# tungphambasement/DCNN

Measured on AMD Instinct MI355X. Metric: images/sec (whole node) ResNet-18 Tiny-ImageNet training at 1/2/4/8 MI355X, higher is better.
Workload: dtype bf16; 1 GPU; model=resnet18_tiny_imagenet, global_batch=256, per_gpu_batch=256, parallelism=dp1, optimizer=adam, hipgraph=True, engine=native (C++ host API)

## Files before the change

### dcnn_amd/csrc/host/dcnn/nn.hpp

```cpp
#pragma once
#include <functional>
#include <map>
#include <memory>
#include <string>
#include <vector>

#include "json.hpp"
#include "ops.hpp"
#include "tensor.hpp"

namespace dcnn {

struct ParamArena;
struct Param {
  std::string name;
  std::vector<int64_t> shape;
  Layout layout = Layout::NCHW;
  Tensor value, grad, shadow;
  Tensor m, v;
  std::shared_ptr<ParamArena> arena;
};

struct ParamArena {
  Tensor value, grad, m, v, shadow;
// ... 39 lines not shown
  };
  MbCache& mbc() { return caches_[mb_]; }
  std::map<int, MbCache> caches_;
  int mb_ = 0;
  bool input_grad_ = true;
  Param& add_param(const std::string& n, const std::vector<int64_t>& shape, Layout phys, const std::vector<float>& init);
  std::string name_;
  Device dev_ = Device::cpu();
  std::vector<Param> params_;
};

class ConvBase : public Layer {
 public:
  std::vector<int64_t> output_shape(const std::vector<int64_t>& in) const override;
  void build(const std::vector<int64_t>& in, Device dev, uint64_t seed) override;
  Tensor forward(const Tensor& x, bool training) override;
  Tensor backward(const Tensor& dy) override { return backward_impl(dy, nullptr); }
  double flops(const std::vector<int64_t>& in) const override;
  virtual bool backward_residual(const Tensor& dy, const Tensor& residual, Tensor& dx) {
    (void)dy; (void)residual; (void)dx;
    return false;
  }

 protected:
  ConvBase(int in_ch, int out_ch, int kh, int kw, int groups, int sh, int sw, int ph, int pw, bool bias,
           std::string name)
      : Layer(std::move(name)), ci_(in_ch), co_(out_ch), kh_(kh), kw_(kw), g_(groups), sh_(sh), sw_(sw), ph_(ph),
        pw_(pw), bias_(bias) {}
  ConvShape shape_for(const std::vector<int64_t>& in) const;
  void geometry_config(json::Value& p) const;
  const float* bias_value() const { return bias_ ? params_[1].value.ptr<float>() : nullptr; }
  float* bias_grad() { return bias_ ? params_[1].grad.ptr<float>() : nullptr; }
  virtual bool depthwise() const { return false; }
  int group_in() const { return depthwise() ? 1 : ci_ / g_; }
  Tensor backward_impl(const Tensor& dy, const Tensor* residual);
  int ci_, co_, kh_, kw_, g_, sh_, sw_, ph_, pw_;
  bool bias_;
};

class Conv2D : public ConvBase {
 public:
  Conv2D(int in_ch, int out_ch, int kh, int kw, int sh = 1, int sw = 1, int ph = 0, int pw = 0, bool bias = true,
         std::string name = "conv2d");
  std::string type() const override { return "conv2d"; }
  json::Value parameters_config() const override;
  Tensor forward(const Tensor& x, bool training) override;
  Tensor backward(const Tensor& dy) override;
  bool takes_raw_input(const std::vector<int64_t>& in) const override;
  void set_stats_consumer(class BatchNorm* bn) { stats_to_ = bn; }
  void set_bnb_producer(class BatchNorm* bn) { bnb_from_ = bn; }
  void set_block_bnb_producer(class BatchNorm* bn) { bnb_block_from_ = bn; }
  bool backward_residual(const Tensor& dy, const Tensor& residual, Tensor& dx) override;
  bool ran_stem() const;
  void backward_stem_bn(const Tensor& dy, const gpu_ops::StemBn& bn);
  void sync_shadow() override;
  bool make_transposed_operand(std::vector<int64_t>& row, long& tiles);

 private:
  class BatchNorm* stats_to_ = nullptr;
  class BatchNorm* bnb_from_ = nullptr;
  class BatchNorm* bnb_block_from_ = nullptr;
  Tensor wt_;
  const void* dgrad_operand(bool& transposed) const;
};

class DepthwiseConv2D : public ConvBase {
 public:
  DepthwiseConv2D(int channels, int kh, int kw, int sh = 1, int sw = 1, int ph = 0, int pw = 0, bool bias = true,
                  std::string name = "depthwise_conv2d");
  std::string type() const override { return "depthwise_conv2d"; }
  json::Value parameters_config() const override;

 protected:
  bool depthwise() const override { return true; }
};

class GroupedConv2D : public ConvBase {
 public:
  GroupedConv2D(int in_ch, int out_ch, int kh, int kw, int groups, int sh = 1, int sw = 1, int ph = 0, int pw = 0,
                bool bias = true, std::string name = "grouped_conv2d");
  std::string type() const override { return "grouped_conv2d"; }
  json::Value parameters_config() const override;
  bool backward_residual(const Tensor& dy, const Tensor& residual, Tensor& dx) override;
};

class Dense : public Layer {
 public:
  Dense(int in_features, int out_features, bool bias = true, std::string name = "dense");
  std::string type() const override { return "dense"; }
  json::Value parameters_config() const override;
  std::vector<int64_t> output_shape(const std::vector<int64_t>& in) const override;
  void build(const std::vector<int64_t>& in, Device dev, uint64_t seed) override;
  Tensor forward(const Tensor& x, bool training) override;
  Tensor backward(const Tensor& dy) override;
  double flops(const std::vector<int64_t>& in) const override { return 6.0 * in[0] * in_ * out_; }

 private:
  int in_, out_;
  bool bias_;
};

class BatchNorm : public Layer {
 public:
  explicit BatchNorm(int num_features, float eps = 1e-5f, float momentum = 0.1f, bool affine = true,
                     std::string name = "batchnorm");
  std::string type() const override { return "batchnorm"; }
  json::Value parameters_config() const override;
  std::vector<int64_t> output_shape(const std::vector<int64_t>& in) const override { return in; }
  double flops(const std::vector<int64_t>& in) const override {
    return 15.0 * (double)in[0] * (double)in[1] * (double)in[2] * (double)in[3];
  }
  void build(const std::vector<int64_t>& in, Device dev, uint64_t seed) override;
  Tensor forward(const Tensor& x, bool training) override;
  Tensor backward(const Tensor& dy) override;
  void set_fused_relu(bool b) { fused_relu_ = b; }
  bool fused_relu() const { return fused_relu_; }
  Tensor forward_residual(const Tensor& x, const Tensor& residual, bool relu, bool training);
  Tensor backward_residual(const Tensor& dy, Tensor* branch);
  void forward_deferred(const Tensor& x, bool training);
  Tensor forward_dual(const Tensor& x, BatchNorm& deferred, bool relu, bool training);
  bool backward_dual(const Tensor& dy, BatchNorm& deferred, Tensor& dx, Tensor& dx_deferred);
  void set_fused_pool(class Pool2D* p) { fused_pool_ = p; }
  bool fused_pool() const { return fused_pool_ != nullptr; }
  gpu_ops::BnbOperands bnb_operands(int mb);
  void offer_bwd_stats(const void* dy, const float* slab, int rows) {
    bwd_dy_ = dy;
    bwd_slab_ = slab;
    bwd_rows_ = rows;
  }
  void offer_stats(const void* x, const float* slab, int rows) {
    pending_x_ = x;
    pending_slab_ = slab;
    pending_rows_ = rows;
  }
  bool backward_into_stem(const Tensor& dy, Conv2D& stem);
  Tensor running_mean, running_var;

 private:
  int c_;
  float eps_, momentum_;
  bool affine_;
  bool train_ = true;
  bool fused_relu_ = false;
  Tensor forward_impl(const Tensor& x, bool training, const Tensor* residual, bool relu);
  Tensor apply_deferred(bool training);
  class Pool2D* fused_pool_ = nullptr;
  gpu_ops::BnRaw deferred_raw_{nullptr, 0};
  const void* bwd_dy_ = nullptr;
  const float* bwd_slab_ = nullptr;
  int bwd_rows_ = 0;
  const void* pending_x_ = nullptr;
  const float* pending_slab_ = nullptr;
  int pending_rows_ = 0;
};

class Activation : public Layer {
 public:
  explicit Activation(std::string kind = "relu", std::string name = "activation");
  std::string type() const override { return "activation"; }
  json::Value parameters_config() const override;
  std::vector<int64_t> output_shape(const std::vector<int64_t>& in) const override { return in; }
  Tensor forward(const Tensor& x, bool training) override;
  Tensor backward(const Tensor& dy) override;
  bool is_relu() const;
  void set_passthrough(bool b) { passthrough_ = b; }

 private:
  std::string kind_;
  int code_;
  bool passthrough_ = false;
};

class GroupNorm : public Layer {
 public:
  GroupNorm(int num_groups, int num_channels, float eps = 1e-5f, bool affine = true, std::string name = "groupnorm");
  std::string type() const override { return "groupnorm"; }
  json::Value parameters_config() const override;
  std::vector<int64_t> output_shape(const std::vector<int64_t>& in) const override { return in; }
  void build(const std::vector<int64_t>& in, Device dev, uint64_t seed) override;
  Tensor forward(const Tensor& x, bool training) override;
  Tensor backward(const Tensor& dy) override;

 private:
  int g_, c_;
  float eps_;
  bool affine_;
  bool gb_identity_ = false;
  Tensor ident_, scratch_;
};

class Dropout : public Layer {
 public:
  explicit Dropout(float rate = 0.5f, std::string name = "dropout");
  std::string type() const override { return "dropout"; }
  json::Value parameters_config() const override;
  std::vector<int64_t> output_shape(const std::vector<int64_t>& in) const override { return in; }
  void build(const std::vector<int64_t>& in, Device dev, uint64_t seed) override;
  Tensor forward(const Tensor& x, bool training) override;
  Tensor backward(const Tensor& dy) override;

 private:
  float p_;
  uint64_t seed_ = 0, draw_ = 0;
};

class Pool2D : public Layer {
 public:
  Pool2D(bool max, int kh, int kw, int sh, int sw, int ph, int pw, std::string name);
  std::string type() const override { return max_ ? "maxpool2d" : "avgpool2d"; }
  json::Value parameters_config() const override;
  std::vector<int64_t> output_shape(const std::vector<int64_t>& in) const override;
  Tensor forward(const Tensor& x, bool training) override;
  Tensor backward(const Tensor& dy) override;
  bool is_max() const { return max_; }
  PoolShape shape_for(const std::vector<int64_t>& in) const;
  void set_fused_producer(class BatchNorm* bn) { bn_ = bn; }
  uint8_t* accept_prepooled(const Tensor& ypool, const std::vector<int64_t>& in);
  void clear_prepooled() { mbc().flag = false; }

 private:
  class BatchNorm* bn_ = nullptr;
  bool max_;
  int kh_, kw_, sh_, sw_, ph_, pw_;
};

class Flatten : public Layer {
 public:
  explicit Flatten(std::string name = "flatten") : Layer(std::move(name)) {}
  std::string type() const override { return "flatten"; }
  json::Value parameters_config() const override { return json::Value::object(); }
  std::vector<int64_t> output_shape(const std::vector<int64_t>& in) const override;
  Tensor forward(const Tensor& x, bool training) override;
  Tensor backward(const Tensor& dy) override;
};

class ResidualBlock : public Layer {
 public:
  ResidualBlock(std::vector<std::unique_ptr<Layer>> main, std::vector<std::unique_ptr<Layer>> shortcut,
                std::string activation = "relu", std::string name = "residual_block");
  std::string type() const override { return "residual_block"; }
  json::Value parameters_config() const override;
  std::vector<int64_t> output_shape(const std::vector<int64_t>& in) const override;
  double flops(const std::vector<int64_t>& in) const override;
  void build(const std::vector<int64_t>& in, Device dev, uint64_t seed) override;
  Tensor forward(const Tensor& x, bool training) override;
  Tensor backward(const Tensor& dy) override;
  void sync_shadow() override;
  void collect_params(std::vector<Param*>& out) override;
  void collect_layers(std::vector<Layer*>& out) override;
  void set_micro_batch(int mb) override;
  const std::vector<std::unique_ptr<Layer>>& main_path() const { return main_; }
  const std::vector<std::unique_ptr<Layer>>& shortcut_path() const { return short_; }
  class BatchNorm* fused_tail() const;
  class Conv2D* head_conv() const;
  class BatchNorm* dual_shortcut() const;

 private:
  std::vector<std::unique_ptr<Layer>> main_, short_;
  std::string act_;
};

std::unique_ptr<Layer> create_layer(const json::Value& rec);

void fuse_bn_relu(std::vector<std::unique_ptr<Layer>>& seq, bool on);
void fuse_blocks(std::vector<std::unique_ptr<Layer>>& seq, bool on);

class Sequential {
 public:
  explicit Sequential(std::string name = "sequential") : name_(std::move(name)) {}
  Sequential(Sequential&&) = default;
  Sequential& operator=(Sequential&&) = default;
// ... 175 lines not shown
```

### dcnn_amd/csrc/host/dcnn/ops.hpp

```cpp
#pragma once
#include <cstdint>

namespace dcnn {

struct ConvShape {
  int N, C, H, W, Co, KH, KW, SH, SW, PH, PW, OH, OW;
};
struct PoolShape {
  int N, C, H, W, OH, OW, KH, KW, SH, SW, PH, PW;
};
enum ActKind { ACT_RELU = 0, ACT_LEAKY_RELU = 1, ACT_ELU = 2, ACT_SIGMOID = 3, ACT_TANH = 4, ACT_LINEAR = 5 };

namespace cpu_ops {
void conv_fwd(const float* x, const float* w, const float* b, float* y, const ConvShape& s);
void conv_bwd(const float* x, const float* w, const float* dy, float* dx, float* dw, float* db, const ConvShape& s);
void dwconv_fwd(const float* x, const float* w, const float* b, float* y, const ConvShape& s);
void dwconv_bwd(const float* x, const float* w, const float* dy, float* dx, float* dw, float* db, const ConvShape& s);
void gconv_fwd(const float* x, const float* w, const float* b, float* y, const ConvShape& s, int groups);
void gconv_bwd(const float* x, const float* w, const float* dy, float* dx, float* dw, float* db, const ConvShape& s,
               int groups);
void dense_fwd(const float* x, const float* w, const float* b, float* y, long N, long In, long Out);
void dense_bwd(const float* x, const float* w, const float* dy, float* dx, float* dw, float* db, long N, long In,
               long Out);
void bn_fwd(const float* x, float* y, long N, long C, long HW, const float* g, const float* b, float eps, bool train,
// ... 22 lines not shown
          float bc2, float wd, bool decoupled);
void sgd(float* p, const float* g, float* vel, long n, float lr, float momentum);
}

namespace gpu_ops {
void begin_deferred_reduce();
void end_deferred_reduce();
void flush_deferred_reduce();
void set_fault(int f);
void input_to_nhwc(const float* x, void* y, int N, int C, int HW);
void nhwc_to_nchw(const void* x, void* y, int N, int HW, int C);
void nchw_to_nhwc_bf16(const void* x, void* y, int N, int HW, int C);
void cast_bf16(const float* x, void* y, long n);
void zero(void* p, long nbytes);
const float* conv_fwd(const void* x, const void* w, const float* bias, void* y, const ConvShape& s,
                      int* stat_rows = nullptr);
struct BnbOperands {
  const void* y;
  const void* x;
  const float* mean;
  const float* istd;
  const float* gamma = nullptr;
  const float* beta = nullptr;
  bool mask_from_x = false;
};
const float* conv_dgrad(const void* dy, const void* w, void* dx, const ConvShape& s, const void* residual = nullptr,
                        bool w_transposed = false, const BnbOperands* bnb = nullptr, int* bnb_rows = nullptr);
void weight_transpose(const void* w, void* wt, int Co, int T, int C);
void multi_weight_transpose(const int64_t* table, int n, long max_tiles);
void conv_wgrad(const void* dy, const void* x, float* gw, float* gb, const ConvShape& s);
void dwconv_fwd(const void* x, const void* w, const float* bias, void* y, const ConvShape& s);
void dwconv_dgrad(const void* dy, const void* w, void* dx, const ConvShape& s, const void* residual = nullptr);
void dwconv_wgrad(const void* dy, const void* x, float* gw, float* gb, const ConvShape& s);
void gconv_fwd(const void* x, const void* w, const float* bias, void* y, const ConvShape& s, int groups);
void gconv_dgrad(const void* dy, const void* w, void* dx, const ConvShape& s, int groups,
                 const void* residual = nullptr);
void gconv_wgrad(const void* dy, const void* x, float* gw, float* gb, const ConvShape& s, int groups);
bool stem_ok(const ConvShape& s);
const float* stem_fwd(const float* x, const void* w, const float* bias, void* y, const ConvShape& s,
                      int* stat_rows = nullptr);
void stem_wgrad(const void* dy, const float* x, float* gw, float* gb, const ConvShape& s);
struct StemBn {
  const void* x;
  const float* mean;
  const float* istd;
  const float* gamma;
  float* dgamma;
  float* dbeta;
  const float* slab;
  int rows;
  bool train;
};
void stem_wgrad_bn(const void* dy, const float* x, float* gw, float* gb, const ConvShape& s, const StemBn& bn);
void dense_fwd(const void* x, const void* w, const float* bias, void* y, int N, int In, int Out);
void dense_dgrad(const void* dy, const void* w, void* dx, int N, int In, int Out);
void dense_wgrad(const void* dy, const void* x, float* gw, float* gb, int N, int In, int Out);
void bn_fwd(const void* x, void* y, long R, int C, const float* g, const float* b, float eps, bool train,
            float* rmean, float* rvar, float momentum, float* smean, float* sistd, bool relu = false,
            const void* residual = nullptr);
void bn_fwd_slab(const void* x, void* y, long R, int C, const float* slab, int rows, const float* g, const float* b,
                 float eps, float* rmean, float* rvar, float momentum, float* smean, float* sistd, bool relu,
                 const void* residual = nullptr);
void bn_bwd_slab(const void* dy, const void* x, void* dx, long R, int C, const float* mean, const float* istd,
                 const float* g, float* dg, float* db, bool train, const float* slab, int rows);
void bn_bwd(const void* dy, const void* x, void* dx, long R, int C, const float* mean, const float* istd,
            const float* g, float* dg, float* db, bool train, const void* yout = nullptr, void* dy_out = nullptr);
struct SecondaryStats {
  SecondaryStats();
  ~SecondaryStats();
};
struct BnRaw {
  const float* slab;
  int rows;
};
BnRaw bn_stats_raw(const void* x, long R, int C, const float* slab, int rows);
struct BnFwdSide {
  const void* x;
  BnRaw raw;
  const float* g;
  const float* b;
  float eps;
  float* rmean;
  float* rvar;
  float momentum;
  float* smean;
  float* sistd;
};
bool bn_dual_ok(long R, int C);
void bn_fwd_dual(const BnFwdSide& a, const BnFwdSide& b, void* y, long R, int C, bool relu, bool train);
struct BnBwdSides {
  const void* x;
  void* dx;
  const float* mean;
  const float* istd;
  const float* g;
  float* dg;
  float* db;
};
void bn_bwd_dual(const void* dy, const BnBwdSides& a, const float* slab_a, int rows_a, const BnBwdSides& b, long R,
                 int C);
bool bn_relu_maxpool_ok(const PoolShape& p);
void bn_relu_maxpool(const void* x, void* y, uint8_t* idx, const PoolShape& p, const float* slab, int rows,
                     const float* g, const float* b, float eps, float* rmean, float* rvar, float momentum,
                     float* smean, float* sistd);
const float* maxpool_bwd_bnb(const void* dy, const uint8_t* idx, const void* ypool, const void* x, const float* mean,
                             const float* istd, void* dx, const PoolShape& p, int* rows);
void maxpool_fwd(const void* x, void* y, uint8_t* idx, const PoolShape& p);
void maxpool_bwd(const void* dy, const uint8_t* idx, void* dx, const PoolShape& p);
void avgpool_fwd(const void* x, void* y, const PoolShape& p);
void avgpool_bwd(const void* dy, void* dx, const PoolShape& p);
void act_fwd(int kind, const void* x, void* y, long n, float alpha);
void act_bwd(int kind, const void* x, const void* dy, void* dx, long n, float alpha);
double softmax_ce(const void* pred, const int64_t* labels, void* grad, int N, int C, long* correct);
double loss(int kind, const void* pred, const float* target, const int64_t* labels, void* grad, int N, int C,
            float param, long* correct, float grad_scale = 1.f);
void loss_launch(int kind, const void* pred, const float* target, const int64_t* labels, void* grad, int N, int C,
                 float param, float grad_scale = 1.f);
double read_last_loss(long* correct);
void groupnorm_fwd(const void* x, void* y, int N, int HW, int C, int G, const float* g, const float* b, float eps,
                   float* smean, float* sistd);
void groupnorm_bwd(const void* dy, const void* x, void* dx, int N, int HW, int C, int G, const float* g,
                   const float* mean, const float* istd, float* dg, float* db);
void softmax_fwd(const void* x, void* y, long rows, int C);
void softmax_bwd(const void* y, const void* dy, void* dx, long rows, int C);
void dropout(const void* x, void* y, long n, float p, uint64_t seed);
void add(const void* a, const void* b, void* y, long n, bool relu);
void relu_mask(const void* dy, const void* y, void* dx, long n);
void adam(float* p, const float* g, float* m, float* v, void* shadow, long n, float lr, float b1, float b2, float eps,
          float bc1, float bc2, float wd, bool decoupled);
void sgd(float* p, const float* g, float* vel, void* shadow, long n, float lr, float momentum);
void adam_hyper_step(float* hyper, float b1, float b2);
void adam_dev(float* p, const float* g, float* m, float* v, void* shadow, long n, float b1, float b2, float eps,
              float wd, bool decoupled, const float* hyper);
const void* loss_device();
}

}
```

### dcnn_amd/csrc/host/nn.cpp

```cpp
#include "dcnn/nn.hpp"

#include "../kernels/fusion_plan.h"

#include <algorithm>
#include <chrono>
#include <cmath>
#include <cstdio>
#include <cstdlib>
#include <filesystem>
#include <fstream>
#include <iostream>
#include <sstream>
#include <stdexcept>

namespace dcnn {

namespace {
struct Rng {
  uint64_t s;
  explicit Rng(uint64_t seed) : s(seed * 0x9e3779b97f4a7c15ull + 0x632be59bd9b4e019ull) {}
  uint64_t next() {
    uint64_t z = (s += 0x9e3779b97f4a7c15ull);
    z = (z ^ (z >> 30)) * 0xbf58476d1ce4e5b9ull;
    z = (z ^ (z >> 27)) * 0x94d049bb133111ebull;
// ... 125 lines not shown
    if (depthwise())
      cpu_ops::dwconv_fwd(x.ptr<float>(), w, b, y.ptr<float>(), s);
    else
      cpu_ops::gconv_fwd(x.ptr<float>(), w, b, y.ptr<float>(), s, g_);
  }
  mbc().a = x;
  return y;
}

Tensor ConvBase::backward_impl(const Tensor& dy, const Tensor* residual) {
  const Tensor& x_ = mbc().a;
  const ConvShape s = shape_for(x_.shape());
  float* gw = params_[0].grad.ptr<float>();
  float* gb = bias_grad();
  if (dev_.is_gpu()) {
    if (depthwise())
      gpu_ops::dwconv_wgrad(dy.data(), x_.data(), gw, gb, s);
    else
      gpu_ops::gconv_wgrad(dy.data(), x_.data(), gw, gb, s, g_);
    if (!input_grad_ && residual == nullptr) return Tensor();
    Tensor dx = act_empty(x_.shape(), dev_);
    const void* w = params_[0].shadow.data();
    const void* r = residual ? residual->data() : nullptr;
    if (depthwise())
      gpu_ops::dwconv_dgrad(dy.data(), w, dx.data(), s, r);
    else
      gpu_ops::gconv_dgrad(dy.data(), w, dx.data(), s, g_, r);
    return dx;
  }
  Tensor dx = input_grad_ ? act_empty(x_.shape(), dev_) : Tensor();
  float* dxp = input_grad_ ? dx.ptr<float>() : nullptr;
  const float* w = params_[0].value.ptr<float>();
  if (depthwise())
    cpu_ops::dwconv_bwd(x_.ptr<float>(), w, dy.ptr<float>(), dxp, gw, gb, s);
  else
    cpu_ops::gconv_bwd(x_.ptr<float>(), w, dy.ptr<float>(), dxp, gw, gb, s, g_);
  return dx;
}

Conv2D::Conv2D(int in_ch, int out_ch, int kh, int kw, int sh, int sw, int ph, int pw, bool bias, std::string name)
    : ConvBase(in_ch, out_ch, kh, kw, 1, sh, sw, ph, pw, bias, std::move(name)) {}

json::Value Conv2D::parameters_config() const {
  json::Value p = json::Value::object();
  p["in_channels"] = ci_;
  p["out_channels"] = co_;
  p["kernel_h"] = kh_;
  p["kernel_w"] = kw_;
  geometry_config(p);
  p["optimized"] = "mfma";
  return p;
}

bool Conv2D::takes_raw_input(const std::vector<int64_t>& in) const {
  return dev_.is_gpu() && in.size() == 4 && in[1] == ci_ && gpu_ops::stem_ok(shape_for(in));
}

Tensor Conv2D::forward(const Tensor& x, bool training) {
  Tensor& x_ = mbc().a;
  check_act(x, dev_, "conv2d");
  const ConvShape s = shape_for(x.shape());
  Tensor y = act_empty({s.N, s.Co, s.OH, s.OW}, dev_);
  const float* b = bias_value();
  if (dev_.is_gpu() && x.dtype() == DType::F32) {
    if (x.layout() != Layout::NCHW || !gpu_ops::stem_ok(s)) throw std::runtime_error(name_ + ": fp32 input");
    int rows = 0;
    const float* st = gpu_ops::stem_fwd(x.ptr<float>(), params_[0].shadow.data(), b, y.data(), s,
                                        stats_to_ && training ? &rows : nullptr);
    if (stats_to_ && training) stats_to_->offer_stats(y.data(), st, rows);
    x_ = x;
    return y;
  }
  if (dev_.is_gpu()) {
    int rows = 0;
    const float* st = gpu_ops::conv_fwd(x.data(), params_[0].shadow.data(), b, y.data(), s,
                                        stats_to_ && training ? &rows : nullptr);
    if (stats_to_ && training) stats_to_->offer_stats(y.data(), st, rows);
  } else
    cpu_ops::conv_fwd(x.ptr<float>(), params_[0].value.ptr<float>(), b, y.ptr<float>(), s);
  x_ = x;
  return y;
}

bool Conv2D::ran_stem() const {
  const Tensor& x_ = const_cast<Conv2D*>(this)->mbc().a;
  return dev_.is_gpu() && x_.defined() && x_.dtype() == DType::F32;
}

void Conv2D::backward_stem_bn(const Tensor& dy, const gpu_ops::StemBn& bn) {
  const Tensor& x_ = mbc().a;
  const ConvShape s = shape_for(x_.shape());
  gpu_ops::stem_wgrad_bn(dy.data(), x_.ptr<float>(), params_[0].grad.ptr<float>(), bias_grad(), s, bn);
}

Tensor Conv2D::backward(const Tensor& dy) {
  const Tensor& x_ = mbc().a;
  const ConvShape s = shape_for(x_.shape());
  float* gb = bias_grad();
  if (dev_.is_gpu() && x_.dtype() == DType::F32) {
    gpu_ops::stem_wgrad(dy.data(), x_.ptr<float>(), params_[0].grad.ptr<float>(), gb, s);
    return Tensor();
  }
  if (dev_.is_gpu()) {
    gpu_ops::conv_wgrad(dy.data(), x_.data(), params_[0].grad.ptr<float>(), gb, s);
    if (!input_grad_) return Tensor();
    Tensor dx = act_empty(x_.shape(), dev_);
    bool tr = false;
    const void* w = dgrad_operand(tr);
    if (bnb_from_ != nullptr) {
      const gpu_ops::BnbOperands ops = bnb_from_->bnb_operands(mb_);
      int rows = 0;
      const float* st = gpu_ops::conv_dgrad(dy.data(), w, dx.data(), s, nullptr, tr, &ops, &rows);
      if (rows > 0) bnb_from_->offer_bwd_stats(dx.data(), st, rows);
      return dx;
    }
    gpu_ops::conv_dgrad(dy.data(), w, dx.data(), s, nullptr, tr);
    return dx;
  }
  Tensor dx = act_empty(x_.shape(), dev_);
  {
    cpu_ops::conv_bwd(x_.ptr<float>(), params_[0].value.ptr<float>(), dy.ptr<float>(), dx.ptr<float>(),
                      params_[0].grad.ptr<float>(), gb, s);
  }
  return dx;
}

bool Conv2D::backward_residual(const Tensor& dy, const Tensor& residual, Tensor& dx) {
  const Tensor& x_ = mbc().a;
  if (!dev_.is_gpu() || x_.dtype() == DType::F32 || residual.shape() != x_.shape())
    throw std::runtime_error(name_ + ": backward_residual is a GPU fusion");
  const ConvShape s = shape_for(x_.shape());
  float* gb = bias_grad();
  gpu_ops::conv_wgrad(dy.data(), x_.data(), params_[0].grad.ptr<float>(), gb, s);
  dx = act_empty(x_.shape(), dev_);
  bool tr = false;
  const void* w = dgrad_operand(tr);
  if (bnb_block_from_ != nullptr) {
    const gpu_ops::BnbOperands ops = bnb_block_from_->bnb_operands(mb_);
    int rows = 0;
    const float* st = gpu_ops::conv_dgrad(dy.data(), w, dx.data(), s, residual.data(), tr, &ops, &rows);
    if (rows > 0) bnb_block_from_->offer_bwd_stats(dx.data(), st, rows);
    return true;
  }
  gpu_ops::conv_dgrad(dy.data(), w, dx.data(), s, residual.data(), tr);
  return true;
// ... 147 lines not shown
json::Value BatchNorm::parameters_config() const {
  json::Value p = json::Value::object();
  p["num_features"] = c_;
  p["epsilon"] = (double)eps_;
  p["momentum"] = (double)momentum_;
  p["affine"] = affine_;
  return p;
}

void BatchNorm::build(const std::vector<int64_t>& in, Device dev, uint64_t seed) {
  (void)in;
  (void)seed;
  dev_ = dev;
  params_.clear();
  if (affine_) {
    add_param("gamma", {c_, 1, 1, 1}, Layout::NCHW, std::vector<float>((size_t)c_, 1.f));
    add_param("beta", {c_, 1, 1, 1}, Layout::NCHW, std::vector<float>((size_t)c_, 0.f));
  }
  running_mean = Tensor::zeros({c_}, DType::F32, dev);
  running_var = Tensor::from_host(std::vector<float>((size_t)c_, 1.f), {c_}, dev);
  caches_.clear();
}

Tensor BatchNorm::forward(const Tensor& x, bool training) { return forward_impl(x, training, nullptr, fused_relu_); }

Tensor BatchNorm::forward_residual(const Tensor& x, const Tensor& residual, bool relu, bool training) {
  if (!dev_.is_gpu()) throw std::runtime_error(name_ + ": forward_residual is a GPU fusion");
  if (residual.shape() != x.shape()) throw std::runtime_error(name_ + ": residual shape mismatch");
  return forward_impl(x, training, &residual, relu);
}

Tensor BatchNorm::forward_impl(const Tensor& x, bool training, const Tensor* residual, bool relu) {
  check_act(x, dev_, "batchnorm");
  MbCache& mc = mbc();
  Tensor& x_ = mc.a;
  Tensor& mean_ = mc.b;
  Tensor& istd_ = mc.c;
  mean_.ensure({c_}, DType::F32, dev_);
  istd_.ensure({c_}, DType::F32, dev_);
  if (x.dim(1) != c_) throw std::runtime_error(name_ + ": channel count mismatch");
  train_ = training;
  const long N = x.dim(0), HW = x.dim(2) * x.dim(3);
  Tensor y = act_empty(x.shape(), dev_);
  const float* g = affine_ ? params_[0].value.ptr<float>() : nullptr;
  const float* b = affine_ ? params_[1].value.ptr<float>() : nullptr;
  const void* res = residual ? residual->data() : nullptr;
  const bool slab = dev_.is_gpu() && training && pending_x_ == x.data() && pending_slab_ && pending_rows_ > 0;
  if (fused_pool_ != nullptr) {
    fused_pool_->set_micro_batch(mb_);
    const PoolShape p = fused_pool_->shape_for(x.shape());
    if (dev_.is_gpu() && training && relu && residual == nullptr && gpu_ops::bn_relu_maxpool_ok(p)) {
      Tensor yp = act_empty({p.N, p.C, p.OH, p.OW}, dev_);
      uint8_t* idx = fused_pool_->accept_prepooled(yp, x.shape());
      gpu_ops::bn_relu_maxpool(x.data(), yp.data(), idx, p, slab ? pending_slab_ : nullptr, slab ? pending_rows_ : 0,
                               g, b, eps_, running_mean.ptr<float>(), running_var.ptr<float>(), momentum_,
                               mean_.ptr<float>(), istd_.ptr<float>());
      mc.d = Tensor();
      mc.flag = false;
      pending_x_ = nullptr;
      pending_slab_ = nullptr;
      pending_rows_ = 0;
      x_ = x;
      return yp;
    }
    fused_pool_->clear_prepooled();
  }
  if (slab) {
    gpu_ops::bn_fwd_slab(x.data(), y.data(), N * HW, c_, pending_slab_, pending_rows_, g, b, eps_,
                         running_mean.ptr<float>(), running_var.ptr<float>(), momentum_, mean_.ptr<float>(),
                         istd_.ptr<float>(), relu, res);
    mc.d = relu ? y : Tensor();
    mc.flag = relu && res == nullptr && training;
  } else if (dev_.is_gpu()) {
    gpu_ops::bn_fwd(x.data(), y.data(), N * HW, c_, g, b, eps_, training, running_mean.ptr<float>(),
                    running_var.ptr<float>(), momentum_, mean_.ptr<float>(), istd_.ptr<float>(), relu, res);
    mc.d = relu ? y : Tensor();
    mc.flag = relu && res == nullptr && training;
  } else {
    cpu_ops::bn_fwd(x.ptr<float>(), y.ptr<float>(), N, c_, HW, g, b, eps_, training, running_mean.ptr<float>(),
                    running_var.ptr<float>(), momentum_, mean_.ptr<float>(), istd_.ptr<float>());
  }
  pending_x_ = nullptr;
  pending_slab_ = nullptr;
  pending_rows_ = 0;
  x_ = x;
  return y;
}

void BatchNorm::forward_deferred(const Tensor& x, bool training) {
  check_act(x, dev_, "batchnorm");
  if (!dev_.is_gpu()) throw std::runtime_error(name_ + ": forward_deferred is a GPU fusion");
  if (x.dim(1) != c_) throw std::runtime_error(name_ + ": channel count mismatch");
  MbCache& mc = mbc();
  mc.a = x;
  mc.b.ensure({c_}, DType::F32, dev_);
  mc.c.ensure({c_}, DType::F32, dev_);
  mc.d = Tensor();
  mc.flag = false;
  train_ = training;
  deferred_raw_ = gpu_ops::BnRaw{nullptr, 0};
  if (training) {
    const bool slab = pending_x_ == x.data() && pending_slab_ && pending_rows_ > 0;
    deferred_raw_ = gpu_ops::bn_stats_raw(x.data(), x.dim(0) * x.dim(2) * x.dim(3), c_, slab ? pending_slab_ : nullptr,
                                          slab ? pending_rows_ : 0);
  }
  pending_x_ = nullptr;
  pending_slab_ = nullptr;
  pending_rows_ = 0;
}
// ... 61 lines not shown
  MbCache& mc = mbc();
  MbCache& oc = o.mbc();
  const Tensor& x_ = mc.a;
  if (!dev_.is_gpu() || bwd_dy_ != dy.data() || bwd_slab_ == nullptr || bwd_rows_ <= 0 || !train_ || !o.train_ ||
      oc.a.shape() != x_.shape() || o.c_ != c_)
    return false;
  const long R = x_.dim(0) * x_.dim(2) * x_.dim(3);
  if (!gpu_ops::bn_dual_ok(R, c_)) return false;
  dx = act_empty(x_.shape(), dev_);
  dx_o = act_empty(oc.a.shape(), dev_);
  auto side = [](BatchNorm& l, MbCache& c, Tensor& d) {
    return gpu_ops::BnBwdSides{c.a.data(),
                               d.data(),
                               c.b.ptr<float>(),
                               c.c.ptr<float>(),
                               l.affine_ ? l.params_[0].value.ptr<float>() : nullptr,
                               l.affine_ ? l.params_[0].grad.ptr<float>() : nullptr,
                               l.affine_ ? l.params_[1].grad.ptr<float>() : nullptr};
  };
  gpu_ops::bn_bwd_dual(dy.data(), side(*this, mc, dx), bwd_slab_, bwd_rows_, side(o, oc, dx_o), R, c_);
  bwd_dy_ = nullptr;
  bwd_slab_ = nullptr;
  bwd_rows_ = 0;
  return true;
}

Tensor BatchNorm::backward_residual(const Tensor& dy, Tensor* branch) {
  MbCache& mc = mbc();
  const Tensor& x_ = mc.a;
  const long N = x_.dim(0), HW = x_.dim(2) * x_.dim(3);
  Tensor dx = act_empty(x_.shape(), dev_);
  const float* g = affine_ ? params_[0].value.ptr<float>() : nullptr;
  float* dg = affine_ ? params_[0].grad.ptr<float>() : nullptr;
  float* db = affine_ ? params_[1].grad.ptr<float>() : nullptr;
  if (bwd_dy_ == dy.data() && bwd_slab_ != nullptr && bwd_rows_ > 0) {
    *branch = dy;
    gpu_ops::bn_bwd_slab(dy.data(), x_.data(), dx.data(), N * HW, c_, mc.b.ptr<float>(), mc.c.ptr<float>(), g, dg, db,
                         train_, bwd_slab_, bwd_rows_);
    bwd_dy_ = nullptr;
    bwd_slab_ = nullptr;
    bwd_rows_ = 0;
  } else if (mc.d.defined()) {
    *branch = act_empty(dy.shape(), dev_);
    gpu_ops::bn_bwd(dy.data(), x_.data(), dx.data(), N * HW, c_, mc.b.ptr<float>(), mc.c.ptr<float>(), g, dg, db,
                    train_, mc.d.data(), branch->data());
  } else {
    *branch = dy;
    gpu_ops::bn_bwd(dy.data(), x_.data(), dx.data(), N * HW, c_, mc.b.ptr<float>(), mc.c.ptr<float>(), g, dg, db,
                    train_);
  }
  return dx;
}

bool BatchNorm::backward_into_stem(const Tensor& dy, Conv2D& stem) {
  MbCache& mc = mbc();
  if (!dev_.is_gpu() || !train_ || bwd_dy_ != dy.data() || bwd_slab_ == nullptr || bwd_rows_ <= 0 ||
      !stem.ran_stem() || mc.a.dtype() != DType::BF16)
    return false;
  gpu_ops::StemBn bn{mc.a.data(),
                     mc.b.ptr<float>(),
                     mc.c.ptr<float>(),
                     affine_ ? params_[0].value.ptr<float>() : nullptr,
                     affine_ ? params_[0].grad.ptr<float>() : nullptr,
                     affine_ ? params_[1].grad.ptr<float>() : nullptr,
                     bwd_slab_,
                     bwd_rows_,
                     train_};
  stem.backward_stem_bn(dy, bn);
  bwd_dy_ = nullptr;
  bwd_slab_ = nullptr;
  bwd_rows_ = 0;
  return true;
}

Tensor BatchNorm::backward(const Tensor& dy) {
  MbCache& mc = mbc();
  const Tensor& x_ = mc.a;
  Tensor& mean_ = mc.b;
  Tensor& istd_ = mc.c;
  const long N = x_.dim(0), HW = x_.dim(2) * x_.dim(3);
  Tensor dx = act_empty(x_.shape(), dev_);
  const float* g = affine_ ? params_[0].value.ptr<float>() : nullptr;
  float* dg = affine_ ? params_[0].grad.ptr<float>() : nullptr;
  float* db = affine_ ? params_[1].grad.ptr<float>() : nullptr;
  if (dev_.is_gpu() && bwd_dy_ == dy.data() && bwd_slab_ != nullptr && bwd_rows_ > 0) {
    gpu_ops::bn_bwd_slab(dy.data(), x_.data(), dx.data(), N * HW, c_, mean_.ptr<float>(), istd_.ptr<float>(), g, dg,
                         db, train_, bwd_slab_, bwd_rows_);
    bwd_dy_ = nullptr;
    bwd_slab_ = nullptr;
    bwd_rows_ = 0;
  } else if (dev_.is_gpu())
    gpu_ops::bn_bwd(dy.data(), x_.data(), dx.data(), N * HW, c_, mean_.ptr<float>(), istd_.ptr<float>(), g, dg, db,
                    train_, mc.d.defined() ? mc.d.data() : nullptr);
  else
    cpu_ops::bn_bwd(x_.ptr<float>(), dy.ptr<float>(), mean_.ptr<float>(), istd_.ptr<float>(), g, dx.ptr<float>(), dg,
                    db, N, c_, HW, train_);
  return dx;
}

Activation::Activation(std::string kind, std::string name)
    : Layer(std::move(name)), kind_(std::move(kind)), code_(act_code(kind_)) {}

json::Value Activation::parameters_config() const {
  json::Value p = json::Value::object();
  p["activation"] = kind_;
  return p;
}

static float act_alpha(int code) { return code == ACT_ELU ? 1.0f : 0.01f; }

bool Activation::is_relu() const { return code_ == ACT_RELU; }

static int fuse_kind(const Layer* l) {
  if (dynamic_cast<const Conv2D*>(l)) return FK_CONV;
  if (dynamic_cast<const BatchNorm*>(l)) return FK_BN;
  if (auto* a = dynamic_cast<const Activation*>(l)) return a->is_relu() ? FK_RELU : FK_ACT;
  if (auto* p = dynamic_cast<const Pool2D*>(l)) return p->is_max() ? FK_MAXPOOL : FK_OTHER;
  return FK_OTHER;
}

static std::vector<int> fuse_kinds(const std::vector<std::unique_ptr<Layer>>& seq) {
  std::vector<int> k;
  for (const auto& l : seq) k.push_back(fuse_kind(l.get()));
  return k;
}

void fuse_bn_relu(std::vector<std::unique_ptr<Layer>>& seq, bool on) {
  const std::vector<int> f = plan_sequence_fusions(fuse_kinds(seq));
  for (size_t i = 0; i < seq.size(); ++i) {
// ... 400 lines not shown
  p.W = (int)in[3];
  p.KH = kh_;
  p.KW = kw_;
  p.SH = sh_;
  p.SW = sw_;
  p.PH = ph_;
  p.PW = pw_;
  p.OH = (p.H + 2 * ph_ - kh_) / sh_ + 1;
  p.OW = (p.W + 2 * pw_ - kw_) / sw_ + 1;
  return p;
}

std::vector<int64_t> Pool2D::output_shape(const std::vector<int64_t>& in) const {
  const PoolShape p = shape_for(in);
  return {in[0], in[1], p.OH, p.OW};
}

uint8_t* Pool2D::accept_prepooled(const Tensor& ypool, const std::vector<int64_t>& in) {
  MbCache& mc = mbc();
  const PoolShape p = shape_for(in);
  mc.a.ensure({(int64_t)p.N * p.C * p.OH * p.OW}, DType::U8, dev_);
  mc.b = ypool;
  mc.shape = in;
  mc.flag = true;
  return mc.a.ptr<uint8_t>();
}

Tensor Pool2D::forward(const Tensor& x, bool training) {
  (void)training;
  if (bn_ != nullptr && mbc().flag && mbc().b.defined() && mbc().b.data() == x.data())
    return x;
  mbc().flag = false;
  Tensor& idx_ = mbc().a;
  std::vector<int64_t>& in_shape_ = mbc().shape;
  check_act(x, dev_, "pool2d");
  const PoolShape p = shape_for(x.shape());
  Tensor y = act_empty({p.N, p.C, p.OH, p.OW}, dev_);
  in_shape_ = x.shape();
  if (max_) {
    const int64_t n = (int64_t)p.N * p.C * p.OH * p.OW;
    if (dev_.is_gpu()) {
      idx_.ensure({n}, DType::U8, dev_);
      gpu_ops::maxpool_fwd(x.data(), y.data(), idx_.ptr<uint8_t>(), p);
    } else {
      idx_.ensure({n}, DType::I32, dev_);
      cpu_ops::maxpool_fwd(x.ptr<float>(), y.ptr<float>(), idx_.ptr<int32_t>(), p);
    }
  } else if (dev_.is_gpu()) {
    gpu_ops::avgpool_fwd(x.data(), y.data(), p);
  } else {
    cpu_ops::avgpool_fwd(x.ptr<float>(), y.ptr<float>(), p);
  }
  return y;
}

Tensor Pool2D::backward(const Tensor& dy) {
  const Tensor& idx_ = mbc().a;
  const std::vector<int64_t>& in_shape_ = mbc().shape;
  const PoolShape p = shape_for(in_shape_);
  Tensor dx = act_empty(in_shape_, dev_);
  if (mbc().flag && bn_ != nullptr) {
    const gpu_ops::BnbOperands ops = bn_->bnb_operands(mb_);
    int rows = 0;
    const float* slab = gpu_ops::maxpool_bwd_bnb(dy.data(), idx_.ptr<uint8_t>(), mbc().b.data(), ops.x, ops.mean,
                                                 ops.istd, dx.data(), p, &rows);
    bn_->offer_bwd_stats(dx.data(), slab, rows);
    return dx;
  }
  if (max_) {
    if (dev_.is_gpu())
      gpu_ops::maxpool_bwd(dy.data(), idx_.ptr<uint8_t>(), dx.data(), p);
    else
      cpu_ops::maxpool_bwd(dy.ptr<float>(), idx_.ptr<int32_t>(), dx.ptr<float>(), p);
  } else if (dev_.is_gpu()) {
    gpu_ops::avgpool_bwd(dy.data(), dx.data(), p);
  } else {
    cpu_ops::avgpool_bwd(dy.ptr<float>(), dx.ptr<float>(), p);
  }
  return dx;
}

std::vector<int64_t> Flatten::output_shape(const std::vector<int64_t>& in) const {
  return {in[0], in[1] * in[2] * in[3], 1, 1};
}

Tensor Flatten::forward(const Tensor& x, bool training) {
  (void)training;
  std::vector<int64_t>& in_shape_ = mbc().shape;
  check_act(x, dev_, "flatten");
  in_shape_ = x.shape();
  const auto os = output_shape(x.shape());
  const int64_t HW = x.dim(2) * x.dim(3);
  if (!dev_.is_gpu()) return x.view(os);
  if (HW == 1) return x.view(os, Layout::NHWC);
  Tensor y = act_empty(os, dev_);
  gpu_ops::nhwc_to_nchw(x.data(), y.data(), (int)x.dim(0), (int)HW, (int)x.dim(1));
  return y;
}

Tensor Flatten::backward(const Tensor& dy) {
  const std::vector<int64_t>& in_shape_ = mbc().shape;
  const int64_t HW = in_shape_[2] * in_shape_[3];
  if (!dev_.is_gpu()) return dy.view(in_shape_);
  if (HW == 1) return dy.view(in_shape_, Layout::NHWC);
  Tensor dx = act_empty(in_shape_, dev_);
  gpu_ops::nchw_to_nhwc_bf16(dy.data(), dx.data(), (int)in_shape_[0], (int)HW, (int)in_shape_[1]);
// ... 153 lines not shown
std::vector<BatchNorm*> Sequential::batchnorms() {
  std::vector<Layer*> all;
  for (auto& l : layers_) l->collect_layers(all);
  std::vector<BatchNorm*> out;
  for (auto* l : all)
    if (auto* bn = dynamic_cast<BatchNorm*>(l)) out.push_back(bn);
  return out;
}

size_t Sequential::num_parameters() {
  size_t n = 0;
  for (auto* p : parameters()) n += (size_t)p->value.numel();
  return n;
}

void Sequential::zero_grad() {
  if (arena_) {
    gpu_ops::zero(arena_->grad.data(), (long)arena_->grad.nbytes());
    return;
  }
  for (auto* p : parameters()) {
    if (dev_.is_gpu())
      gpu_ops::zero(p->grad.data(), (long)p->grad.nbytes());
    else
      p->grad.zero_();
  }
}

std::vector<double> Sequential::layer_flops(const std::vector<int64_t>& in) const {
  std::vector<double> out;
  std::vector<int64_t> s = in;
  for (auto& l : layers_) {
    out.push_back(l->flops(s));
    s = l->output_shape(s);
  }
  return out;
}

Tensor Sequential::input_activation(const Tensor& x_in) const {
  if (x_in.rank() != 4 || x_in.dtype() != DType::F32) throw std::runtime_error("forward: expected fp32 (N, C, H, W)");
  Tensor x = x_in.device() == dev_ ? x_in : x_in.to(dev_);
  if (dev_.is_gpu() && !layers_.empty() && layers_[0]->takes_raw_input(x.shape())) return x;
  if (dev_.is_gpu()) {
    Tensor a = Tensor::empty(x.shape(), DType::BF16, dev_, Layout::NHWC);
    gpu_ops::input_to_nhwc(x.ptr<float>(), a.data(), (int)x.dim(0), (int)x.dim(1), (int)(x.dim(2) * x.dim(3)));
    x = a;
  }
  return x;
}

Tensor Sequential::forward_activation(const Tensor& x_in, int mb) {
  if (!initialized_) throw std::runtime_error("Sequential::forward before initialize()");
  Tensor x = x_in;
  for (auto& l : layers_) {
    l->set_micro_batch(mb);
    x = l->forward(x, training_);
  }
  return x;
}

Tensor Sequential::backward_activation(const Tensor& g_in, int mb) {
  Tensor g = g_in;
  static const bool defer_env = [] {
    const char* v = std::getenv("DCNN_DEFER_REDUCE");
    return !(v && std::string(v) == "0");
  }();
  const bool defer = dev_.is_gpu() && defer_env;
  static const bool stem_bn_env = [] {
    const char* v = std::getenv("DCNN_STEM_BN_FOLD");
    return !(v && std::string(v) == "0");
  }();
  const bool stem_bn_fold = dev_.is_gpu() && stem_bn_env && layers_.size() > 1;
  if (defer) gpu_ops::begin_deferred_reduce();
  try {
    for (size_t i = layers_.size(); i-- > 0;) {
      layers_[i]->set_micro_batch(mb);
      if (i == 1 && stem_bn_fold) {
        auto* bn = dynamic_cast<BatchNorm*>(layers_[1].get());
        auto* conv = dynamic_cast<Conv2D*>(layers_[0].get());
        if (bn && conv) {
          conv->set_micro_batch(mb);
          if (bn->backward_into_stem(g, *conv)) {
            if (bwd_hook_) bwd_hook_(1);
            if (bwd_hook_) bwd_hook_(0);
            g = Tensor();
            break;
          }
        }
      }
      g = layers_[i]->backward(g);
      if (bwd_hook_) bwd_hook_(i);
    }
  } catch (...) {
    if (defer) gpu_ops::end_deferred_reduce();
    throw;
  }
  if (defer) gpu_ops::end_deferred_reduce();
  return g;
}

Tensor Sequential::forward(const Tensor& x_in, int mb) {
  Tensor x = forward_activation(input_activation(x_in), mb);
  return x.view({x.dim(0), x.dim(1) * x.dim(2) * x.dim(3)}, x.layout());
}

void Sequential::backward(const Tensor& dlogits, int mb) {
  if (!layers_.empty()) layers_[0]->set_input_grad(false);
  Tensor g = dlogits.view({dlogits.dim(0), dlogits.dim(1), 1, 1}, dev_.is_gpu() ? Layout::NHWC : Layout::NCHW);
  backward_activation(g, mb);
}

json::Value Sequential::get_config() const {
  json::Value c = json::Value::object();
  c["name"] = name_;
  c["is_training"] = training_;
  json::Value ls = json::Value::array();
  for (auto& l : layers_) {
    json::Value r = json::Value::object();
    r["type"] = l->type();
    r["name"] = l->name();
    r["parameters"] = l->parameters_config();
    ls.push(std::move(r));
  }
  c["layers"] = std::move(ls);
  if (!input_chw_.empty() && input_chw_[0] > 0) {
    json::Value in = json::Value::array();
    for (auto v : input_chw_) in.push(v);
    c["input_shape"] = std::move(in);
  }
  return c;
}

void Sequential::print_config() const { std::cout << get_config().dump(2) << std::endl; }

Sequential Sequential::load_from_config(const json::Value& cfg) {
  Sequential m(cfg.get_string("name", "sequential"));
  for (auto& r : cfg.at("layers").items()) m.add(create_layer(r));
  m.set_training(cfg.get_bool("is_training", true));
  if (const json::Value* in = cfg.find("input_shape")) {
// ... 428 lines not shown
```

### dcnn_amd/csrc/host/ops_gpu.hip

```cpp
#include <hip/hip_runtime.h>

#include <algorithm>
#include <cmath>
#include <cstdio>
#include <cstdlib>
#include <cstring>
#include <map>
#include <mutex>
#include <stdexcept>
#include <string>
#include <unordered_map>
#include <vector>

#include "../kernels/api.h"
#include "dcnn/ops.hpp"
#include "dcnn/tensor.hpp"

#define HOST_HIP_CHECK(x)                                                                    \
  do {                                                                                       \
    hipError_t e_ = (x);                                                                     \
    if (e_ != hipSuccess) throw std::runtime_error(std::string(#x) + ": " + hipGetErrorString(e_)); \
  } while (0)

namespace dcnn {
// ... 663 lines not shown
  wgrad_split(splits, (long)s.C * s.KH * s.KW, s.C, gw, gb,
              [&](float* slab, float* bslab) { dcnn::dwconv_wgrad(kBF16, dy, x, slab, bslab, g, cur()); });
}

namespace {
GcArgs gc_args(const ConvShape& s, int groups) {
  return GcArgs{s.N, s.H, s.W, s.C, s.Co, groups, s.OH, s.OW, s.KH, s.KW, s.SH, s.SW, s.PH, s.PW};
}
}

void gconv_fwd(const void* x, const void* w, const float* bias, void* y, const ConvShape& s, int groups) {
  rec("gc_fwd", s, -1, {{"bias", bias != nullptr}});
  dcnn::gconv_fwd(kBF16, x, w, bias, y, gc_args(s, groups), cur());
}

void gconv_dgrad(const void* dy, const void* w, void* dx, const ConvShape& s, int groups, const void* residual) {
  rec("gc_dgrad", s, -1, {{"residual", residual != nullptr}});
  const GcArgs g = gc_args(s, groups);
  if (!dcnn::gconv_supported(kBF16, g)) throw std::invalid_argument("gconv_dgrad: unsupported grouped conv shape");
  void* wt = scratch(W_T, (size_t)s.C * s.KH * s.KW * (s.Co / groups) * 2);
  dcnn::gconv_weight_t(kBF16, w, wt, g, cur());
  dcnn::gconv_dgrad(kBF16, dy, wt, residual, dx, g, cur());
}

void gconv_wgrad(const void* dy, const void* x, float* gw, float* gb, const ConvShape& s, int groups) {
  rec("gc_wgrad", s, -1, {{"bias", gb != nullptr}, {"deferred", g_defer}});
  const GcArgs g = gc_args(s, groups);
  const int splits = dcnn::gconv_wgrad_splits(kBF16, g);
  wgrad_split(splits, (long)s.Co * s.KH * s.KW * (s.C / groups), s.Co, gw, gb,
              [&](float* slab, float* bslab) { dcnn::gconv_wgrad(kBF16, dy, x, slab, bslab, g, cur()); });
}

bool stem_ok(const ConvShape& s) {
  return s.KH == 3 && s.KW == 3 && s.SH == 1 && s.SW == 1 && s.PH == 1 && s.PW == 1 &&
         stem_supported(s.N, s.C, s.H, s.W, s.Co);
}

const float* stem_fwd(const float* x, const void* w, const float* bias, void* y, const ConvShape& s, int* stat_rows) {
  rec("stem_fwd", s, -1, {{"bias", bias != nullptr}, {"stats", stat_rows != nullptr}});
  StemArgs a{};
  a.x = x; a.w = w; a.w_bf16 = 1;
  a.ws[0] = 9l * s.C; a.ws[1] = 1; a.ws[2] = 3l * s.C; a.ws[3] = s.C;
  a.bias = bias; a.y = static_cast<bf16*>(y);
  a.N = s.N; a.Ci = s.C; a.H = s.H; a.W = s.W; a.Co = s.Co;
  if (stat_rows) {
    *stat_rows = stem_tiles_host(s.N, s.H, s.W);
    a.slab = static_cast<float*>(scratch(fwd_stats_slot(), (size_t)*stat_rows * 3 * s.Co * 4));
  }
  dcnn::stem_fwd(a, cur());
  return a.slab;
}

static void stem_wgrad_impl(const void* dy, const float* x, float* gw, float* gb, const ConvShape& s,
                            const StemBn* bn);

void stem_wgrad(const void* dy, const float* x, float* gw, float* gb, const ConvShape& s) {
  stem_wgrad_impl(dy, x, gw, gb, s, nullptr);
}

static std::pair<const float*, int> reduce_stats(int mode, const float* slab, int rows, int C);

void stem_wgrad_bn(const void* dy, const float* x, float* gw, float* gb, const ConvShape& s, const StemBn& bn) {
  stem_wgrad_impl(dy, x, gw, gb, s, &bn);
}

static void stem_wgrad_impl(const void* dy, const float* x, float* gw, float* gb, const ConvShape& s,
                            const StemBn* bn) {
  rec("stem_wgrad", s, -1, {{"bias", gb != nullptr}, {"deferred", g_defer}, {"bn", bn != nullptr}});
  std::pair<const float*, int> st{nullptr, 0};
  if (bn) st = reduce_stats(1, bn->slab, bn->rows, s.Co);
  const int blocks = bn ? stem_wgrad_blocks_bnt(s.N, s.H, s.W) : stem_wgrad_blocks(s.N, s.H, s.W);
  const long n = 9l * s.C * s.Co;
  wgrad_split(blocks, n, s.Co, gw, gb, [&](float* slab, float* bslab) {
    StemArgs a{};
    a.x = x; a.dy = static_cast<const bf16*>(dy); a.slab = slab; a.bias_slab = bslab;
    a.gs[0] = 9l * s.C; a.gs[1] = 1; a.gs[2] = 3l * s.C; a.gs[3] = s.C;
    a.n_slab = n;
    a.N = s.N; a.Ci = s.C; a.H = s.H; a.W = s.W; a.Co = s.Co;
    if (bn) {
      a.bn_x = static_cast<const bf16*>(bn->x); a.bn_mean = bn->mean; a.bn_istd = bn->istd; a.bn_gamma = bn->gamma;
      a.bn_sums = st.first; a.bn_parts = st.second; a.bn_count = (float)((long)s.N * s.H * s.W);
      a.bn_dgamma = bn->dgamma; a.bn_dbeta = bn->dbeta; a.bn_eval = bn->train ? 0 : 1;
    }
    dcnn::stem_wgrad(a, blocks, cur());
  });
}

void dense_fwd(const void* x, const void* w, const float* bias, void* y, int N, int In, int Out) {
  NtArgs a{static_cast<const bf16*>(x), static_cast<const bf16*>(w), y, N, Out, In, In, In, Out, kPlain, 0, 0, 0, 0,
           1, 1, 1, 1, 1, 1, 0, 0, bias, nullptr, nullptr, 0, 0};
  gemm_nt(a, cur());
}

void dense_dgrad(const void* dy, const void* w, void* dx, int N, int In, int Out) {
  bf16* wt = static_cast<bf16*>(scratch(W_T, (size_t)In * Out * 2));
  conv_weight_transpose(kBF16, w, wt, Out, 1, In, cur());
  NtArgs a{static_cast<const bf16*>(dy), wt, dx, N, In, Out, Out, Out, In, kPlain, 0, 0, 0, 0, 1, 1, 1, 1, 1, 1, 0, 0,
           nullptr, nullptr, nullptr, 0, 0};
  gemm_nt(a, cur());
}

void dense_wgrad(const void* dy, const void* x, float* gw, float* gb, int N, int In, int Out) {
  const int splits = gemm_tn_splits(Out, In, N);
  wgrad_split(splits, (long)Out * In, Out, gw, gb, [&](float* slab, float* bslab) {
    TnArgs a{static_cast<const bf16*>(dy), static_cast<const bf16*>(x), slab, bslab, Out, In, N, kPlain, 0, 0, 0, 0,
             1, 1, 1, 1, 1, 1, 0, 0, In, 0};
    gemm_tn(a, splits, cur());
  });
}

static std::pair<const float*, int> reduce_stats(int mode, const float* slab, int rows, int C) {
  const int parts = bn_stat_parts(rows);
  float* sums = static_cast<float*>(scratch(STAT_SUMS, (size_t)2 * C * 4));
  float* part = parts > 1 ? static_cast<float*>(scratch(STAT_PART, (size_t)parts * 3 * C * 4)) : nullptr;
  bn_stat_reduce(mode, slab, rows, C, sums, part, nullptr, cur());
  return {parts > 1 ? part : sums, parts};
}

void bn_fwd(const void* x, void* y, long R, int C, const float* g, const float* b, float eps, bool train,
            float* rmean, float* rvar, float momentum, float* smean, float* sistd, bool relu, const void* residual) {
  if (!train) {
    bn_apply(kBF16, x, y, R, C, nullptr, 1, (float)R, g, b, eps, residual, relu ? 1 : 0, smean, sistd, rmean, rvar,
             momentum, 1, cur());
    return;
  }
  const int rows = bn_partial_rows(R, C);
  float* slab = static_cast<float*>(scratch(STAT_SLAB, (size_t)rows * 3 * C * 4));
  bn_partial(kBF16, x, nullptr, nullptr, nullptr, nullptr, nullptr, R, C, slab, 0, nullptr, cur());
  const auto st = reduce_stats(0, slab, rows, C);
  bn_apply(kBF16, x, y, R, C, st.first, st.second, (float)R, g, b, eps, residual, relu ? 1 : 0, smean, sistd, rmean,
           rvar, momentum, 0, cur());
}

void bn_fwd_slab(const void* x, void* y, long R, int C, const float* slab, int rows, const float* g, const float* b,
                 float eps, float* rmean, float* rvar, float momentum, float* smean, float* sistd, bool relu,
                 const void* residual) {
// ... 24 lines not shown
  if (slab != nullptr && rows > 0) return BnRaw{slab, rows};
  const int n = bn_partial_rows(R, C);
  float* s = static_cast<float*>(scratch(STAT_SLAB2, (size_t)n * 3 * C * 4));
  bn_partial(kBF16, x, nullptr, nullptr, nullptr, nullptr, nullptr, R, C, s, 0, nullptr, cur());
  return BnRaw{s, n};
}

bool bn_dual_ok(long R, int C) { return bn_apply_dual_supported(R, C); }

static void reduce_pair(int mode, const float* slab_a, int rows_a, const float* slab_b, int rows_b, int C,
                        std::pair<const float*, int>& a, std::pair<const float*, int>& b) {
  const int pa = bn_stat_parts(rows_a), pb = bn_stat_parts(rows_b);
  float* sa = static_cast<float*>(scratch(STAT_SUMS, (size_t)2 * C * 4));
  float* sb = static_cast<float*>(scratch(STAT_SUMS2, (size_t)2 * C * 4));
  float* qa = pa > 1 ? static_cast<float*>(scratch(STAT_PART, (size_t)pa * 3 * C * 4)) : nullptr;
  float* qb = pb > 1 ? static_cast<float*>(scratch(STAT_PART2, (size_t)pb * 3 * C * 4)) : nullptr;
  bn_stat_reduce2(mode, slab_a, rows_a, sa, qa, slab_b, rows_b, sb, qb, C, cur());
  a = {pa > 1 ? qa : sa, pa};
  b = {pb > 1 ? qb : sb, pb};
}

void bn_fwd_dual(const BnFwdSide& a, const BnFwdSide& b, void* y, long R, int C, bool relu, bool train) {
  std::pair<const float*, int> sa{nullptr, 1}, sb{nullptr, 1};
  if (train) reduce_pair(0, a.raw.slab, a.raw.rows, b.raw.slab, b.raw.rows, C, sa, sb);
  auto side = [&](const BnFwdSide& s, const std::pair<const float*, int>& st) {
    return BnSide{s.x,     st.first, st.second, (float)R, s.g,        s.b,    s.eps,
                  s.smean, s.sistd,  s.rmean,   s.rvar,   s.momentum, train ? 0 : 1};
  };
  if (!bn_apply_dual(side(a, sa), side(b, sb), y, R, C, relu ? 1 : 0, cur()))
    throw std::runtime_error("bn_fwd_dual: unsupported shape");
}

void bn_bwd_dual(const void* dy, const BnBwdSides& a, const float* slab_a, int rows_a, const BnBwdSides& b, long R,
                 int C) {
  const int rows_b = bn_partial_rows(R, C);
  float* slab_b = static_cast<float*>(scratch(STAT_SLAB, (size_t)rows_b * 2 * C * 4));
  bn_partial(kBF16, b.x, dy, nullptr, nullptr, b.mean, b.istd, R, C, slab_b, 1, nullptr, cur());
  std::pair<const float*, int> sa, sb;
  reduce_pair(1, slab_a, rows_a, slab_b, rows_b, C, sa, sb);
  auto side = [&](const BnBwdSides& s, const std::pair<const float*, int>& st) {
    return BnBwdSide{s.x, s.dx, s.mean, s.istd, s.g, st.first, st.second, (float)R, s.dg, s.db};
  };
  if (!bn_bwd_apply_dual(dy, side(a, sa), side(b, sb), R, C, cur()))
    throw std::runtime_error("bn_bwd_dual: unsupported shape");
}

bool bn_relu_maxpool_ok(const PoolShape& p) {
  const PoolGeom g = geom(p);
  return dcnn::bn_relu_maxpool_supported(g) && dcnn::maxpool_bwd_bnb_supported(g);
}

void bn_relu_maxpool(const void* x, void* y, uint8_t* idx, const PoolShape& p, const float* slab, int rows,
                     const float* g, const float* b, float eps, float* rmean, float* rvar, float momentum,
                     float* smean, float* sistd) {
  const long R = (long)p.N * p.H * p.W;
  if (slab == nullptr || rows <= 0) {
    rows = bn_partial_rows(R, p.C);
    float* s = static_cast<float*>(scratch(STAT_SLAB, (size_t)rows * 3 * p.C * 4));
    bn_partial(kBF16, x, nullptr, nullptr, nullptr, nullptr, nullptr, R, p.C, s, 0, nullptr, cur());
    slab = s;
  }
  const auto st = reduce_stats(0, slab, rows, p.C);
  dcnn::bn_relu_maxpool(static_cast<const bf16*>(x), static_cast<bf16*>(y), idx, geom(p), st.first, st.second,
                        (float)R, g, b, eps, smean, sistd, rmean, rvar, momentum, cur());
}

const float* maxpool_bwd_bnb(const void* dy, const uint8_t* idx, const void* ypool, const void* x, const float* mean,
                             const float* istd, void* dx, const PoolShape& p, int* rows) {
  const PoolGeom g = geom(p);
  *rows = maxpool_bwd_bnb_rows(g);
  float* slab = static_cast<float*>(scratch(BWD_STATS, (size_t)*rows * 2 * p.C * 4));
  dcnn::maxpool_bwd_bnb(static_cast<const bf16*>(dy), idx, static_cast<const bf16*>(ypool),
                        static_cast<const bf16*>(x), mean, istd, static_cast<bf16*>(dx), g, slab, nullptr, cur());
  return slab;
}

void maxpool_fwd(const void* x, void* y, uint8_t* idx, const PoolShape& p) {
  if (p.KH * p.KW > 256) throw std::invalid_argument("maxpool: window larger than 256 taps");
  dcnn::maxpool_fwd(kBF16, x, y, idx, geom(p), cur());
}
void maxpool_bwd(const void* dy, const uint8_t* idx, void* dx, const PoolShape& p) {
  dcnn::maxpool_bwd(kBF16, dy, idx, dx, geom(p), cur());
}
void avgpool_fwd(const void* x, void* y, const PoolShape& p) { dcnn::avgpool_fwd(kBF16, x, y, geom(p), cur()); }
void avgpool_bwd(const void* dy, void* dx, const PoolShape& p) { dcnn::avgpool_bwd(kBF16, dy, dx, geom(p), cur()); }

void act_fwd(int kind, const void* x, void* y, long n, float alpha) { dcnn::act_fwd(kBF16, x, y, n, kind, alpha, cur()); }
void act_bwd(int kind, const void* x, const void* dy, void* dx, long n, float alpha) {
  dcnn::act_bwd(kBF16, x, dy, dx, n, kind, alpha, cur());
}

double read_loss(const char* out, long* correct) {
  if (gpu::Graph::capturing()) {
    if (correct) *correct = -1;
    return std::nan("");
  }
  char host[16];
  hipStream_t s = cur();
  HOST_HIP_CHECK(hipMemcpyAsync(host, out, 16, hipMemcpyDeviceToHost, s));
  HOST_HIP_CHECK(hipStreamSynchronize(s));
  float l;
  int c;
  std::memcpy(&l, host, 4);
  std::memcpy(&c, host + 8, 4);
  if (correct) *correct = c;
  return l;
}

double softmax_ce(const void* pred, const int64_t* labels, void* grad, int N, int C, long* correct) {
  float* ws = N > 4 ? static_cast<float*>(scratch(LOSS_WS, (size_t)loss_workspace_floats(N) * 4)) : nullptr;
  static unsigned* tickets = nullptr;
  if (N > 4 && !tickets) {
    tickets = static_cast<unsigned*>(scratch(TICKETS, 64 * 4));
    HOST_HIP_CHECK(hipMemsetAsync(tickets, 0, 64 * 4, cur()));
  }
  char* out = static_cast<char*>(scratch(LOSS_OUT, 16));
  float* loss = reinterpret_cast<float*>(out);
  int* corr = reinterpret_cast<int*>(out + 8);
  loss_fused(kBF16, pred, nullptr, labels, grad, loss, corr, N, C, 1, 1e-15f, 1.0f, ws, N > 4 ? tickets : nullptr,
             cur());
  return read_loss(out, correct);
}

double loss(int kind, const void* pred, const float* target, const int64_t* labels, void* grad, int N, int C,
            float param, long* correct, float grad_scale) {
  loss_launch(kind, pred, target, labels, grad, N, C, param, grad_scale);
// ... 67 lines not shown
```

### dcnn_amd/csrc/host/train.cpp

```cpp
#include "dcnn/train.hpp"

#include <algorithm>
#include <atomic>
#include <chrono>
#include <cmath>
#include <cstdio>
#include <cstring>
#include <filesystem>
#include <fstream>
#include <sstream>
#include <stdexcept>
#include <thread>

namespace dcnn_native {
bool decode_jpeg(const unsigned char* data, size_t n, std::vector<unsigned char>& rgb, int& w, int& h,
                 std::string* err);
}

namespace dcnn {

LossResult Loss::compute(const Tensor& pred, const Tensor* labels_in, const Tensor* target_in, float grad_scale) const {
  if (pred.rank() != 2) throw std::runtime_error("loss: expected [N, C] predictions");
  const int N = (int)pred.dim(0), C = (int)pred.dim(1);
  const Device dev = pred.device();
// ... 496 lines not shown
  }
  std::vector<std::pair<std::string, int>> files;
  if (split == "train") {
    for (size_t c = 0; c < wnids.size(); ++c) {
      const std::string dir = root + "/train/" + wnids[c] + "/images";
      std::vector<std::string> names;
      for (auto& e : std::filesystem::directory_iterator(dir)) names.push_back(e.path().filename().string());
      std::sort(names.begin(), names.end());
      int k = 0;
      for (auto& n : names) {
        if (max_per_class > 0 && k++ >= max_per_class) break;
        files.emplace_back(dir + "/" + n, (int)c);
      }
    }
  } else {
    std::istringstream ss(read_file(root + "/val/val_annotations.txt"));
    std::string l;
    while (std::getline(ss, l)) {
      std::istringstream ls(l);
      std::string f, w;
      if (!std::getline(ls, f, '\t') || !std::getline(ls, w, '\t')) continue;
      auto it = std::find(wnids.begin(), wnids.end(), w);
      if (it != wnids.end()) files.emplace_back(root + "/val/images/" + f, (int)(it - wnids.begin()));
    }
  }
  const size_t N = files.size();
  std::vector<float> img(N * 3 * 64 * 64, 0.f);
  std::vector<int64_t> lab(N);
  std::atomic<int> failures{0};
  parallel_for(N, [&](size_t i) {
    lab[i] = files[i].second;
    std::vector<unsigned char> rgb;
    int w = 0, h = 0;
    bool ok = false;
    try {
      const std::string blob = read_file(files[i].first);
      ok = dcnn_native::decode_jpeg(reinterpret_cast<const unsigned char*>(blob.data()), blob.size(), rgb, w, h,
                                    nullptr);
    } catch (...) {
    }
    if (!ok || w != 64 || h != 64) {
      ++failures;
      return;
    }
    float* o = img.data() + i * 3 * 4096;
    for (int c = 0; c < 3; ++c)
      for (int p = 0; p < 4096; ++p) o[c * 4096 + p] = rgb[(size_t)p * 3 + c] / 255.f;
  });
  if (failures) std::fprintf(stderr, "load_tiny_imagenet: %d undecodable images zero-filled\n", failures.load());
  return ImageDataset(std::move(img), std::move(lab), 3, 64, 64, (int)wnids.size(), seed);
}

Sequential create_model(const std::string& name) {
  if (name == "mnist_cnn")
    return SequentialBuilder("mnist_cnn_model").input({1, 28, 28})
        .conv2d(8, 5, 5, 1, 1, 0, 0, true, "conv1").batchnorm(1e-5f, 0.1f, true, "bn1")
        .activation("relu", "relu1").maxpool2d(3, 3, 3, 3, 0, 0, "pool1")
        .conv2d(16, 1, 1, 1, 1, 0, 0, true, "conv2_1x1").batchnorm(1e-5f, 0.1f, true, "bn2")
        .activation("relu", "relu2")
        .conv2d(48, 5, 5, 1, 1, 0, 0, true, "conv3").batchnorm(1e-5f, 0.1f, true, "bn3")
        .activation("relu", "relu3").maxpool2d(2, 2, 2, 2, 0, 0, "pool2")
        .flatten("flatten").dense(10, true, "output").build();
  if (name == "resnet9_cifar10")
    return SequentialBuilder("ResNet-9-CIFAR10").input({3, 32, 32})
        .conv2d(64, 3, 3, 1, 1, 1, 1, true, "conv1").batchnorm(1e-5f, 0.1f, true, "bn1").activation("relu", "relu1")
        .conv2d(128, 3, 3, 1, 1, 1, 1, true, "conv2").batchnorm(1e-5f, 0.1f, true, "bn2").activation("relu", "relu2")
        .maxpool2d(2, 2, 2, 2, 0, 0, "pool1")
        .basic_residual_block(128, 128, 1, "res_block1").basic_residual_block(128, 128, 1, "res_block2")
        .conv2d(256, 3, 3, 1, 1, 1, 1, true, "conv3").batchnorm(1e-5f, 0.1f, true, "bn3").activation("relu", "relu3")
        .maxpool2d(2, 2, 2, 2, 0, 0, "pool2")
        .basic_residual_block(256, 256, 1, "res_block3").basic_residual_block(256, 256, 1, "res_block4")
        .conv2d(512, 3, 3, 1, 1, 1, 1, true, "conv4").batchnorm(1e-5f, 0.1f, true, "bn4").activation("relu", "relu4")
        .maxpool2d(2, 2, 2, 2, 0, 0, "pool3")
        .basic_residual_block(512, 512, 1, "res_block5")
        .avgpool2d(4, 4, 1, 1, 0, 0, "avgpool").flatten("flatten").dense(10, true, "output").build();
  if (name == "resnet18_tiny_imagenet" || name == "resnet34_tiny_imagenet") {
    const bool r34 = name == "resnet34_tiny_imagenet";
    SequentialBuilder b(r34 ? "ResNet-34-Tiny-ImageNet" : "ResNet-18-Tiny-ImageNet");
    b.input({3, 64, 64}).conv2d(32, 3, 3, 1, 1, 1, 1, false, "conv1").batchnorm(1e-3f, 0.1f, true, "bn1")
        .activation("relu", "relu1").maxpool2d(2, 2, 2, 2, 0, 0, "maxpool");
    const int per[4] = {r34 ? 3 : 2, r34 ? 4 : 2, r34 ? 6 : 2, r34 ? 3 : 2};
    const int width[4] = {64, 128, 256, 512};
    int in = 32;
    for (int L = 0; L < 4; ++L)
      for (int i = 1; i <= per[L]; ++i) {
        b.basic_residual_block(in, width[L], (i == 1 && L > 0) ? 2 : 1,
                               "layer" + std::to_string(L + 1) + "_block" + std::to_string(i));
        in = width[L];
      }
    return b.avgpool2d(4, 4, 1, 1, 0, 0, "avgpool").flatten("flatten").dense(200, true, "fc").build();
  }
  if (name == "resnet50_tiny_imagenet") {
    SequentialBuilder b("ResNet-50-Tiny-ImageNet");
    b.input({3, 64, 64}).conv2d(64, 3, 3, 1, 1, 1, 1, true, "conv1").batchnorm(1e-5f, 0.1f, true, "bn1")
        .activation("relu", "relu1").maxpool2d(3, 3, 2, 2, 1, 1, "maxpool");
    const int per[4] = {3, 4, 6, 3}, mid[4] = {64, 128, 256, 512};
    int in = 64;
    for (int L = 0; L < 4; ++L)
      for (int i = 1; i <= per[L]; ++i) {
        b.bottleneck_residual_block(in, mid[L], 4 * mid[L], (i == 1 && L > 0) ? 2 : 1,
                                    "layer" + std::to_string(L + 1) + "_block" + std::to_string(i));
        in = 4 * mid[L];
      }
    return b.avgpool2d(4, 4, 1, 1, 0, 0, "avgpool").flatten("flatten").dense(200, true, "fc").build();
  }
  if (name == "mobilenet_v1_cifar10" || name == "mobilenet_v1_tiny_imagenet") {
// ... 97 lines not shown
```

### dcnn_amd/csrc/kernels/api.h

```cpp
#pragma once
#include <hip/hip_runtime.h>
#include <stdint.h>

#include "fusion_plan.h"
typedef __bf16 bf16;

namespace dcnn {
struct BnbArgs {
  const bf16* y; const bf16* x; const float* mean; const float* istd;
  const float* gamma; const float* beta; int mask_x;
};
struct NtArgs {
  const bf16* A; const bf16* B; void* C;
  int M, N, K; int lda, ldb, ldc; int mode;
  int nb, sh, sw, cs, gh, gw; int kh, kw, strh, strw, padh, padw;
  const float* bias; const bf16* residual; float* stats; int out_f32; int relu;
};
struct TnArgs {
  const bf16* dY; const bf16* X; float* slab; float* bias_slab;
  int M, N, P; int mode; int nb, sh, sw, cs, gh, gw; int kh, kw, strh, strw, padh, padw; int ldx; int k_per_split;
};
struct G2Args {
  const bf16* A; const bf16* B; bf16* C;
  unsigned a_bytes, b_bytes;
// ... 113 lines not shown
void gemm_g2f(const G2Args& a, hipStream_t s);
int gemm_g2f_stat_rows(int M, int N);
void gemm_t2f(T2Args a, int splits, hipStream_t s);
int gemm_t2f_splits(int M, int N, int P);
void set_f32_mode(int mode);
int get_f32_mode();
void conv_weight_transpose_f32(const float* w, float* wt, int Co, int T_, int Ci, hipStream_t s);
void gemm_tn(TnArgs a, int splits, hipStream_t s);
int gemm_tn_splits(int M, int N, int P);
struct ConvRouteGeom {
  int N, C, H, W, Co, KH, KW, SH, SW, PH, PW, OH, OW, g1s_mode;
};
enum ConvRoute : int { ROUTE_GENERIC = 0, ROUTE_GEMM_G2 = 1, ROUTE_HALO = 2, ROUTE_G1S = 3, ROUTE_HALO_S2 = 4 };
int conv_fwd_route(ConvRouteGeom g);
int conv_dgrad_route(ConvRouteGeom g);
int conv_wgrad_route(ConvRouteGeom g);
void splitk_reduce(const float* slab, float* out, long n, int splits, int accumulate, hipStream_t s);
void splitk_reduce2(const float* slab, float* out, long n, const float* bslab, float* bout, long nb, int splits,
                    int accumulate, hipStream_t s);

constexpr int kMaxRed = 48;
struct RedEnt { const float* slab; float* out; long n; int splits, unit0, chunks, groups, vec, wpc; };
struct MultiRed { int count; RedEnt e[kMaxRed]; };
void multi_splitk_reduce(MultiRed t, hipStream_t s);

int bn_partial_rows(long R, int C);
void bn_partial(int dtype, const void* x, const void* dy, const void* yout, void* dy_out, const float* mean,
                const float* istd, long R, int C, float* slab, int mode, float* zero_sums, hipStream_t s);
int bn_stat_parts(int rows);
void bn_stat_reduce2(int mode, const float* slab, int rows, float* out, float* part, const float* slab2, int rows2,
                     float* out2, float* part2, int C, hipStream_t s);
void bn_stat_reduce(int mode, const float* slab, int rows, int C, float* out, float* part, unsigned* ticket,
                    hipStream_t s);
void bn_apply(int dtype, const void* x, void* y, long R, int C, const float* sums, int parts, float count, const float* gamma,
              const float* beta, float eps, const void* residual, int relu, float* save_mean, float* save_istd,
              float* run_mean, float* run_var, float momentum, int use_running, hipStream_t s);
struct BnSide {
  const void* x; const float* sums; int parts; float count; const float* gamma; const float* beta; float eps;
  float* save_mean; float* save_istd; float* run_mean; float* run_var; float momentum; int use_running;
};
bool bn_apply_dual(const BnSide& a, const BnSide& b, void* y, long R, int C, int relu, hipStream_t s);
bool bn_apply_dual_supported(long R, int C);
struct BnBwdSide {
  const void* x; void* dx; const float* mean; const float* istd; const float* gamma; const float* sums; int parts;
  float count; float* dgamma; float* dbeta;
};
bool bn_bwd_apply_dual(const void* dy, const BnBwdSide& a, const BnBwdSide& b, long R, int C, hipStream_t s);
void bn_bwd_apply(int dtype, const void* dy, const void* yout, const void* x, void* dx, long R, int C, const float* mean,
                  const float* istd, const float* gamma, const float* sums, int parts, float count, float* dgamma,
                  float* dbeta, int eval_mode, hipStream_t s);
bool bn_relu_maxpool_supported(PoolGeom g);
void bn_relu_maxpool(const bf16* x, bf16* y, uint8_t* idx, PoolGeom g, const float* sums, int parts, float count,
                     const float* gamma, const float* beta, float eps, float* save_mean, float* save_istd,
                     float* run_mean, float* run_var, float momentum, hipStream_t s);
void gn_fwd(int dtype, const void* x, void* y, int N, int HW, int C, int G, const float* gamma, const float* beta,
            float eps, float* save_mean, float* save_istd, hipStream_t s);
void gn_bwd(int dtype, const void* dy, const void* x, void* dx, int N, int HW, int C, int G, const float* gamma,
            const float* mean, const float* istd, float* dgamma, float* dbeta, float* aff, hipStream_t s);

void maxpool_fwd(int dt, const void* x, void* y, uint8_t* idx, PoolGeom g, hipStream_t s);
void maxpool_bwd(int dt, const void* dy, const uint8_t* idx, void* dx, PoolGeom g, hipStream_t s);
bool maxpool_bwd_bnb_supported(PoolGeom g);
int maxpool_bwd_bnb_rows(PoolGeom g);
void maxpool_bwd_bnb(const bf16* dy, const uint8_t* idx, const bf16* ypool, const bf16* x, const float* mean,
                     const float* istd, bf16* dx, PoolGeom g, float* slab, float* zero_sums, hipStream_t s);
void avgpool_fwd(int dt, const void* x, void* y, PoolGeom g, hipStream_t s);
void avgpool_bwd(int dt, const void* dy, void* dx, PoolGeom g, hipStream_t s);
void act_fwd(int dt, const void* x, void* y, long n, int type, float a, hipStream_t s);
void act_bwd(int dt, const void* x, const void* dy, void* dx, long n, int type, float a, hipStream_t s);
void softmax_rows(int dt, const void* x, void* y, long rows, int C, hipStream_t s);
void softmax_rows_bwd(int dt, const void* y, const void* dy, void* dx, long rows, int C, hipStream_t s);
void dropout(int dt, const void* x, void* y, long n, float p, uint64_t seed, const uint64_t* ctr, hipStream_t s);
void counter_bump(uint64_t* ctr, uint64_t* slot, hipStream_t s);
void nchw_to_nhwc(int dt, const float* x, void* y, int N, int C, int HW, hipStream_t s);
void nchw_to_nhwc_pad(int dt, const float* x, void* y, int N, int C, int Cp, int HW, hipStream_t s);
void conv_weight_transpose(int src_dt, const void* w, bf16* wt, int Co, int T_, int Ci, hipStream_t s);
void cast_f32_bf16(const float* x, bf16* y, long n, hipStream_t s);
struct StemArgs {
  const float* x; const void* w; int w_bf16; long ws[4];
  const float* bias; bf16* y; float* slab; float* zero_ptr; int zero_n;
  const bf16* dy; float* bias_slab; long gs[4]; long n_slab;
  int halo_bytes; int N, Ci, H, W, Co, TH;
  const bf16* bn_x; const float* bn_mean; const float* bn_istd; const float* bn_gamma; const float* bn_sums;
  int bn_parts; float bn_count; float* bn_dgamma; float* bn_dbeta; int bn_eval;
};
bool stem_supported(int N, int Ci, int H, int W, int Co);
int stem_tiles_host(int N, int H, int W);
int stem_wgrad_blocks(int N, int H, int W);
int stem_wgrad_blocks_bnt(int N, int H, int W);
void stem_fwd(StemArgs a, hipStream_t s);
void stem_wgrad(StemArgs a, int blocks, hipStream_t s);
void multi_weight_transpose(const int64_t* table, int n, long max_tiles, hipStream_t s, int f32 = 0);
void im2col(const float* x, float* col, int N, int C, int H, int W, int KH, int KW, int SH, int SW, int PH, int PW,
            int OH, int OW, hipStream_t s);
void col2im(const float* col, float* x, int N, int C, int H, int W, int KH, int KW, int SH, int SW, int PH, int PW,
            int OH, int OW, hipStream_t s);
int loss_workspace_floats(int N);
void loss_fused(int dt, const void* pred, const float* target, const int64_t* labels, void* grad, float* loss_out,
                int* correct, int N, int C, int type, float param, float gscale, float* ws, unsigned* ticket,
                hipStream_t s);
void adam_step(float* p, const float* g, float* m, float* v, bf16* shadow, long n, float lr, float b1, float b2,
               float eps, float bc1, float bc2, float wd, int decoupled, const float* hyper, hipStream_t s);
void sgd_step(float* p, const float* g, float* vel, bf16* shadow, long n, float lr, float mom, const float* hyper,
              hipStream_t s);
void adam_scalars(float* hyper, float b1, float b2, hipStream_t s);
void grad_pack_bf16(const float* g, bf16* out, long n, float scale, hipStream_t s);
void grad_sum_chunks_bf16(const bf16* src, int w, long ld, long n, bf16* dst, hipStream_t s);
void grad_unpack_bf16(const bf16* in, float* g, long n, hipStream_t s);
void zero_bytes(void* p, long nbytes, hipStream_t s);
void copy_pair(void* d0, const void* s0, long n0, void* d1, const void* s1, long n1, hipStream_t s);
void split3_bf16(const float* in, bf16* out, long rows, int C, int pattern, hipStream_t s);
void im2col_nhwc(int dt, const void* x, void* col, const ConvGeom& g, hipStream_t s);
void col2im_nhwc(int dt, const void* col, void* x, const void* residual, const ConvGeom& g, int chan_major,
                 hipStream_t s);
enum { AUG_HFLIP = 0, AUG_VFLIP, AUG_ROTATION, AUG_BRIGHTNESS, AUG_CONTRAST, AUG_NOISE, AUG_CROP, AUG_CUTOUT,
       AUG_NORMALIZE };
constexpr int kAugMaxOps = 12;
constexpr int kAugMaxFloats = 16384;
struct AugOpDev {
  int kind;
  float p;
  float a[6];
};
struct AugBatchArgs {
  const void* src;
  int src_u8;
  const int64_t* idx;
  const int64_t* labels;
  int64_t* labels_out;
  float* out;
  int B, C, H, W;
  unsigned long long seed;
  int nops;
  AugOpDev ops[kAugMaxOps];
};
bool augment_batch_supported(int C, int H, int W);
void augment_batch(const AugBatchArgs& a, hipStream_t s);
// ... 4 lines not shown
```

### dcnn_amd/csrc/kernels/bindings.cpp

```cpp
#include <tuple>
#include <pybind11/pybind11.h>
#include <pybind11/stl.h>
#include <algorithm>
#include <array>
#include <vector>
#include <hip/hip_runtime.h>
#include <stdint.h>

namespace py = pybind11;
#include "api.h"


using namespace dcnn;
void bind_runtime(py::module_& m);
void bind_rccl(py::module_& m);
template <typename T>
static inline T P(uintptr_t x) { return reinterpret_cast<T>(x); }
static inline hipStream_t S(uintptr_t x) { return reinterpret_cast<hipStream_t>(x); }

using Ptr4 = std::array<uintptr_t, 4>;
static BnbArgs bnb_of(const Ptr4& b) {
  return BnbArgs{P<const bf16*>(b[0]), P<const bf16*>(b[1]), P<const float*>(b[2]), P<const float*>(b[3])};
}

// ... 342 lines not shown

  auto gc = [](const std::array<int, 14>& g) {
    return GcArgs{g[0], g[1], g[2], g[3], g[4], g[5], g[6], g[7], g[8], g[9], g[10], g[11], g[12], g[13]};
  };
  m.def("gconv_supported", [gc](int dt, std::array<int, 14> g) { return gconv_supported(dt, gc(g)); });
  m.def("gconv_wgrad_splits", [gc](int dt, std::array<int, 14> g) { return gconv_wgrad_splits(dt, gc(g)); });
  m.def("gconv_fwd", [gc](int dt, uintptr_t x, uintptr_t w, uintptr_t bias, uintptr_t y, std::array<int, 14> g,
                          uintptr_t st) {
    gconv_fwd(dt, P<const void*>(x), P<const void*>(w), P<const float*>(bias), P<void*>(y), gc(g), S(st));
  });
  m.def("gconv_weight_t", [gc](int dt, uintptr_t w, uintptr_t wt, std::array<int, 14> g, uintptr_t st) {
    gconv_weight_t(dt, P<const void*>(w), P<void*>(wt), gc(g), S(st));
  });
  m.def("gconv_dgrad", [gc](int dt, uintptr_t dy, uintptr_t wt, uintptr_t residual, uintptr_t dx,
                            std::array<int, 14> g, uintptr_t st) {
    gconv_dgrad(dt, P<const void*>(dy), P<const void*>(wt), P<const void*>(residual), P<void*>(dx), gc(g), S(st));
  });
  m.def("gconv_wgrad", [gc](int dt, uintptr_t dy, uintptr_t x, uintptr_t slab, uintptr_t bslab,
                            std::array<int, 14> g, uintptr_t st) {
    gconv_wgrad(dt, P<const void*>(dy), P<const void*>(x), P<float*>(slab), P<float*>(bslab), gc(g), S(st));
  });

  auto geom = [](int N, int H, int W, int C, int OH, int OW, int ph, int pw, int sh, int sw, int padh, int padw) {
    return PoolGeom{N, H, W, C, OH, OW, ph, pw, sh, sw, padh, padw};
  };
  m.def("maxpool_fwd", [geom](int dt, uintptr_t x, uintptr_t y, uintptr_t idx, int N, int H, int W, int C, int OH,
                              int OW, int ph, int pw, int sh, int sw, int padh, int padw, uintptr_t st) {
    maxpool_fwd(dt, P<const void*>(x), P<void*>(y), P<uint8_t*>(idx), geom(N, H, W, C, OH, OW, ph, pw, sh, sw, padh, padw),
                S(st));
  });
  m.def("maxpool_bwd", [geom](int dt, uintptr_t dy, uintptr_t idx, uintptr_t dx, int N, int H, int W, int C, int OH,
                              int OW, int ph, int pw, int sh, int sw, int padh, int padw, uintptr_t st) {
    maxpool_bwd(dt, P<const void*>(dy), P<const uint8_t*>(idx), P<void*>(dx),
                geom(N, H, W, C, OH, OW, ph, pw, sh, sw, padh, padw), S(st));
  });
  m.def("maxpool_bwd_bnb_supported", [geom](int N, int H, int W, int C, int OH, int OW, int ph, int pw, int sh, int sw,
                                            int padh, int padw) {
    return maxpool_bwd_bnb_supported(geom(N, H, W, C, OH, OW, ph, pw, sh, sw, padh, padw));
  });
  m.def("bn_relu_maxpool_supported", [geom](int N, int H, int W, int C, int OH, int OW, int ph, int pw, int sh, int sw,
                                            int padh, int padw) {
    return bn_relu_maxpool_supported(geom(N, H, W, C, OH, OW, ph, pw, sh, sw, padh, padw));
  });
  m.def("bn_relu_maxpool", [geom](uintptr_t x, uintptr_t y, uintptr_t idx, int N, int H, int W, int C, int OH, int OW,
                                  int ph, int pw, int sh, int sw, int padh, int padw, uintptr_t sums, int parts,
                                  float count,
                                  uintptr_t gamma, uintptr_t beta, float eps, uintptr_t save_mean, uintptr_t save_istd,
                                  uintptr_t run_mean, uintptr_t run_var, float momentum, uintptr_t st) {
    bn_relu_maxpool(P<const bf16*>(x), P<bf16*>(y), P<uint8_t*>(idx), geom(N, H, W, C, OH, OW, ph, pw, sh, sw, padh, padw),
                    P<const float*>(sums), parts, count, P<const float*>(gamma), P<const float*>(beta), eps,
                    P<float*>(save_mean), P<float*>(save_istd), P<float*>(run_mean), P<float*>(run_var), momentum,
                    S(st));
  });
  m.def("maxpool_bwd_bnb_rows", [geom](int N, int H, int W, int C, int OH, int OW, int ph, int pw, int sh, int sw,
                                       int padh, int padw) {
    return maxpool_bwd_bnb_rows(geom(N, H, W, C, OH, OW, ph, pw, sh, sw, padh, padw));
  });
  m.def("maxpool_bwd_bnb", [geom](uintptr_t dy, uintptr_t idx, uintptr_t ypool, uintptr_t x, uintptr_t mean,
                                  uintptr_t istd, uintptr_t dx, int N, int H, int W, int C, int OH, int OW, int ph,
                                  int pw, int sh, int sw, int padh, int padw, uintptr_t slab, uintptr_t zero_sums,
                                  uintptr_t st) {
    maxpool_bwd_bnb(P<const bf16*>(dy), P<const uint8_t*>(idx), P<const bf16*>(ypool), P<const bf16*>(x),
                    P<const float*>(mean), P<const float*>(istd), P<bf16*>(dx),
                    geom(N, H, W, C, OH, OW, ph, pw, sh, sw, padh, padw), P<float*>(slab), P<float*>(zero_sums), S(st));
  });
  m.def("avgpool_fwd", [geom](int dt, uintptr_t x, uintptr_t y, int N, int H, int W, int C, int OH, int OW, int ph,
                              int pw, int sh, int sw, int padh, int padw, uintptr_t st) {
    avgpool_fwd(dt, P<const void*>(x), P<void*>(y), geom(N, H, W, C, OH, OW, ph, pw, sh, sw, padh, padw), S(st));
  });
  m.def("avgpool_bwd", [geom](int dt, uintptr_t dy, uintptr_t dx, int N, int H, int W, int C, int OH, int OW, int ph,
                              int pw, int sh, int sw, int padh, int padw, uintptr_t st) {
    avgpool_bwd(dt, P<const void*>(dy), P<void*>(dx), geom(N, H, W, C, OH, OW, ph, pw, sh, sw, padh, padw), S(st));
  });
  m.def("act_fwd", [](int dt, uintptr_t x, uintptr_t y, long n, int type, float a, uintptr_t st) {
    act_fwd(dt, P<const void*>(x), P<void*>(y), n, type, a, S(st));
  });
  m.def("act_bwd", [](int dt, uintptr_t x, uintptr_t dy, uintptr_t dx, long n, int type, float a, uintptr_t st) {
    act_bwd(dt, P<const void*>(x), P<const void*>(dy), P<void*>(dx), n, type, a, S(st));
  });
  m.def("softmax_rows", [](int dt, uintptr_t x, uintptr_t y, long rows, int C, uintptr_t st) {
    softmax_rows(dt, P<const void*>(x), P<void*>(y), rows, C, S(st));
  });
  m.def("softmax_rows_bwd", [](int dt, uintptr_t y, uintptr_t dy, uintptr_t dx, long rows, int C, uintptr_t st) {
    softmax_rows_bwd(dt, P<const void*>(y), P<const void*>(dy), P<void*>(dx), rows, C, S(st));
  });
  m.def("dropout", [](int dt, uintptr_t x, uintptr_t y, long n, float p, uint64_t seed, uintptr_t ctr, uintptr_t st) {
    dropout(dt, P<const void*>(x), P<void*>(y), n, p, seed, P<const uint64_t*>(ctr), S(st));
  });
  m.def("counter_bump", [](uintptr_t ctr, uintptr_t slot, uintptr_t st) {
    counter_bump(P<uint64_t*>(ctr), P<uint64_t*>(slot), S(st));
  });
  m.def("nchw_to_nhwc", [](int dt, uintptr_t x, uintptr_t y, int N, int C, int HW, uintptr_t st) {
    nchw_to_nhwc(dt, P<const float*>(x), P<void*>(y), N, C, HW, S(st));
  });
  m.def("nchw_to_nhwc_pad", [](int dt, uintptr_t x, uintptr_t y, int N, int C, int Cp, int HW, uintptr_t st) {
    nchw_to_nhwc_pad(dt, P<const float*>(x), P<void*>(y), N, C, Cp, HW, S(st));
  });
  m.def("conv_weight_transpose", [](int dt, uintptr_t w, uintptr_t wt, int Co, int T_, int Ci, uintptr_t st) {
    conv_weight_transpose(dt, P<const void*>(w), P<bf16*>(wt), Co, T_, Ci, S(st));
  });
  m.def("multi_splitk_reduce", [](std::vector<std::array<int64_t, 4>> ents, uintptr_t st) {
    for (size_t b = 0; b < ents.size(); b += kMaxRed) {
      MultiRed t{};
      t.count = (int)std::min(ents.size() - b, (size_t)kMaxRed);
      for (int k = 0; k < t.count; ++k) {
        const auto& e = ents[b + k];
        t.e[k].slab = P<const float*>((uintptr_t)e[0]); t.e[k].out = P<float*>((uintptr_t)e[1]);
        t.e[k].n = e[2]; t.e[k].splits = (int)e[3];
      }
      multi_splitk_reduce(t, S(st));
    }
  });
  m.def("multi_red_max", []() { return kMaxRed; });
  m.def("stem_supported", &stem_supported);
  m.def("stem_tiles", &stem_tiles_host);
  m.def("stem_wgrad_blocks", &stem_wgrad_blocks);
  m.def("stem_fwd", [](uintptr_t x, uintptr_t w, int w_bf16, std::array<long, 4> ws, uintptr_t bias, uintptr_t y,
                       uintptr_t slab, uintptr_t zero_ptr, int zero_n, int N, int Ci, int H, int W, int Co,
                       uintptr_t st) {
    StemArgs a{};
    a.x = P<const float*>(x); a.w = P<const void*>(w); a.w_bf16 = w_bf16;
    for (int i = 0; i < 4; ++i) a.ws[i] = ws[i];
    a.bias = P<const float*>(bias); a.y = P<bf16*>(y); a.slab = P<float*>(slab);
    a.zero_ptr = P<float*>(zero_ptr); a.zero_n = zero_n;
    a.N = N; a.Ci = Ci; a.H = H; a.W = W; a.Co = Co;
    stem_fwd(a, S(st));
  });
  m.def("stem_wgrad", [](uintptr_t x, uintptr_t dy, uintptr_t slab, uintptr_t bias_slab, std::array<long, 4> gs,
                         int N, int Ci, int H, int W, int Co, int blocks, uintptr_t st) {
    StemArgs a{};
    a.x = P<const float*>(x); a.dy = P<const bf16*>(dy); a.slab = P<float*>(slab);
    a.bias_slab = P<float*>(bias_slab);
    for (int i = 0; i < 4; ++i) a.gs[i] = gs[i];
    a.n_slab = (long)Co * Ci * 9;
    a.N = N; a.Ci = Ci; a.H = H; a.W = W; a.Co = Co;
    stem_wgrad(a, blocks, S(st));
  });
  m.def("multi_weight_transpose", [](uintptr_t table, int n, long max_tiles, uintptr_t st, int f32) {
    multi_weight_transpose(P<const int64_t*>(table), n, max_tiles, S(st), f32);
  });
  m.def("cast_f32_bf16",[](uintptr_t x, uintptr_t y, long n, uintptr_t st) {
    cast_f32_bf16(P<const float*>(x), P<bf16*>(y), n, S(st));
  });
  m.def("im2col_nhwc", [](int dt, uintptr_t x, uintptr_t col, int N, int H, int W, int C, int OH, int OW, int KH, int KW,
                          int SH, int SW, int PH, int PW, uintptr_t st) {
    im2col_nhwc(dt, P<const void*>(x), P<void*>(col), ConvGeom{N, H, W, C, OH, OW, KH, KW, SH, SW, PH, PW}, S(st));
  });
  m.def("col2im_nhwc", [](int dt, uintptr_t col, uintptr_t x, uintptr_t residual, int N, int H, int W, int C, int OH,
                          int OW, int KH, int KW, int SH, int SW, int PH, int PW, int chan_major, uintptr_t st) {
    col2im_nhwc(dt, P<const void*>(col), P<void*>(x), P<const void*>(residual),
                ConvGeom{N, H, W, C, OH, OW, KH, KW, SH, SW, PH, PW}, chan_major, S(st));
  });
  m.def("im2col", [](uintptr_t x, uintptr_t col, int N, int C, int H, int W, int KH, int KW, int SH, int SW, int PH,
                     int PW, int OH, int OW, uintptr_t st) {
    im2col(P<const float*>(x), P<float*>(col), N, C, H, W, KH, KW, SH, SW, PH, PW, OH, OW, S(st));
  });
  m.def("col2im", [](uintptr_t col, uintptr_t x, int N, int C, int H, int W, int KH, int KW, int SH, int SW, int PH,
                     int PW, int OH, int OW, uintptr_t st) {
    col2im(P<const float*>(col), P<float*>(x), N, C, H, W, KH, KW, SH, SW, PH, PW, OH, OW, S(st));
  });
  m.def("loss_workspace_floats", &loss_workspace_floats);
  m.def("loss_fused", [](int dt, uintptr_t pred, uintptr_t target, uintptr_t labels, uintptr_t grad, uintptr_t loss,
                         uintptr_t correct, int N, int C, int type, float param, float gscale, uintptr_t ws,
                         uintptr_t ticket, uintptr_t st) {
    loss_fused(dt, P<const void*>(pred), P<const float*>(target), P<const int64_t*>(labels), P<void*>(grad),
               P<float*>(loss), P<int*>(correct), N, C, type, param, gscale, P<float*>(ws), P<unsigned*>(ticket),
               S(st));
  });
  m.def("adam_step", [](uintptr_t p, uintptr_t g, uintptr_t mm, uintptr_t v, uintptr_t shadow, long n, float lr,
                        float b1, float b2, float eps, float bc1, float bc2, float wd, int dec, uintptr_t hyper,
                        uintptr_t st) {
    adam_step(P<float*>(p), P<const float*>(g), P<float*>(mm), P<float*>(v), P<bf16*>(shadow), n, lr, b1, b2, eps, bc1,
              bc2, wd, dec, P<const float*>(hyper), S(st));
  });
  m.def("adam_scalars", [](uintptr_t hyper, float b1, float b2, uintptr_t st) {
    adam_scalars(P<float*>(hyper), b1, b2, S(st));
  });
  m.def("sgd_step", [](uintptr_t p, uintptr_t g, uintptr_t vel, uintptr_t shadow, long n, float lr, float mom,
                       uintptr_t hyper, uintptr_t st) {
    sgd_step(P<float*>(p), P<const float*>(g), P<float*>(vel), P<bf16*>(shadow), n, lr, mom, P<const float*>(hyper),
             S(st));
  });
  m.def("zero_bytes", [](uintptr_t p, long nbytes, uintptr_t st) { zero_bytes(P<void*>(p), nbytes, S(st)); });
  m.def("grad_pack_bf16", [](uintptr_t g, uintptr_t out, long n, float scale, uintptr_t st) {
    grad_pack_bf16(P<const float*>(g), P<bf16*>(out), n, scale, S(st));
  });
  m.def("grad_sum_chunks_bf16", [](uintptr_t src, int w, long ld, long n, uintptr_t dst, uintptr_t st) {
    grad_sum_chunks_bf16(P<const bf16*>(src), w, ld, n, P<bf16*>(dst), S(st));
  });
// ... 26 lines not shown
```

### dcnn_amd/csrc/kernels/norm.hip

```cpp
#include <cstdlib>
#include <type_traits>

#include "common.h"
#include "api.h"

namespace dcnn {

template <typename T, int V>
struct VecIO;
template <>
struct VecIO<bf16, 8> {
  __device__ static __forceinline__ void load(const bf16* p, float* f) {
    unpack8(*reinterpret_cast<const uint4*>(p), f);
  }
  __device__ static __forceinline__ void store(bf16* p, const float* f) {
    *reinterpret_cast<uint4*>(p) = pack8(f);
  }
};
template <>
struct VecIO<float, 8> {
  __device__ static __forceinline__ void load(const float* p, float* f) {
    const float4 a = reinterpret_cast<const float4*>(p)[0], b = reinterpret_cast<const float4*>(p)[1];
    f[0] = a.x; f[1] = a.y; f[2] = a.z; f[3] = a.w; f[4] = b.x; f[5] = b.y; f[6] = b.z; f[7] = b.w;
  }
// ... 230 lines not shown
__global__ void __launch_bounds__(256) bn_apply_kernel(const T* __restrict__ x, T* __restrict__ y, long R, int C,
                                                       const float* __restrict__ sums, int parts, float count,
                                                       const float* __restrict__ gamma,
                                                       const float* __restrict__ beta, float eps,
                                                       const T* __restrict__ residual, int relu,
                                                       float* __restrict__ save_mean, float* __restrict__ save_istd,
                                                       float* __restrict__ run_mean, float* __restrict__ run_var,
                                                       float momentum, int use_running) {
  extern __shared__ __attribute__((aligned(16))) float sh[];
  float* scale = sh;
  float* shift = sh + C;
  for (int c = threadIdx.x; c < C; c += blockDim.x) {
    float mean, istd;
    if (use_running) {
      mean = run_mean[c];
      istd = rsqrtf(run_var[c] + eps);
    } else {
      float var;
      read_stats<0>(sums, parts, C, c, mean, var);
      istd = rsqrtf(var + eps);
      if (blockIdx.x == 0) {
        if (save_mean) { save_mean[c] = mean; save_istd[c] = istd; }
        if (run_mean) {
          const float unbiased = count > 1.f ? var * count / (count - 1.f) : var;
          run_mean[c] = (1.f - momentum) * run_mean[c] + momentum * mean;
          run_var[c] = (1.f - momentum) * run_var[c] + momentum * unbiased;
        }
      }
    }
    const float g = gamma ? gamma[c] : 1.f, b = beta ? beta[c] : 0.f;
    scale[c] = g * istd;
    shift[c] = b - mean * g * istd;
  }
  __syncthreads();
  const long nv = R * C / V;
  for (long i = blockIdx.x * (long)blockDim.x + threadIdx.x; i < nv; i += (long)gridDim.x * blockDim.x) {
    const long o = i * V;
    const int c0 = (int)(o % C);
    float xv[V];
    vload<T, V>(x + o, xv);
    float r[V];
    if (residual) vload<T, V>(residual + o, r);
#pragma unroll
    for (int v = 0; v < V; ++v) {
      float t = xv[v] * scale[c0 + v] + shift[c0 + v];
      if (residual) t += r[v];
      if (relu) t = fmaxf(t, 0.f);
      xv[v] = t;
    }
    vstore<T, V>(y + o, xv);
  }
}

template <int P>
__global__ void __launch_bounds__(256) bn_relu_maxpool_kernel(const bf16* __restrict__ x, bf16* __restrict__ y,
                                                              uint8_t* __restrict__ idx, PoolGeom g,
                                                              const float* __restrict__ sums, int parts,
                                                              float count, const float* __restrict__ gamma,
                                                              const float* __restrict__ beta, float eps,
                                                              float* __restrict__ save_mean,
                                                              float* __restrict__ save_istd,
                                                              float* __restrict__ run_mean,
                                                              float* __restrict__ run_var, float momentum) {
  extern __shared__ __attribute__((aligned(16))) float sh[];
  float* scale = sh;
  float* shift = sh + g.C;
  for (int c = threadIdx.x; c < g.C; c += blockDim.x) {
    float mean, var;
    read_stats<0>(sums, parts, g.C, c, mean, var);
    const float istd = rsqrtf(var + eps);
    if (blockIdx.x == 0) {
      if (save_mean) { save_mean[c] = mean; save_istd[c] = istd; }
      if (run_mean) {
        const float unbiased = count > 1.f ? var * count / (count - 1.f) : var;
        run_mean[c] = (1.f - momentum) * run_mean[c] + momentum * mean;
        run_var[c] = (1.f - momentum) * run_var[c] + momentum * unbiased;
      }
    }
    const float gm = gamma ? gamma[c] : 1.f, b = beta ? beta[c] : 0.f;
    scale[c] = gm * istd;
    shift[c] = b - mean * gm * istd;
  }
  __syncthreads();
  const int CV = g.C / 8;
  const long total = (long)g.N * g.OH * g.OW * CV;
  const bool small = total < (1l << 32);
  for (long i = blockIdx.x * (long)blockDim.x + threadIdx.x; i < total; i += (long)gridDim.x * blockDim.x) {
    int cv, ox, oy, n;
    if (small) {
      const unsigned iu = (unsigned)i;
      unsigned t = iu / (unsigned)CV;
      cv = (int)(iu - t * (unsigned)CV);
      ox = (int)(t % (unsigned)g.OW);
      t /= (unsigned)g.OW;
      oy = (int)(t % (unsigned)g.OH);
      n = (int)(t / (unsigned)g.OH);
    } else {
      cv = (int)(i % CV);
      long t = i / CV;
      ox = (int)(t % g.OW);
      t /= g.OW;
      oy = (int)(t % g.OH);
      n = (int)(t / g.OH);
    }
    float sc[8], sf[8], best[8], v[8];
    uint8_t bi[8];
#pragma unroll
    for (int e = 0; e < 8; ++e) { sc[e] = scale[cv * 8 + e]; sf[e] = shift[cv * 8 + e]; best[e] = -INFINITY; bi[e] = 0; }
    auto take = [&](const uint4& raw, int local) {
      unpack8(raw, v);
#pragma unroll
      for (int e = 0; e < 8; ++e) {
        const float r = (float)(bf16)fmaxf(v[e] * sc[e] + sf[e], 0.f);
        if (r > best[e]) { best[e] = r; bi[e] = (uint8_t)local; }
      }
    };
    if constexpr (P > 0) {
      uint4 w[P * P];
#pragma unroll
      for (int ky = 0; ky < P; ++ky)
#pragma unroll
        for (int kx = 0; kx < P; ++kx)
          w[ky * P + kx] = *reinterpret_cast<const uint4*>(
              x + (((long)n * g.H + oy * P + ky) * g.W + ox * P + kx) * g.C + cv * 8);
#pragma unroll
      for (int k = 0; k < P * P; ++k) take(w[k], k);
    } else {
      for (int ky = 0; ky < g.ph; ++ky)
        for (int kx = 0; kx < g.pw; ++kx) {
          const int iy = oy * g.ph + ky, ix = ox * g.pw + kx;
          take(*reinterpret_cast<const uint4*>(x + (((long)n * g.H + iy) * g.W + ix) * g.C + cv * 8), ky * g.pw + kx);
        }
    }
    *reinterpret_cast<uint4*>(y + i * 8) = pack8(best);
    *reinterpret_cast<uint2*>(idx + i * 8) = *reinterpret_cast<uint2*>(bi);
  }
}

template <typename T, int V>
__global__ void __launch_bounds__(256) bn_bwd_apply_kernel(const T* __restrict__ dy, const T* __restrict__ yout,
                                                           const T* __restrict__ x, T* __restrict__ dx, long R,
                                                           int C, const float* __restrict__ mean,
                                                           const float* __restrict__ istd,
                                                           const float* __restrict__ gamma,
                                                           const float* __restrict__ sums, int parts,
                                                           float count, float* __restrict__ dgamma,
                                                           float* __restrict__ dbeta, int eval_mode) {
  extern __shared__ __attribute__((aligned(16))) float sh[];
  float* ca = sh;
  float* cb = sh + C;
  float* cc = sh + 2 * C;
  float* cm = sh + 3 * C;
  float* ci = sh + 4 * C;
  for (int c = threadIdx.x; c < C; c += blockDim.x) {
    const float g = gamma ? gamma[c] : 1.f;
    float sdy = 0.f, sdyx = 0.f;
    if (sums) read_stats<1>(sums, parts, C, c, sdy, sdyx);
    ca[c] = g * istd[c];
    cb[c] = eval_mode ? 0.f : sdy / count;
    cc[c] = eval_mode ? 0.f : sdyx / count;
    cm[c] = mean[c];
    ci[c] = istd[c];
    if (blockIdx.x == 0 && sums) {
      if (dgamma) dgamma[c] += sdyx;
      if (dbeta) dbeta[c] += sdy;
    }
  }
  __syncthreads();
  const long nv = R * C / V;
  for (long i = blockIdx.x * (long)blockDim.x + threadIdx.x; i < nv; i += (long)gridDim.x * blockDim.x) {
    const long o = i * V;
    const int c0 = (int)(o % C);
    float d[V], xv[V];
    vload<T, V>(dy + o, d);
    vload<T, V>(x + o, xv);
    if (yout) {
      float yo[V];
      vload<T, V>(yout + o, yo);
#pragma unroll
      for (int v = 0; v < V; ++v) d[v] = yo[v] > 0.f ? d[v] : 0.f;
    }
#pragma unroll
    for (int v = 0; v < V; ++v) {
      const int c = c0 + v;
      const float xh = (xv[v] - cm[c]) * ci[c];
      d[v] = ca[c] * (d[v] - cb[c] - xh * cc[c]);
    }
    vstore<T, V>(dx + o, d);
// ... 613 lines not shown
    hipLaunchKernelGGL((bn_partial_kernel<T, 1>), dim3(blocks), dim3(256), shm, s, x, dy, yout, dy_out, mean,
                       istd, R, C, rpb, slab, mode, zs);
  }
  DCNN_LAUNCH_CHECK();
}

void bn_partial(int dtype, const void* x, const void* dy, const void* yout, void* dy_out, const float* mean,
                const float* istd, long R, int C, float* slab, int mode, float* zero_sums, hipStream_t s) {
  if (dtype == 0)
    bn_partial_t<float>((const float*)x, (const float*)dy, (const float*)yout, (float*)dy_out, mean, istd, R, C,
                        slab, mode, zero_sums, s);
  else
    bn_partial_t<bf16>((const bf16*)x, (const bf16*)dy, (const bf16*)yout, (bf16*)dy_out, mean, istd, R, C, slab,
                       mode, zero_sums, s);
}

int bn_stat_parts(int rows) {
  const int per = g_stat_waves * kStatRW;
  return (rows + per - 1) / per;
}

void bn_stat_reduce2(int mode, const float* slab, int rows, float* out, float* part, const float* slab2, int rows2,
                     float* out2, float* part2, int C, hipStream_t s) {
  const int ny = bn_stat_parts(rows), ny2 = slab2 ? bn_stat_parts(rows2) : 0;
  if ((ny > 1 && !part) || (ny2 > 1 && !part2)) throw std::runtime_error("bn_stat_reduce: partials buffer required");
  const dim3 grid((unsigned)((C + 63) / 64), (unsigned)(ny > ny2 ? ny : ny2), slab2 ? 2u : 1u);
#define DCNN_SR(W)                                                                                           \
  if (g_stat_waves == W) {                                                                                   \
    if (mode == 0)                                                                                           \
      hipLaunchKernelGGL((bn_stat_reduce_kernel<0, W>), grid, dim3(64 * W), 0, s, slab, rows, C, part, nullptr, out, \
                         ny, slab2, rows2, part2, out2, ny2);                                                \
    else                                                                                                     \
      hipLaunchKernelGGL((bn_stat_reduce_kernel<1, W>), grid, dim3(64 * W), 0, s, slab, rows, C, part, nullptr, out, \
                         ny, slab2, rows2, part2, out2, ny2);                                                \
  }
  DCNN_SR(4) DCNN_SR(8) DCNN_SR(16)
#undef DCNN_SR
  DCNN_LAUNCH_CHECK();
}

void bn_stat_reduce(int mode, const float* slab, int rows, int C, float* out, float* part, unsigned* ticket,
                    hipStream_t s) {
  (void)ticket;
  bn_stat_reduce2(mode, slab, rows, out, part, nullptr, 0, nullptr, nullptr, C, s);
}

bool bn_relu_maxpool_supported(PoolGeom g) {
  return g.C % 8 == 0 && g.ph == g.sh && g.pw == g.sw && g.padh == 0 && g.padw == 0 && g.ph * g.pw <= 255 &&
         g.OH == g.H / g.ph && g.OW == g.W / g.pw;
}

void bn_relu_maxpool(const bf16* x, bf16* y, uint8_t* idx, PoolGeom g, const float* sums, int parts, float count,
                     const float* gamma, const float* beta, float eps, float* save_mean, float* save_istd,
                     float* run_mean, float* run_var, float momentum, hipStream_t s) {
  if (!bn_relu_maxpool_supported(g)) throw std::runtime_error("bn_relu_maxpool: unsupported geometry");
  const long total = (long)g.N * g.OH * g.OW * g.C / 8;
  auto k = (g.ph == 2 && g.pw == 2) ? bn_relu_maxpool_kernel<2> : bn_relu_maxpool_kernel<0>;
  hipLaunchKernelGGL(k, dim3(grid_for(total, 256, 2048)), dim3(256), 2 * g.C * sizeof(float), s,
                     x, y, idx, g, sums, parts, count, gamma, beta, eps, save_mean, save_istd, run_mean, run_var,
                     momentum);
  DCNN_LAUNCH_CHECK();
}

template <typename T>
static void bn_apply_t(const T* x, T* y, long R, int C, const float* sums, int parts, float count, const float* gamma,
                       const float* beta, float eps, const T* residual, int relu, float* save_mean,
                       float* save_istd, float* run_mean, float* run_var, float momentum, int use_running,
                       hipStream_t s) {
  const size_t shm = 2 * C * sizeof(float);
  if (bn_v_ok(R, C)) {
    int U, g;
    const unsigned nv = (unsigned)(R * C / 8);
    bn_v_launch_shape(nv, C, &U, &g);
#define DCNN_BNV(U_, RES_)                                                                                       \
  if (U == U_ && (residual != nullptr) == RES_)                                                                  \
    hipLaunchKernelGGL((bn_apply_v_kernel<T, U_, RES_>), dim3(g), dim3(256), shm, s, x, y, nv, C, sums, parts, count, \
                       gamma, beta, eps, residual, relu, save_mean, save_istd, run_mean, run_var, momentum, use_running);
    DCNN_BNV(1, false) DCNN_BNV(2, false) DCNN_BNV(4, false) DCNN_BNV(1, true) DCNN_BNV(2, true) DCNN_BNV(4, true)
#undef DCNN_BNV
    DCNN_LAUNCH_CHECK();
    return;
  }
  if (C % 8 == 0) {
    const int g = grid_for(R * C / 8, 256, 2048);
    hipLaunchKernelGGL((bn_apply_kernel<T, 8>), dim3(g), dim3(256), shm, s, x, y, R, C, sums, parts, count, gamma, beta,
                       eps, residual, relu, save_mean, save_istd, run_mean, run_var, momentum, use_running);
  } else {
    const int g = grid_for(R * C, 256, 2048);
    hipLaunchKernelGGL((bn_apply_kernel<T, 1>), dim3(g), dim3(256), shm, s, x, y, R, C, sums, parts, count, gamma, beta,
                       eps, residual, relu, save_mean, save_istd, run_mean, run_var, momentum, use_running);
  }
  DCNN_LAUNCH_CHECK();
}

void bn_apply(int dtype, const void* x, void* y, long R, int C, const float* sums, int parts, float count,
              const float* gamma, const float* beta, float eps, const void* residual, int relu, float* save_mean,
              float* save_istd, float* run_mean, float* run_var, float momentum, int use_running, hipStream_t s) {
  if (dtype == 0)
    bn_apply_t<float>((const float*)x, (float*)y, R, C, sums, parts, count, gamma, beta, eps, (const float*)residual,
                      relu, save_mean, save_istd, run_mean, run_var, momentum, use_running, s);
  else
    bn_apply_t<bf16>((const bf16*)x, (bf16*)y, R, C, sums, parts, count, gamma, beta, eps, (const bf16*)residual,
                     relu, save_mean, save_istd, run_mean, run_var, momentum, use_running, s);
}

template <typename T>
static void bn_bwd_apply_t(const T* dy, const T* yout, const T* x, T* dx, long R, int C, const float* mean,
                           const float* istd, const float* gamma, const float* sums, int parts, float count,
                           float* dgamma, float* dbeta, int eval_mode, hipStream_t s) {
  if (bn_v_ok(R, C)) {
    int U, g;
    const unsigned nv = (unsigned)(R * C / 8);
// ... 63 lines not shown
```

### dcnn_amd/csrc/kernels/pool_act.hip

```cpp
#include "common.h"
#include "api.h"

namespace dcnn {

template <typename T>
__device__ __forceinline__ float ld(const T* p, long i) { return to_f(p[i]); }



template <typename T>
__global__ void maxpool_fwd_kernel(const T* __restrict__ x, T* __restrict__ y, uint8_t* __restrict__ idx, PoolGeom g) {
  const long total = (long)g.N * g.OH * g.OW * g.C;
  for (long i = blockIdx.x * (long)blockDim.x + threadIdx.x; i < total; i += (long)gridDim.x * blockDim.x) {
    const int c = (int)(i % g.C);
    long t = i / g.C;
    const int ox = (int)(t % g.OW);
    t /= g.OW;
    const int oy = (int)(t % g.OH);
    const int n = (int)(t / g.OH);
    float best = -INFINITY;
    int bi = 0;
    for (int ky = 0; ky < g.ph; ++ky) {
      const int iy = oy * g.sh - g.padh + ky;
      if (iy < 0 || iy >= g.H) continue;
// ... 166 lines not shown
      const int iy = oy * g.sh - g.padh + ky;
      if (iy < 0 || iy >= g.H) continue;
      for (int kx = 0; kx < g.pw; ++kx) {
        const int ix = ox * g.sw - g.padw + kx;
        if (ix < 0 || ix >= g.W) continue;
        unpack8(*reinterpret_cast<const uint4*>(x + ((size_t)(n * g.H + iy) * g.W + ix) * g.C + cv * 8), v);
#pragma unroll
        for (int e = 0; e < 8; ++e)
          if (v[e] > best[e]) { best[e] = v[e]; bi[e] = (uint8_t)(ky * g.pw + kx); }
      }
    }
    *reinterpret_cast<uint4*>(y + (size_t)i * 8) = pack8(best);
    *reinterpret_cast<uint2*>(idx + (size_t)i * 8) = *reinterpret_cast<uint2*>(bi);
  }
}

__global__ void __launch_bounds__(256) maxpool_bwd_ov8_kernel(const bf16* __restrict__ dy,
                                                              const uint8_t* __restrict__ idx, bf16* __restrict__ dx,
                                                              PoolGeom g) {
  const int CV = g.C >> 3;
  const int total = g.N * g.H * g.W * CV;
  for (int i = blockIdx.x * blockDim.x + threadIdx.x; i < total; i += gridDim.x * blockDim.x) {
    const int cv = i % CV;
    int t = i / CV;
    const int ix = t % g.W;
    t /= g.W;
    const int iy = t % g.H, n = t / g.H;
    const int oy0 = max(0, (iy + g.padh - g.ph + g.sh) / g.sh), oy1 = min(g.OH - 1, (iy + g.padh) / g.sh);
    const int ox0 = max(0, (ix + g.padw - g.pw + g.sw) / g.sw), ox1 = min(g.OW - 1, (ix + g.padw) / g.sw);
    float acc[8];
#pragma unroll
    for (int e = 0; e < 8; ++e) acc[e] = 0.f;
    for (int oy = oy0; oy <= oy1; ++oy) {
      const int ky = iy - (oy * g.sh - g.padh);
      if (ky < 0 || ky >= g.ph) continue;
      for (int ox = ox0; ox <= ox1; ++ox) {
        const int kx = ix - (ox * g.sw - g.padw);
        if (kx < 0 || kx >= g.pw) continue;
        const size_t o = ((size_t)(n * g.OH + oy) * g.OW + ox) * g.C + cv * 8;
        const uint2 ib = *reinterpret_cast<const uint2*>(idx + o);
        const uint8_t* b = reinterpret_cast<const uint8_t*>(&ib);
        const int local = ky * g.pw + kx;
        float d[8];
        unpack8(*reinterpret_cast<const uint4*>(dy + o), d);
#pragma unroll
        for (int e = 0; e < 8; ++e)
          if (b[e] == local) acc[e] += d[e];
      }
    }
    *reinterpret_cast<uint4*>(dx + (size_t)i * 8) = pack8(acc);
  }
}

__global__ void __launch_bounds__(256) maxpool_bwd_bnb_kernel(const bf16* __restrict__ dy,
                                                              const uint8_t* __restrict__ idx,
                                                              const bf16* __restrict__ ypool,
                                                              const bf16* __restrict__ x,
                                                              const float* __restrict__ mean,
                                                              const float* __restrict__ istd, bf16* __restrict__ dx,
                                                              PoolGeom g, float* __restrict__ slab,
                                                              float* __restrict__ zero_sums) {
  __shared__ float red[256 * 16];
  if (zero_sums && blockIdx.x == 0)
    for (int j = threadIdx.x; j < 2 * g.C; j += blockDim.x) zero_sums[j] = 0.f;
  const int CV = g.C / 8;
  const long total = (long)g.N * g.H * g.W * CV;
  const int cv = threadIdx.x % CV;
  float mu[8], is[8], s[8], q[8];
#pragma unroll
  for (int e = 0; e < 8; ++e) {
    mu[e] = mean[cv * 8 + e];
    is[e] = istd[cv * 8 + e];
    s[e] = q[e] = 0.f;
  }
  for (long i = blockIdx.x * (long)blockDim.x + threadIdx.x; i < total; i += (long)gridDim.x * blockDim.x) {
    long t = i / CV;
    const int ix = (int)(t % g.W);
    t /= g.W;
    const int iy = (int)(t % g.H);
    const int n = (int)(t / g.H);
    const int oy = iy / g.ph, ox = ix / g.pw;
    float out[8];
    if (oy < g.OH && ox < g.OW) {
      const long o = (((long)n * g.OH + oy) * g.OW + ox) * g.C + cv * 8;
      const int local = (iy - oy * g.ph) * g.pw + (ix - ox * g.pw);
      float d[8], yp[8], xv[8];
      unpack8(*reinterpret_cast<const uint4*>(dy + o), d);
      unpack8(*reinterpret_cast<const uint4*>(ypool + o), yp);
      unpack8(*reinterpret_cast<const uint4*>(x + i * 8), xv);
      const uint2 ib = *reinterpret_cast<const uint2*>(idx + o);
      const uint8_t* b = reinterpret_cast<const uint8_t*>(&ib);
#pragma unroll
      for (int e = 0; e < 8; ++e) {
        out[e] = (b[e] == local && yp[e] > 0.f) ? d[e] : 0.f;
        s[e] += out[e];
        q[e] += out[e] * (xv[e] - mu[e]) * is[e];
      }
    } else {
#pragma unroll
      for (int e = 0; e < 8; ++e) out[e] = 0.f;
    }
    *reinterpret_cast<uint4*>(dx + i * 8) = pack8(out);
  }
#pragma unroll
  for (int e = 0; e < 8; ++e) {
    red[threadIdx.x * 16 + e] = s[e];
// ... 359 lines not shown
    if (pool_nov4f(g)) {
      const long total = (long)g.N * g.H * g.W * g.C / 4;
      hipLaunchKernelGGL(maxpool_bwd_nov4f_kernel, dim3(grid_for(total, 256)), dim3(256), 0, s, (const float*)dy, idx,
                         (float*)dx, g);
      DCNN_LAUNCH_CHECK();
      return;
    }
  }
  if constexpr (std::is_same<T, bf16>::value) {
    if (pool_nov8(g)) {
      const long total = (long)g.N * g.H * g.W * g.C / 8;
      hipLaunchKernelGGL(maxpool_bwd_nov8_kernel, dim3(grid_for(total, 256)), dim3(256), 0, s, (const bf16*)dy, idx,
                         (bf16*)dx, g);
      DCNN_LAUNCH_CHECK();
      return;
    }
  }
  if constexpr (std::is_same<T, bf16>::value) {
    if (pool_ov8(g)) {
      const long total = (long)g.N * g.H * g.W * g.C / 8;
      hipLaunchKernelGGL(maxpool_bwd_ov8_kernel, dim3(grid_for(total, 256)), dim3(256), 0, s, (const bf16*)dy, idx,
                         (bf16*)dx, g);
      DCNN_LAUNCH_CHECK();
      return;
    }
  }
  const long total = (long)g.N * g.H * g.W * g.C;
  hipLaunchKernelGGL(maxpool_bwd_kernel<T>, dim3(grid_for(total, 256)), dim3(256), 0, s, (const T*)dy, idx, (T*)dx, g);
  DCNN_LAUNCH_CHECK();
}
template <typename T>
static void avgpool_fwd_t(const void* x, void* y, PoolGeom g, hipStream_t s) {
  if (g.OH == 1 && g.OW == 1 && g.ph == g.H && g.pw == g.W && g.padh == 0 && g.padw == 0) {
    const long total = (long)g.N * g.C;
    hipLaunchKernelGGL(global_avgpool_fwd_kernel<T>, dim3(grid_for(total, 256)), dim3(256), 0, s, (const T*)x, (T*)y,
                       g.N, g.H * g.W, g.C);
  } else {
    const long total = (long)g.N * g.OH * g.OW * g.C;
    hipLaunchKernelGGL(avgpool_fwd_kernel<T>, dim3(grid_for(total, 256)), dim3(256), 0, s, (const T*)x, (T*)y, g);
  }
  DCNN_LAUNCH_CHECK();
}
template <typename T>
static void avgpool_bwd_t(const void* dy, void* dx, PoolGeom g, hipStream_t s) {
  const long total = (long)g.N * g.H * g.W * g.C;
  if (g.OH == 1 && g.OW == 1 && g.ph == g.H && g.pw == g.W && g.padh == 0 && g.padw == 0)
    hipLaunchKernelGGL(global_avgpool_bwd_kernel<T>, dim3(grid_for(total, 256)), dim3(256), 0, s, (const T*)dy, (T*)dx,
                       g.N, g.H * g.W, g.C);
  else
    hipLaunchKernelGGL(avgpool_bwd_kernel<T>, dim3(grid_for(total, 256)), dim3(256), 0, s, (const T*)dy, (T*)dx, g);
  DCNN_LAUNCH_CHECK();
}

template <int P>
__global__ void __launch_bounds__(256) maxpool_bwd_bnb_w_kernel(const bf16* __restrict__ dy,
                                                                const uint8_t* __restrict__ idx,
                                                                const bf16* __restrict__ ypool,
                                                                const bf16* __restrict__ x,
                                                                const float* __restrict__ mean,
                                                                const float* __restrict__ istd,
                                                                bf16* __restrict__ dx, PoolGeom g,
                                                                float* __restrict__ slab,
                                                                float* __restrict__ zero_sums) {
  __shared__ float red[256 * 16];
  if (zero_sums && blockIdx.x == 0)
    for (int j = threadIdx.x; j < 2 * g.C; j += blockDim.x) zero_sums[j] = 0.f;
  const unsigned CV = g.C / 8;
  const unsigned total = (unsigned)g.N * g.OH * g.OW * CV;
  const int cv = threadIdx.x % CV;
  float mu[8], is[8], s[8], q[8];
#pragma unroll
  for (int e = 0; e < 8; ++e) {
    mu[e] = mean[cv * 8 + e];
    is[e] = istd[cv * 8 + e];
    s[e] = q[e] = 0.f;
  }
  for (unsigned i = blockIdx.x * 256u + threadIdx.x; i < total; i += gridDim.x * 256u) {
    unsigned t = i / CV;
    const int ox = (int)(t % g.OW);
    t /= g.OW;
    const int oy = (int)(t % g.OH);
    const int n = (int)(t / g.OH);
    float d[8], yp[8];
    unpack8(*reinterpret_cast<const uint4*>(dy + (size_t)i * 8), d);
    unpack8(*reinterpret_cast<const uint4*>(ypool + (size_t)i * 8), yp);
    const uint2 ib = *reinterpret_cast<const uint2*>(idx + (size_t)i * 8);
    const uint8_t* b = reinterpret_cast<const uint8_t*>(&ib);
    auto put = [&](const uint4& raw, int local, size_t xi) {
      float xv[8], out[8];
      unpack8(raw, xv);
#pragma unroll
      for (int e = 0; e < 8; ++e) {
        out[e] = (b[e] == local && yp[e] > 0.f) ? d[e] : 0.f;
        s[e] += out[e];
        q[e] += out[e] * (xv[e] - mu[e]) * is[e];
      }
      *reinterpret_cast<uint4*>(dx + xi) = pack8(out);
    };
    if constexpr (P > 0) {
      size_t xi[P * P];
      uint4 w[P * P];
#pragma unroll
      for (int ky = 0; ky < P; ++ky)
#pragma unroll
        for (int kx = 0; kx < P; ++kx) {
          xi[ky * P + kx] = (((size_t)n * g.H + oy * P + ky) * g.W + ox * P + kx) * g.C + cv * 8;
          w[ky * P + kx] = *reinterpret_cast<const uint4*>(x + xi[ky * P + kx]);
        }
#pragma unroll
      for (int k = 0; k < P * P; ++k) put(w[k], k, xi[k]);
    } else {
      for (int ky = 0; ky < g.ph; ++ky)
        for (int kx = 0; kx < g.pw; ++kx) {
          const size_t xi = (((size_t)n * g.H + oy * g.ph + ky) * g.W + ox * g.pw + kx) * g.C + cv * 8;
          put(*reinterpret_cast<const uint4*>(x + xi), ky * g.pw + kx, xi);
        }
    }
  }
#pragma unroll
  for (int e = 0; e < 8; ++e) {
    red[threadIdx.x * 16 + e] = s[e];
    red[threadIdx.x * 16 + 8 + e] = q[e];
  }
  __syncthreads();
  for (int j = threadIdx.x; j < 2 * g.C; j += blockDim.x) {
    const int which = j / g.C, c = j % g.C, grp = c / 8, e = c % 8;
    float a = 0.f;
    for (int tt = grp; tt < (int)blockDim.x; tt += CV) a += red[tt * 16 + which * 8 + e];
    slab[((long)blockIdx.x * 2 + which) * g.C + c] = a;
  }
}

static int bnb_pool_blocks(const PoolGeom& g) {
  const long total = (long)g.N * g.H * g.W * g.C / 8;
  return grid_for(total, 256, 1024);
}

bool maxpool_bwd_bnb_supported(PoolGeom g) { return pool_nov8(g) && 256 % (g.C / 8) == 0; }

int maxpool_bwd_bnb_rows(PoolGeom g) { return bnb_pool_blocks(g); }

void maxpool_bwd_bnb(const bf16* dy, const uint8_t* idx, const bf16* ypool, const bf16* x, const float* mean,
                     const float* istd, bf16* dx, PoolGeom g, float* slab, float* zero_sums, hipStream_t s) {
  if (!maxpool_bwd_bnb_supported(g)) throw std::runtime_error("maxpool_bwd_bnb: unsupported geometry");
  if (g.H % g.ph == 0 && g.W % g.pw == 0 && g.OH == g.H / g.ph && g.OW == g.W / g.pw &&
      (long)g.N * g.H * g.W * g.C < (1l << 31)) {
    hipLaunchKernelGGL((g.ph == 2 && g.pw == 2) ? maxpool_bwd_bnb_w_kernel<2> : maxpool_bwd_bnb_w_kernel<0>,
                       dim3(bnb_pool_blocks(g)), dim3(256), 0, s, dy, idx, ypool, x, mean,
                       istd, dx, g, slab, zero_sums);
    DCNN_LAUNCH_CHECK();
    return;
  }
  hipLaunchKernelGGL(maxpool_bwd_bnb_kernel, dim3(bnb_pool_blocks(g)), dim3(256), 0, s, dy, idx, ypool, x, mean, istd,
                     dx, g, slab, zero_sums);
  DCNN_LAUNCH_CHECK();
}

void maxpool_fwd(int dt, const void* x, void* y, uint8_t* idx, PoolGeom g, hipStream_t s) { DCNN_DT(dt, maxpool_fwd_t, x, y, idx, g, s); }
void maxpool_bwd(int dt, const void* dy, const uint8_t* idx, void* dx, PoolGeom g, hipStream_t s) { DCNN_DT(dt, maxpool_bwd_t, dy, idx, dx, g, s); }
void avgpool_fwd(int dt, const void* x, void* y, PoolGeom g, hipStream_t s) { DCNN_DT(dt, avgpool_fwd_t, x, y, g, s); }
void avgpool_bwd(int dt, const void* dy, void* dx, PoolGeom g, hipStream_t s) { DCNN_DT(dt, avgpool_bwd_t, dy, dx, g, s); }

template <typename T>
static void act_fwd_t(const void* x, void* y, long n, int type, float a, hipStream_t s) {
  hipLaunchKernelGGL(act_fwd_kernel<T>, dim3(grid_for(n / 8 + 1, 256)), dim3(256), 0, s, (const T*)x, (T*)y, n, type, a);
  DCNN_LAUNCH_CHECK();
}
template <typename T>
static void act_bwd_t(const void* x, const void* dy, void* dx, long n, int type, float a, hipStream_t s) {
  hipLaunchKernelGGL(act_bwd_kernel<T>, dim3(grid_for(n, 256)), dim3(256), 0, s, (const T*)x, (const T*)dy, (T*)dx, n,
                     type, a);
  DCNN_LAUNCH_CHECK();
}
template <typename T>
static void softmax_t(const void* x, void* y, long rows, int C, hipStream_t s) {
  hipLaunchKernelGGL(softmax_rows_kernel<T>, dim3((rows * 64 + 255) / 256), dim3(256), 0, s, (const T*)x, (T*)y, rows, C);
  DCNN_LAUNCH_CHECK();
}
template <typename T>
static void softmax_bwd_t(const void* y, const void* dy, void* dx, long rows, int C, hipStream_t s) {
  hipLaunchKernelGGL(softmax_rows_bwd_kernel<T>, dim3((rows * 64 + 255) / 256), dim3(256), 0, s, (const T*)y,
                     (const T*)dy, (T*)dx, rows, C);
  DCNN_LAUNCH_CHECK();
}
template <typename T>
static void dropout_t(const void* x, void* y, long n, float p, uint64_t seed, const uint64_t* ctr, hipStream_t s) {
  hipLaunchKernelGGL(dropout_kernel<T>, dim3(grid_for((n + 3) / 4, 256)), dim3(256), 0, s, (const T*)x, (T*)y, n, p, seed,
                     ctr);
  DCNN_LAUNCH_CHECK();
}
template <typename T>
static void nchw_to_nhwc_t(const float* x, void* y, int N, int C, int HW, hipStream_t s) {
  hipLaunchKernelGGL(nchw_to_nhwc_kernel<T>, dim3(grid_for((long)N * C * HW, 256)), dim3(256), 0, s, x, (T*)y, N, C, HW);
  DCNN_LAUNCH_CHECK();
}
template <typename T>
static void nchw_to_nhwc_pad_t(const float* x, void* y, int N, int C, int Cp, int HW, hipStream_t s) {
  hipLaunchKernelGGL(nchw_to_nhwc_pad_kernel<T>, dim3(grid_for((long)N * Cp * HW, 256)), dim3(256), 0, s, x, (T*)y, N, C,
                     Cp, HW);
  DCNN_LAUNCH_CHECK();
}
template <typename T>
static void wt_t(const void* w, bf16* wt, int Co, int T_, int Ci, hipStream_t s) {
  hipLaunchKernelGGL(conv_weight_transpose_kernel<T>, dim3(grid_for((long)Co * T_ * Ci, 256)), dim3(256), 0, s,
                     (const T*)w, wt, Co, T_, Ci);
  DCNN_LAUNCH_CHECK();
}

void act_fwd(int dt, const void* x, void* y, long n, int type, float a, hipStream_t s) { DCNN_DT(dt, act_fwd_t, x, y, n, type, a, s); }
void act_bwd(int dt, const void* x, const void* dy, void* dx, long n, int type, float a, hipStream_t s) { DCNN_DT(dt, act_bwd_t, x, dy, dx, n, type, a, s); }
// ... 33 lines not shown
```

### dcnn_amd/csrc/kernels/stem.hip

```cpp
#include "common.h"
#include "api.h"

namespace dcnn {

namespace {
constexpr int SPX = 512;
constexpr int HALO_MAX = 6 * 130 * 4;

__device__ __forceinline__ int stem_tiles(const StemArgs& p) { return p.N * (p.H / p.TH); }

__device__ __forceinline__ void stage_halo(const StemArgs& p, int tile, bf16* hs) {
  constexpr int J = 3;
  const int tpi = p.H / p.TH, n = tile / tpi, y0 = (tile - n * tpi) * p.TH;
  const int HW2 = p.W + 2, rows = p.TH + 2, w4 = p.W >> 2, per_c = rows * w4, total = p.Ci * per_c;
  float4 v[J];
#pragma unroll
  for (int j = 0; j < J; ++j) {
    const int i = threadIdx.x + j * 256;
    const int c = i / per_c, r = i - c * per_c, hy = r / w4, x4 = r - hy * w4;
    const int y = y0 + hy - 1;
    v[j] = make_float4(0.f, 0.f, 0.f, 0.f);
    if (i < total && (unsigned)y < (unsigned)p.H)
      v[j] = *reinterpret_cast<const float4*>(p.x + (((long)n * p.Ci + c) * p.H + y) * p.W + x4 * 4);
  }
  for (int i = threadIdx.x; i < (4 - p.Ci) * rows * HW2; i += 256) {
    const int c = p.Ci + i / (rows * HW2), r = i % (rows * HW2);
    hs[r * 4 + c] = (bf16)0.f;
  }
  for (int i = threadIdx.x; i < p.Ci * rows * 2; i += 256) {
    const int c = i / (rows * 2), r = i % (rows * 2), hy = r >> 1;
    hs[(hy * HW2 + (r & 1) * (HW2 - 1)) * 4 + c] = (bf16)0.f;
  }
#pragma unroll
  for (int j = 0; j < J; ++j) {
    const int i = threadIdx.x + j * 256;
    const int c = i / per_c, r = i - c * per_c, hy = r / w4, x4 = r - hy * w4;
    if (i < total) {
      bf16* d = hs + (hy * HW2 + 1 + x4 * 4) * 4 + c;
      d[0] = (bf16)v[j].x; d[4] = (bf16)v[j].y; d[8] = (bf16)v[j].z; d[12] = (bf16)v[j].w;
    }
  }
}

__device__ __forceinline__ float wval(const StemArgs& p, int co, int tap, int ch) {
  if (ch >= p.Ci || tap > 8) return 0.f;
  const long o = co * p.ws[0] + ch * p.ws[1] + (tap / 3) * p.ws[2] + (tap % 3) * p.ws[3];
  return p.w_bf16 ? (float)reinterpret_cast<const bf16*>(p.w)[o] : reinterpret_cast<const float*>(p.w)[o];
}

__device__ __forceinline__ bf16x8 cat44(bf16x4 lo, bf16x4 hi) {
  return bf16x8{lo[0], lo[1], lo[2], lo[3], hi[0], hi[1], hi[2], hi[3]};
}
}

template <int NCB>
__global__ void __launch_bounds__(256, NCB <= 2 ? 8 : 4) stem_fwd_kernel(StemArgs p) {
  constexpr int CO = NCB * 16;
  __shared__ __attribute__((aligned(16))) bf16 halo[HALO_MAX];
  __shared__ __attribute__((aligned(16))) bf16 stg[4][16 * CO];
  __shared__ float red[4][3][CO];
  const int lane = threadIdx.x & 63, wid = threadIdx.x >> 6, kg = lane >> 4, col = lane & 15;
  const int tile = blockIdx.x;
  if (p.zero_ptr && tile == 0)
    for (int i = threadIdx.x; i < p.zero_n; i += 256) p.zero_ptr[i] = 0.f;
  stage_halo(p, tile, halo);

  bf16x8 b0[NCB], b1[NCB];
  float bias[NCB];
#pragma unroll
  for (int cb = 0; cb < NCB; ++cb) {
    const int co = cb * 16 + col;
#pragma unroll
    for (int e = 0; e < 8; ++e) {
      b0[cb][e] = (bf16)wval(p, co, 2 * kg + (e >> 2), e & 3);
      b1[cb][e] = (bf16)(kg == 0 ? wval(p, co, 8, e & 3) * (e < 4) : 0.f);
    }
    bias[cb] = p.bias ? p.bias[co] : 0.f;
  }
  __syncthreads();

  const int HW2 = p.W + 2;
  const int tpi = p.H / p.TH, n = tile / tpi, y0 = (tile - n * tpi) * p.TH;
  const int t0 = 2 * kg, t1 = 2 * kg + 1;
  const int o0 = (t0 / 3) * HW2 + t0 % 3, o1 = (t1 / 3) * HW2 + t1 % 3, o8 = 2 * HW2 + 2;
  float s[NCB], q[NCB], piv[NCB];
#pragma unroll
  for (int cb = 0; cb < NCB; ++cb) s[cb] = q[cb] = piv[cb] = 0.f;
  bool first = true;
  const bf16x4 z4 = bf16x4{(bf16)0.f, (bf16)0.f, (bf16)0.f, (bf16)0.f};
  for (int g = wid; g < SPX / 16; g += 4) {
    const int px = g * 16 + col, py = px / p.W, pxx = px - py * p.W;
    const int hp = py * HW2 + pxx;
    const bf16x4* h4 = reinterpret_cast<const bf16x4*>(halo);
    const bf16x8 a0 = cat44(h4[hp + o0], h4[hp + o1]);
    const bf16x8 a1 = cat44(kg == 0 ? h4[hp + o8] : z4, z4);
#pragma unroll
    for (int cb = 0; cb < NCB; ++cb) {
      f32x4 acc = __builtin_amdgcn_mfma_f32_16x16x32_bf16(a0, b0[cb], f32x4{0.f, 0.f, 0.f, 0.f}, 0, 0, 0);
      acc = __builtin_amdgcn_mfma_f32_16x16x32_bf16(a1, b1[cb], acc, 0, 0, 0);
      if (first) piv[cb] = __shfl((float)(bf16)(acc[0] + bias[cb]), col, 64);
#pragma unroll
      for (int r = 0; r < 4; ++r) {
        const bf16 v = (bf16)(acc[r] + bias[cb]);
        const float f = (float)v - piv[cb];
        s[cb] += f;
        q[cb] += f * f;
        stg[wid][(kg * 4 + r) * CO + cb * 16 + col] = v;
      }
    }
    first = false;
    asm volatile("s_waitcnt lgkmcnt(0)" ::: "memory");
    __builtin_amdgcn_wave_barrier();
    const long obase = (((long)n * p.H + y0) * p.W + g * 16) * CO;
    for (int c = lane; c < 2 * CO; c += 64)
      reinterpret_cast<uint4*>(p.y + obase)[c] = reinterpret_cast<const uint4*>(stg[wid])[c];
    asm volatile("s_waitcnt lgkmcnt(0)" ::: "memory");
    __builtin_amdgcn_wave_barrier();
  }
  if (!p.slab) return;
#pragma unroll
  for (int cb = 0; cb < NCB; ++cb) {
    s[cb] += __shfl_xor(s[cb], 16);
    s[cb] += __shfl_xor(s[cb], 32);
    q[cb] += __shfl_xor(q[cb], 16);
    q[cb] += __shfl_xor(q[cb], 32);
    if (kg == 0) {
      red[wid][0][cb * 16 + col] = s[cb];
      red[wid][1][cb * 16 + col] = q[cb];
      red[wid][2][cb * 16 + col] = piv[cb];
    }
  }
  __syncthreads();
  for (int c = threadIdx.x; c < CO; c += 256) {
    Welford t{0.f, 0.f, 0.f};
#pragma unroll
    for (int w = 0; w < 4; ++w) {
      const int ng = w < SPX / 16 ? (SPX / 16 - 1 - w) / 4 + 1 : 0;
      t = welford_merge(t, welford_from_shifted((float)(ng * 16), red[w][2][c], red[w][0][c], red[w][1][c]));
    }
    store_welford(p.slab, tile, CO, c, t);
  }
}

template <int NCB, bool BNT>
__global__ void __launch_bounds__(256, NCB <= 2 ? (BNT ? 3 : 4) : 2) stem_wgrad_kernel(StemArgs p) {
  constexpr int CO = NCB * 16;
  extern __shared__ __attribute__((aligned(16))) char smem[];
  bf16* halo = reinterpret_cast<bf16*>(smem);
  bf16* dys = reinterpret_cast<bf16*>(smem + p.halo_bytes);
  const int lane = threadIdx.x & 63, wid = threadIdx.x >> 6, kg = lane >> 4, col = lane & 15;
  const int HW2 = p.W + 2;
  const int ntile = stem_tiles(p);
  const i32x4 rs_dy = raw_rsrc(p.dy, (unsigned)((long)p.N * p.H * p.W * CO * 2));
  float* coef = reinterpret_cast<float*>(smem + p.halo_bytes + SPX * CO * 2);
  if constexpr (BNT) {
    for (int c = threadIdx.x; c < CO; c += 256) {
      float sdy, sdyx;
      if (p.bn_parts <= 1) {
        sdy = p.bn_sums[c];
        sdyx = p.bn_sums[CO + c];
      } else {
        sdy = p.bn_sums[c];
        sdyx = p.bn_sums[CO + c];
        for (int q = 1; q < p.bn_parts; ++q) {
          sdy += p.bn_sums[(long)q * 3 * CO + c];
          sdyx += p.bn_sums[(long)q * 3 * CO + CO + c];
        }
      }
      const float is = p.bn_istd[c], a = (p.bn_gamma ? p.bn_gamma[c] : 1.f) * is;
      coef[c] = a;
      coef[CO + c] = p.bn_eval ? 0.f : -a * is * (sdyx / p.bn_count);
      coef[2 * CO + c] = p.bn_mean[c];
      coef[3 * CO + c] = p.bn_eval ? 0.f : -a * (sdy / p.bn_count);
      if (blockIdx.x == 0) {
        if (p.bn_dgamma) p.bn_dgamma[c] += sdyx;
        if (p.bn_dbeta) p.bn_dbeta[c] += sdy;
      }
    }
  }
  constexpr int NVT = SPX * CO / 8 / 256;
  f32x4 acc[NCB][3];
#pragma unroll
  for (int cb = 0; cb < NCB; ++cb)
#pragma unroll
    for (int nb = 0; nb < 3; ++nb) acc[cb][nb] = f32x4{0.f, 0.f, 0.f, 0.f};
  int koff[3];
  bool kval[3], kone[3];
#pragma unroll
  for (int nb = 0; nb < 3; ++nb) {
    const int k = nb * 16 + col, tap = k >> 2, ch = k & 3;
    kval[nb] = k < 36 && ch < p.Ci;
    kone[nb] = k == 36;
    koff[nb] = ((tap < 9 ? (tap / 3) * HW2 + tap % 3 : 0) * 4) + ch;
  }
  for (int tile = blockIdx.x; tile < ntile; tile += gridDim.x) {
    __syncthreads();
    const int tpi = p.H / p.TH, n = tile / tpi, y0 = (tile - n * tpi) * p.TH;
    const unsigned src = (unsigned)((((long)n * p.H + y0) * p.W) * CO * 2);
#pragma unroll
    for (int j = 0; j < SPX * CO * 2 / 1024 / 4; ++j) {
      const int blk = wid * (SPX * CO * 2 / 1024 / 4) + j;
      glds16_opaque(rs_dy, reinterpret_cast<char*>(dys) + blk * 1024, src + blk * 1024 + lane * 16);
    }
    stage_halo(p, tile, halo);
    uint4 xv[BNT ? NVT : 1];
    if constexpr (BNT) {
      const char* xb = reinterpret_cast<const char*>(p.bn_x) + src;
#pragma unroll
      for (int j = 0; j < NVT; ++j) xv[j] = *reinterpret_cast<const uint4*>(xb + (threadIdx.x + j * 256) * 16);
    }
    asm volatile("s_waitcnt vmcnt(0)" ::: "memory");
    __syncthreads();
    if constexpr (BNT) {
      {
        constexpr int j0 = 0, RV = NVT;
#pragma unroll
        for (int j = 0; j < RV; ++j) {
          const int v = threadIdx.x + (j0 + j) * 256;
          int c0 = (v % (CO / 8)) * 8;
          asm volatile("" : "+v"(c0));
          uint4* q = reinterpret_cast<uint4*>(dys) + v;
          float d[8], xf[8];
          unpack8(*q, d);
          unpack8(xv[j], xf);
#pragma unroll
          for (int e = 0; e < 8; ++e)
            d[e] = coef[c0 + e] * d[e] + coef[CO + c0 + e] * (xf[e] - coef[2 * CO + c0 + e]) + coef[3 * CO + c0 + e];
          *q = pack8(d);
        }
      }
      __syncthreads();
    }
    for (int ks = wid; ks < SPX / 32; ks += 4) {
      const int p0 = ks * 32 + kg * 8, py = p0 / p.W, px0 = p0 - py * p.W;
      bf16x8 a[NCB], b[3];
#pragma unroll
      for (int cb = 0; cb < NCB; ++cb)
#pragma unroll
        for (int e = 0; e < 8; ++e) a[cb][e] = dys[(p0 + e) * CO + cb * 16 + col];
      const int hb = (py * HW2 + px0) * 4;
#pragma unroll
      for (int nb = 0; nb < 3; ++nb)
#pragma unroll
        for (int e = 0; e < 8; ++e)
          b[nb][e] = kval[nb] ? halo[hb + e * 4 + koff[nb]] : (bf16)(kone[nb] ? 1.f : 0.f);
#pragma unroll
      for (int cb = 0; cb < NCB; ++cb)
#pragma unroll
        for (int nb = 0; nb < 3; ++nb) acc[cb][nb] = __builtin_amdgcn_mfma_f32_16x16x32_bf16(a[cb], b[nb], acc[cb][nb], 0, 0, 0);
    }
  }
  __syncthreads();
  float* red = reinterpret_cast<float*>(smem);
#pragma unroll
  for (int cb = 0; cb < NCB; ++cb)
#pragma unroll
    for (int nb = 0; nb < 3; ++nb)
#pragma unroll
      for (int r = 0; r < 4; ++r) red[(wid * CO + cb * 16 + kg * 4 + r) * 48 + nb * 16 + col] = acc[cb][nb][r];
  __syncthreads();
  float* out = p.slab + (long)blockIdx.x * p.n_slab;
  for (int i = threadIdx.x; i < CO * 37; i += 256) {
    const int co = i / 37, k = i - co * 37, tap = k >> 2, ch = k & 3;
    const float v = red[(0 * CO + co) * 48 + k] + red[(1 * CO + co) * 48 + k] + red[(2 * CO + co) * 48 + k] +
                    red[(3 * CO + co) * 48 + k];
    if (k == 36) {
      if (p.bias_slab) p.bias_slab[(long)blockIdx.x * CO + co] = v;
    } else if (ch < p.Ci) {
      out[co * p.gs[0] + ch * p.gs[1] + (tap / 3) * p.gs[2] + (tap % 3) * p.gs[3]] = v;
    }
  }
}

bool stem_supported(int N, int Ci, int H, int W, int Co) {
  if (Ci < 1 || Ci > 4 || Co % 16 || Co > 64 || W % 16 || SPX % W) return false;
  const int th = SPX / W;
  if (H % th || (th + 2) * (W + 2) * 4 > HALO_MAX || Ci * (th + 2) * (W / 4) > 3 * 256) return false;
  return N > 0 && (long)N * Ci * H * W < (1l << 31);
}

int stem_tiles_host(int N, int H, int W) { return N * (H / (SPX / W)); }

int stem_wgrad_blocks(int N, int H, int W) {
  const int t = stem_tiles_host(N, H, W);
  return t < 1024 ? t : 1024;
}

int stem_wgrad_blocks_bnt(int N, int H, int W) {
  static const int forced = [] {
    const char* e = std::getenv("DCNN_STEM_BNT_BLOCKS");
    return e ? std::atoi(e) : 0;
  }();
  int dev = 0, cus = 256;
  if (hipGetDevice(&dev) == hipSuccess) hipDeviceGetAttribute(&cus, hipDeviceAttributeMultiprocessorCount, dev);
  const int t = stem_tiles_host(N, H, W), want = forced > 0 ? forced : 3 * cus;
  return t < want ? t : want;
}

void stem_fwd(StemArgs a, hipStream_t s) {
  if (!stem_supported(a.N, a.Ci, a.H, a.W, a.Co)) throw std::runtime_error("stem_fwd: unsupported shape");
  a.TH = SPX / a.W;
  const int grid = stem_tiles_host(a.N, a.H, a.W);
  switch (a.Co / 16) {
    case 1: hipLaunchKernelGGL(stem_fwd_kernel<1>, dim3(grid), dim3(256), 0, s, a); break;
    case 2: hipLaunchKernelGGL(stem_fwd_kernel<2>, dim3(grid), dim3(256), 0, s, a); break;
    case 3: hipLaunchKernelGGL(stem_fwd_kernel<3>, dim3(grid), dim3(256), 0, s, a); break;
    default: hipLaunchKernelGGL(stem_fwd_kernel<4>, dim3(grid), dim3(256), 0, s, a); break;
  }
  DCNN_LAUNCH_CHECK();
}

void stem_wgrad(StemArgs a, int blocks, hipStream_t s) {
  if (!stem_supported(a.N, a.Ci, a.H, a.W, a.Co)) throw std::runtime_error("stem_wgrad: unsupported shape");
  if (blocks < 1 || blocks > stem_tiles_host(a.N, a.H, a.W)) throw std::runtime_error("stem_wgrad: bad block count");
  a.TH = SPX / a.W;
  a.halo_bytes = (((a.TH + 2) * (a.W + 2) * 8) + 15) / 16 * 16;
  const bool bnt = a.bn_x != nullptr;
  if (bnt && (!a.bn_mean || !a.bn_istd || !a.bn_sums || a.bn_parts < 1 || a.bn_count <= 0.f))
    throw std::runtime_error("stem_wgrad: incomplete BatchNorm-backward operands");
  const int main = a.halo_bytes + SPX * a.Co * 2 + (bnt ? 4 * a.Co * 4 : 0), epi = 4 * a.Co * 48 * 4;
  const int lds = main > epi ? main : epi;
#define DCNN_SW(C)                                                                                        \
  {                                                                                                       \
    auto k = bnt ? stem_wgrad_kernel<C, true> : stem_wgrad_kernel<C, false>;                              \
    DCNN_HIP_CHECK(hipFuncSetAttribute((const void*)k, hipFuncAttributeMaxDynamicSharedMemorySize, lds)); \
    hipLaunchKernelGGL(k, dim3(blocks), dim3(256), lds, s, a);                                            \
  }
  switch (a.Co / 16) {
    case 1: DCNN_SW(1) break;
    case 2: DCNN_SW(2) break;
    case 3: DCNN_SW(3) break;
    default: DCNN_SW(4) break;
  }
#undef DCNN_SW
  DCNN_LAUNCH_CHECK();
}

}
```

Before: 91290 images/sec.

## Fold stem max-pool backward into stem BN-fused weight-gradient kernel

Backward through the stem's max-pool no longer writes the full-resolution input gradient. A sums-only kernel computes the BatchNorm backward statistics from a forward-saved selected-x tensor. The stem wgrad kernel then recomputes the unpooled, BN-adjusted gradient on the fly from the pooled dy, argmax indices and pooled output. This removes a full-size bf16 gradient write and read, at the cost of an extra xsel buffer in forward, gathered loads in the wgrad kernel, and more complex host gating. It is on by default and can be disabled with environment variables.

```diff
diff --git a/dcnn_amd/csrc/host/dcnn/nn.hpp b/dcnn_amd/csrc/host/dcnn/nn.hpp
--- a/dcnn_amd/csrc/host/dcnn/nn.hpp
+++ b/dcnn_amd/csrc/host/dcnn/nn.hpp
@@ -115,7 +115,7 @@
   void set_block_bnb_producer(class BatchNorm* bn) { bnb_block_from_ = bn; }
   bool backward_residual(const Tensor& dy, const Tensor& residual, Tensor& dx) override;
   bool ran_stem() const;
-  void backward_stem_bn(const Tensor& dy, const gpu_ops::StemBn& bn);
+  void backward_stem_bn(const Tensor& dy, const gpu_ops::StemBn& bn, const gpu_ops::StemPool* pool = nullptr);
   void sync_shadow() override;
   bool make_transposed_operand(std::vector<int64_t>& row, long& tiles);
 
@@ -197,6 +197,12 @@
     pending_rows_ = rows;
   }
   bool backward_into_stem(const Tensor& dy, Conv2D& stem);
+  bool stem_fold_ready(const Conv2D& stem);
+  void set_stem_xsel(bool b) { stem_xsel_ = b; }
+  void offer_bwd_stats_pooled(const void* dy, const float* slab, int rows, const gpu_ops::StemPool& pool) {
+    offer_bwd_stats(dy, slab, rows);
+    bwd_pool_ = pool;
+  }
   Tensor running_mean, running_var;
 
  private:
@@ -205,6 +211,7 @@
   bool affine_;
   bool train_ = true;
   bool fused_relu_ = false;
+  bool stem_xsel_ = false;
   Tensor forward_impl(const Tensor& x, bool training, const Tensor* residual, bool relu);
   Tensor apply_deferred(bool training);
   class Pool2D* fused_pool_ = nullptr;
@@ -212,6 +219,7 @@
   const void* bwd_dy_ = nullptr;
   const float* bwd_slab_ = nullptr;
   int bwd_rows_ = 0;
+  gpu_ops::StemPool bwd_pool_{};
   const void* pending_x_ = nullptr;
   const float* pending_slab_ = nullptr;
   int pending_rows_ = 0;
@@ -227,6 +235,7 @@
   Tensor backward(const Tensor& dy) override;
   bool is_relu() const;
   void set_passthrough(bool b) { passthrough_ = b; }
+  bool passthrough() const { return passthrough_; }
 
  private:
   std::string kind_;
@@ -278,8 +287,12 @@
   bool is_max() const { return max_; }
   PoolShape shape_for(const std::vector<int64_t>& in) const;
   void set_fused_producer(class BatchNorm* bn) { bn_ = bn; }
+  class BatchNorm* fused_producer() const { return bn_; }
+  bool stem_pooled_ok();
+  Tensor backward_stem_pooled(const Tensor& dy);
   uint8_t* accept_prepooled(const Tensor& ypool, const std::vector<int64_t>& in);
   void clear_prepooled() { mbc().flag = false; }
+  void* prepooled_xsel(bool want);
 
  private:
   class BatchNorm* bn_ = nullptr;
diff --git a/dcnn_amd/csrc/host/dcnn/ops.hpp b/dcnn_amd/csrc/host/dcnn/ops.hpp
--- a/dcnn_amd/csrc/host/dcnn/ops.hpp
+++ b/dcnn_amd/csrc/host/dcnn/ops.hpp
@@ -98,6 +98,13 @@
   bool train;
 };
 void stem_wgrad_bn(const void* dy, const float* x, float* gw, float* gb, const ConvShape& s, const StemBn& bn);
+struct StemPool {
+  const void* dy;
+  const uint8_t* idx;
+  const void* ypool;
+};
+void stem_wgrad_bn_pool(const StemPool& pool, const float* x, float* gw, float* gb, const ConvShape& s,
+                        const StemBn& bn);
 void dense_fwd(const void* x, const void* w, const float* bias, void* y, int N, int In, int Out);
 void dense_dgrad(const void* dy, const void* w, void* dx, int N, int In, int Out);
 void dense_wgrad(const void* dy, const void* x, float* gw, float* gb, int N, int In, int Out);
@@ -148,9 +155,12 @@
 bool bn_relu_maxpool_ok(const PoolShape& p);
 void bn_relu_maxpool(const void* x, void* y, uint8_t* idx, const PoolShape& p, const float* slab, int rows,
                      const float* g, const float* b, float eps, float* rmean, float* rvar, float momentum,
-                     float* smean, float* sistd);
+                     float* smean, float* sistd, void* xsel = nullptr);
 const float* maxpool_bwd_bnb(const void* dy, const uint8_t* idx, const void* ypool, const void* x, const float* mean,
                              const float* istd, void* dx, const PoolShape& p, int* rows);
+bool maxpool_bwd_bnb_sums_ok(const PoolShape& p);
+const float* maxpool_bwd_bnb_sums(const void* dy, const uint8_t* idx, const void* ypool, const void* xsel,
+                                  const float* mean, const float* istd, const PoolShape& p, int* rows);
 void maxpool_fwd(const void* x, void* y, uint8_t* idx, const PoolShape& p);
 void maxpool_bwd(const void* dy, const uint8_t* idx, void* dx, const PoolShape& p);
 void avgpool_fwd(const void* x, void* y, const PoolShape& p);
diff --git a/dcnn_amd/csrc/host/nn.cpp b/dcnn_amd/csrc/host/nn.cpp
--- a/dcnn_amd/csrc/host/nn.cpp
+++ b/dcnn_amd/csrc/host/nn.cpp
@@ -201,6 +201,15 @@
   return p;
 }
 
+static bool stem_recompute_env() {
+  static const bool on = [] {
+    const char* v = std::getenv("DCNN_STEM_RECOMPUTE");
+    const char* f = std::getenv("DCNN_STEM_BN_FOLD");
+    return !(v && std::string(v) == "0") && !(f && std::string(f) == "0");
+  }();
+  return on;
+}
+
 bool Conv2D::takes_raw_input(const std::vector<int64_t>& in) const {
   return dev_.is_gpu() && in.size() == 4 && in[1] == ci_ && gpu_ops::stem_ok(shape_for(in));
 }
@@ -236,10 +245,13 @@
   return dev_.is_gpu() && x_.defined() && x_.dtype() == DType::F32;
 }
 
-void Conv2D::backward_stem_bn(const Tensor& dy, const gpu_ops::StemBn& bn) {
+void Conv2D::backward_stem_bn(const Tensor& dy, const gpu_ops::StemBn& bn, const gpu_ops::StemPool* pool) {
   const Tensor& x_ = mbc().a;
   const ConvShape s = shape_for(x_.shape());
-  gpu_ops::stem_wgrad_bn(dy.data(), x_.ptr<float>(), params_[0].grad.ptr<float>(), bias_grad(), s, bn);
+  if (pool)
+    gpu_ops::stem_wgrad_bn_pool(*pool, x_.ptr<float>(), params_[0].grad.ptr<float>(), bias_grad(), s, bn);
+  else
+    gpu_ops::stem_wgrad_bn(dy.data(), x_.ptr<float>(), params_[0].grad.ptr<float>(), bias_grad(), s, bn);
 }
 
 Tensor Conv2D::backward(const Tensor& dy) {
@@ -493,9 +505,10 @@
     if (dev_.is_gpu() && training && relu && residual == nullptr && gpu_ops::bn_relu_maxpool_ok(p)) {
       Tensor yp = act_empty({p.N, p.C, p.OH, p.OW}, dev_);
       uint8_t* idx = fused_pool_->accept_prepooled(yp, x.shape());
+      void* xsel = fused_pool_->prepooled_xsel(stem_xsel_ && gpu_ops::maxpool_bwd_bnb_sums_ok(p));
       gpu_ops::bn_relu_maxpool(x.data(), yp.data(), idx, p, slab ? pending_slab_ : nullptr, slab ? pending_rows_ : 0,
                                g, b, eps_, running_mean.ptr<float>(), running_var.ptr<float>(), momentum_,
-                               mean_.ptr<float>(), istd_.ptr<float>());
+                               mean_.ptr<float>(), istd_.ptr<float>(), xsel);
       mc.d = Tensor();
       mc.flag = false;
       pending_x_ = nullptr;
@@ -663,11 +676,20 @@
   return dx;
 }
 
+bool BatchNorm::stem_fold_ready(const Conv2D& stem) {
+  return dev_.is_gpu() && train_ && stem.ran_stem() && mbc().a.defined() && mbc().a.dtype() == DType::BF16;
+}
+
 bool BatchNorm::backward_into_stem(const Tensor& dy, Conv2D& stem) {
   MbCache& mc = mbc();
-  if (!dev_.is_gpu() || !train_ || bwd_dy_ != dy.data() || bwd_slab_ == nullptr || bwd_rows_ <= 0 ||
-      !stem.ran_stem() || mc.a.dtype() != DType::BF16)
+  const bool pooled = bwd_pool_.dy != nullptr;
+  if (bwd_dy_ != dy.data() || bwd_slab_ == nullptr || bwd_rows_ <= 0 || !stem_fold_ready(stem)) {
+    if (pooled) {
+      bwd_pool_ = gpu_ops::StemPool{};
+      throw std::runtime_error(name_ + ": the max-pool backward left its input gradient to the stem fold, which cannot run");
+    }
     return false;
+  }
   gpu_ops::StemBn bn{mc.a.data(),
                      mc.b.ptr<float>(),
                      mc.c.ptr<float>(),
@@ -677,7 +699,9 @@
                      bwd_slab_,
                      bwd_rows_,
                      train_};
-  stem.backward_stem_bn(dy, bn);
+  const gpu_ops::StemPool pool = bwd_pool_;
+  bwd_pool_ = gpu_ops::StemPool{};
+  stem.backward_stem_bn(dy, bn, pooled ? &pool : nullptr);
   bwd_dy_ = nullptr;
   bwd_slab_ = nullptr;
   bwd_rows_ = 0;
@@ -686,6 +710,10 @@
 
 Tensor BatchNorm::backward(const Tensor& dy) {
   MbCache& mc = mbc();
+  if (bwd_pool_.dy != nullptr) {
+    bwd_pool_ = gpu_ops::StemPool{};
+    throw std::runtime_error(name_ + ": backward after a max-pool backward that left its input gradient to the stem fold");
+  }
   const Tensor& x_ = mc.a;
   Tensor& mean_ = mc.b;
   Tensor& istd_ = mc.c;
@@ -1192,6 +1220,33 @@
     cpu_ops::avgpool_fwd(x.ptr<float>(), y.ptr<float>(), p);
   }
   return y;
+}
+
+void* Pool2D::prepooled_xsel(bool want) {
+  MbCache& mc = mbc();
+  if (!want) {
+    mc.c = Tensor();
+    return nullptr;
+  }
+  mc.c = act_empty(mc.b.shape(), dev_);
+  return mc.c.data();
+}
+
+bool Pool2D::stem_pooled_ok() {
+  return dev_.is_gpu() && max_ && bn_ != nullptr && mbc().flag && mbc().b.defined() && mbc().c.defined() &&
+         gpu_ops::maxpool_bwd_bnb_sums_ok(shape_for(mbc().shape));
+}
+
+Tensor Pool2D::backward_stem_pooled(const Tensor& dy) {
+  if (!stem_pooled_ok()) throw std::runtime_error(name_ + ": backward_stem_pooled without a pre-pooled forward");
+  const PoolShape p = shape_for(mbc().shape);
+  const gpu_ops::BnbOperands ops = bn_->bnb_operands(mb_);
+  const uint8_t* idx = mbc().a.ptr<uint8_t>();
+  int rows = 0;
+  const float* slab =
+      gpu_ops::maxpool_bwd_bnb_sums(dy.data(), idx, mbc().b.data(), mbc().c.data(), ops.mean, ops.istd, p, &rows);
+  bn_->offer_bwd_stats_pooled(dy.data(), slab, rows, gpu_ops::StemPool{dy.data(), idx, mbc().b.data()});
+  return dy;
 }
 
 Tensor Pool2D::backward(const Tensor& dy) {
@@ -1451,6 +1506,14 @@
 Tensor Sequential::forward_activation(const Tensor& x_in, int mb) {
   if (!initialized_) throw std::runtime_error("Sequential::forward before initialize()");
   Tensor x = x_in;
+  if (layers_.size() > 3)
+    if (auto* bn = dynamic_cast<BatchNorm*>(layers_[1].get())) {
+      auto* pool = dynamic_cast<Pool2D*>(layers_[3].get());
+      auto* act = dynamic_cast<Activation*>(layers_[2].get());
+      bn->set_stem_xsel(dev_.is_gpu() && training_ && stem_recompute_env() && x.dtype() == DType::F32 &&
+                        layers_[0]->takes_raw_input(x.shape()) && dynamic_cast<Conv2D*>(layers_[0].get()) &&
+                        act && act->passthrough() && pool && pool->fused_producer() == bn);
+    }
   for (auto& l : layers_) {
     l->set_micro_batch(mb);
     x = l->forward(x, training_);
@@ -1470,6 +1533,7 @@
     return !(v && std::string(v) == "0");
   }();
   const bool stem_bn_fold = dev_.is_gpu() && stem_bn_env && layers_.size() > 1;
+  const bool stem_pool_fold = stem_bn_fold && stem_recompute_env();
   if (defer) gpu_ops::begin_deferred_reduce();
   try {
     for (size_t i = layers_.size(); i-- > 0;) {
@@ -1484,6 +1548,21 @@
             if (bwd_hook_) bwd_hook_(0);
             g = Tensor();
             break;
+          }
+        }
+      }
+      if (i == 3 && stem_pool_fold) {
+        auto* pool = dynamic_cast<Pool2D*>(layers_[i].get());
+        auto* bn = dynamic_cast<BatchNorm*>(layers_[1].get());
+        auto* conv = dynamic_cast<Conv2D*>(layers_[0].get());
+        auto* act = dynamic_cast<Activation*>(layers_[2].get());
+        if (pool && bn && conv && act && act->passthrough() && pool->fused_producer() == bn) {
+          bn->set_micro_batch(mb);
+          conv->set_micro_batch(mb);
+          if (bn->stem_fold_ready(*conv) && pool->stem_pooled_ok()) {
+            g = pool->backward_stem_pooled(g);
+            if (bwd_hook_) bwd_hook_(i);
+            continue;
           }
         }
       }
diff --git a/dcnn_amd/csrc/host/ops_gpu.hip b/dcnn_amd/csrc/host/ops_gpu.hip
--- a/dcnn_amd/csrc/host/ops_gpu.hip
+++ b/dcnn_amd/csrc/host/ops_gpu.hip
@@ -739,7 +739,7 @@
 }
 
 static void stem_wgrad_impl(const void* dy, const float* x, float* gw, float* gb, const ConvShape& s,
-                            const StemBn* bn);
+                            const StemBn* bn, const StemPool* pool = nullptr);
 
 void stem_wgrad(const void* dy, const float* x, float* gw, float* gb, const ConvShape& s) {
   stem_wgrad_impl(dy, x, gw, gb, s, nullptr);
@@ -751,9 +751,16 @@
   stem_wgrad_impl(dy, x, gw, gb, s, &bn);
 }
 
+void stem_wgrad_bn_pool(const StemPool& pool, const float* x, float* gw, float* gb, const ConvShape& s,
+                        const StemBn& bn) {
+  if (!pool.dy || !pool.idx || !pool.ypool) throw std::runtime_error("stem_wgrad_bn_pool: incomplete pooled operands");
+  stem_wgrad_impl(nullptr, x, gw, gb, s, &bn, &pool);
+}
+
 static void stem_wgrad_impl(const void* dy, const float* x, float* gw, float* gb, const ConvShape& s,
-                            const StemBn* bn) {
-  rec("stem_wgrad", s, -1, {{"bias", gb != nullptr}, {"deferred", g_defer}, {"bn", bn != nullptr}});
+                            const StemBn* bn, const StemPool* pool) {
+  rec("stem_wgrad", s, -1,
+      {{"bias", gb != nullptr}, {"deferred", g_defer}, {"bn", bn != nullptr}, {"pool", pool != nullptr}});
   std::pair<const float*, int> st{nullptr, 0};
   if (bn) st = reduce_stats(1, bn->slab, bn->rows, s.Co);
   const int blocks = bn ? stem_wgrad_blocks_bnt(s.N, s.H, s.W) : stem_wgrad_blocks(s.N, s.H, s.W);
@@ -769,6 +776,10 @@
       a.bn_sums = st.first; a.bn_parts = st.second; a.bn_count = (float)((long)s.N * s.H * s.W);
       a.bn_dgamma = bn->dgamma; a.bn_dbeta = bn->dbeta; a.bn_eval = bn->train ? 0 : 1;
     }
+    if (pool) {
+      a.pool_dy = static_cast<const bf16*>(pool->dy); a.pool_idx = pool->idx;
+      a.pool_y = static_cast<const bf16*>(pool->ypool);
+    }
     dcnn::stem_wgrad(a, blocks, cur());
   });
 }
@@ -899,7 +910,7 @@
 
 void bn_relu_maxpool(const void* x, void* y, uint8_t* idx, const PoolShape& p, const float* slab, int rows,
                      const float* g, const float* b, float eps, float* rmean, float* rvar, float momentum,
-                     float* smean, float* sistd) {
+                     float* smean, float* sistd, void* xsel) {
   const long R = (long)p.N * p.H * p.W;
   if (slab == nullptr || rows <= 0) {
     rows = bn_partial_rows(R, p.C);
@@ -909,7 +920,7 @@
   }
   const auto st = reduce_stats(0, slab, rows, p.C);
   dcnn::bn_relu_maxpool(static_cast<const bf16*>(x), static_cast<bf16*>(y), idx, geom(p), st.first, st.second,
-                        (float)R, g, b, eps, smean, sistd, rmean, rvar, momentum, cur());
+                        (float)R, g, b, eps, smean, sistd, rmean, rvar, momentum, cur(), static_cast<bf16*>(xsel));
 }
 
 const float* maxpool_bwd_bnb(const void* dy, const uint8_t* idx, const void* ypool, const void* x, const float* mean,
@@ -919,6 +930,18 @@
   float* slab = static_cast<float*>(scratch(BWD_STATS, (size_t)*rows * 2 * p.C * 4));
   dcnn::maxpool_bwd_bnb(static_cast<const bf16*>(dy), idx, static_cast<const bf16*>(ypool),
                         static_cast<const bf16*>(x), mean, istd, static_cast<bf16*>(dx), g, slab, nullptr, cur());
+  return slab;
+}
+
+bool maxpool_bwd_bnb_sums_ok(const PoolShape& p) { return dcnn::maxpool_bwd_bnb_sums_supported(geom(p)); }
+
+const float* maxpool_bwd_bnb_sums(const void* dy, const uint8_t* idx, const void* ypool, const void* xsel,
+                                  const float* mean, const float* istd, const PoolShape& p, int* rows) {
+  const PoolGeom g = geom(p);
+  *rows = maxpool_bwd_bnb_rows(g);
+  float* slab = static_cast<float*>(scratch(BWD_STATS, (size_t)*rows * 2 * p.C * 4));
+  dcnn::maxpool_bwd_bnb_sums(static_cast<const bf16*>(dy), idx, static_cast<const bf16*>(ypool),
+                             static_cast<const bf16*>(xsel), mean, istd, g, slab, nullptr, cur());
   return slab;
 }
 
diff --git a/dcnn_amd/csrc/host/train.cpp b/dcnn_amd/csrc/host/train.cpp
--- a/dcnn_amd/csrc/host/train.cpp
+++ b/dcnn_amd/csrc/host/train.cpp
@@ -572,6 +572,13 @@
 }
 
 Sequential create_model(const std::string& name) {
+  if (name.size() > 5 && name.compare(name.size() - 5, 5, ".json") == 0) {
+    std::ifstream f(name);
+    if (!f) throw std::invalid_argument("cannot read model config '" + name + "'");
+    std::stringstream ss;
+    ss << f.rdbuf();
+    return Sequential::load_from_config(json::Value::parse(ss.str()));
+  }
   if (name == "mnist_cnn")
     return SequentialBuilder("mnist_cnn_model").input({1, 28, 28})
         .conv2d(8, 5, 5, 1, 1, 0, 0, true, "conv1").batchnorm(1e-5f, 0.1f, true, "bn1")
diff --git a/dcnn_amd/csrc/kernels/api.h b/dcnn_amd/csrc/kernels/api.h
--- a/dcnn_amd/csrc/kernels/api.h
+++ b/dcnn_amd/csrc/kernels/api.h
@@ -189,7 +189,7 @@
 bool bn_relu_maxpool_supported(PoolGeom g);
 void bn_relu_maxpool(const bf16* x, bf16* y, uint8_t* idx, PoolGeom g, const float* sums, int parts, float count,
                      const float* gamma, const float* beta, float eps, float* save_mean, float* save_istd,
-                     float* run_mean, float* run_var, float momentum, hipStream_t s);
+                     float* run_mean, float* run_var, float momentum, hipStream_t s, bf16* xsel = nullptr);
 void gn_fwd(int dtype, const void* x, void* y, int N, int HW, int C, int G, const float* gamma, const float* beta,
             float eps, float* save_mean, float* save_istd, hipStream_t s);
 void gn_bwd(int dtype, const void* dy, const void* x, void* dx, int N, int HW, int C, int G, const float* gamma,
@@ -201,6 +201,9 @@
 int maxpool_bwd_bnb_rows(PoolGeom g);
 void maxpool_bwd_bnb(const bf16* dy, const uint8_t* idx, const bf16* ypool, const bf16* x, const float* mean,
                      const float* istd, bf16* dx, PoolGeom g, float* slab, float* zero_sums, hipStream_t s);
+bool maxpool_bwd_bnb_sums_supported(PoolGeom g);
+void maxpool_bwd_bnb_sums(const bf16* dy, const uint8_t* idx, const bf16* ypool, const bf16* xsel, const float* mean,
+                          const float* istd, PoolGeom g, float* slab, float* zero_sums, hipStream_t s);
 void avgpool_fwd(int dt, const void* x, void* y, PoolGeom g, hipStream_t s);
 void avgpool_bwd(int dt, const void* dy, void* dx, PoolGeom g, hipStream_t s);
 void act_fwd(int dt, const void* x, void* y, long n, int type, float a, hipStream_t s);
@@ -220,6 +223,7 @@
   int halo_bytes; int N, Ci, H, W, Co, TH;
   const bf16* bn_x; const float* bn_mean; const float* bn_istd; const float* bn_gamma; const float* bn_sums;
   int bn_parts; float bn_count; float* bn_dgamma; float* bn_dbeta; int bn_eval;
+  const bf16* pool_dy; const uint8_t* pool_idx; const bf16* pool_y;
 };
 bool stem_supported(int N, int Ci, int H, int W, int Co);
 int stem_tiles_host(int N, int H, int W);
diff --git a/dcnn_amd/csrc/kernels/bindings.cpp b/dcnn_amd/csrc/kernels/bindings.cpp
--- a/dcnn_amd/csrc/kernels/bindings.cpp
+++ b/dcnn_amd/csrc/kernels/bindings.cpp
@@ -418,6 +418,17 @@
                     P<float*>(save_mean), P<float*>(save_istd), P<float*>(run_mean), P<float*>(run_var), momentum,
                     S(st));
   });
+  m.def("bn_relu_maxpool_xsel", [geom](uintptr_t x, uintptr_t y, uintptr_t idx, uintptr_t xsel, int N, int H, int W,
+                                       int C, int OH, int OW, int ph, int pw, int sh, int sw, int padh, int padw,
+                                       uintptr_t sums, int parts, float count, uintptr_t gamma, uintptr_t beta,
+                                       float eps, uintptr_t save_mean, uintptr_t save_istd, uintptr_t run_mean,
+                                       uintptr_t run_var, float momentum, uintptr_t st) {
+    if (!xsel) throw std::invalid_argument("bn_relu_maxpool_xsel: xsel is null");
+    bn_relu_maxpool(P<const bf16*>(x), P<bf16*>(y), P<uint8_t*>(idx), geom(N, H, W, C, OH, OW, ph, pw, sh, sw, padh, padw),
+                    P<const float*>(sums), parts, count, P<const float*>(gamma), P<const float*>(beta), eps,
+                    P<float*>(save_mean), P<float*>(save_istd), P<float*>(run_mean), P<float*>(run_var), momentum,
+                    S(st), P<bf16*>(xsel));
+  });
   m.def("maxpool_bwd_bnb_rows", [geom](int N, int H, int W, int C, int OH, int OW, int ph, int pw, int sh, int sw,
                                        int padh, int padw) {
     return maxpool_bwd_bnb_rows(geom(N, H, W, C, OH, OW, ph, pw, sh, sw, padh, padw));
@@ -501,6 +512,35 @@
     a.n_slab = (long)Co * Ci * 9;
     a.N = N; a.Ci = Ci; a.H = H; a.W = W; a.Co = Co;
     stem_wgrad(a, blocks, S(st));
+  });
+  m.def("stem_wgrad_bn", [](uintptr_t x, uintptr_t dy, std::array<uintptr_t, 7> bn, int parts, float count,
+                            std::array<uintptr_t, 3> pool, uintptr_t slab, uintptr_t bias_slab,
+                            std::array<long, 4> gs, int N, int Ci, int H, int W, int Co, int blocks, uintptr_t st) {
+    StemArgs a{};
+    a.x = P<const float*>(x); a.dy = P<const bf16*>(dy); a.slab = P<float*>(slab);
+    a.bias_slab = P<float*>(bias_slab);
+    for (int i = 0; i < 4; ++i) a.gs[i] = gs[i];
+    a.n_slab = (long)Co * Ci * 9;
+    a.N = N; a.Ci = Ci; a.H = H; a.W = W; a.Co = Co;
+    a.bn_x = P<const bf16*>(bn[0]); a.bn_mean = P<const float*>(bn[1]); a.bn_istd = P<const float*>(bn[2]);
+    a.bn_gamma = P<const float*>(bn[3]); a.bn_sums = P<const float*>(bn[4]); a.bn_parts = parts; a.bn_count = count;
+    a.bn_dgamma = P<float*>(bn[5]); a.bn_dbeta = P<float*>(bn[6]);
+    a.pool_dy = P<const bf16*>(pool[0]); a.pool_idx = P<const uint8_t*>(pool[1]); a.pool_y = P<const bf16*>(pool[2]);
+    stem_wgrad(a, blocks, S(st));
+  });
+  m.def("stem_wgrad_blocks_bnt", &stem_wgrad_blocks_bnt);
+  m.def("maxpool_bwd_bnb_sums_supported", [geom](int N, int H, int W, int C, int OH, int OW, int ph, int pw, int sh,
+                                                 int sw, int padh, int padw) {
+    return maxpool_bwd_bnb_sums_supported(geom(N, H, W, C, OH, OW, ph, pw, sh, sw, padh, padw));
+  });
+  m.def("maxpool_bwd_bnb_sums", [geom](uintptr_t dy, uintptr_t idx, uintptr_t ypool, uintptr_t xsel, uintptr_t mean,
+                                       uintptr_t istd, int N, int H, int W, int C, int OH, int OW, int ph, int pw,
+                                       int sh, int sw, int padh, int padw, uintptr_t slab, uintptr_t zero_sums,
+                                       uintptr_t st) {
+    maxpool_bwd_bnb_sums(P<const bf16*>(dy), P<const uint8_t*>(idx), P<const bf16*>(ypool), P<const bf16*>(xsel),
+                         P<const float*>(mean), P<const float*>(istd),
+                         geom(N, H, W, C, OH, OW, ph, pw, sh, sw, padh, padw), P<float*>(slab), P<float*>(zero_sums),
+                         S(st));
   });
   m.def("multi_weight_transpose", [](uintptr_t table, int n, long max_tiles, uintptr_t st, int f32) {
     multi_weight_transpose(P<const int64_t*>(table), n, max_tiles, S(st), f32);
diff --git a/dcnn_amd/csrc/kernels/norm.hip b/dcnn_amd/csrc/kernels/norm.hip
--- a/dcnn_amd/csrc/kernels/norm.hip
+++ b/dcnn_amd/csrc/kernels/norm.hip
@@ -306,9 +306,10 @@
   }
 }
 
-template <int P>
+template <int P, bool XS = false>
 __global__ void __launch_bounds__(256) bn_relu_maxpool_kernel(const bf16* __restrict__ x, bf16* __restrict__ y,
-                                                              uint8_t* __restrict__ idx, PoolGeom g,
+                                                              uint8_t* __restrict__ idx, bf16* __restrict__ xsel,
+                                                              PoolGeom g,
                                                               const float* __restrict__ sums, int parts,
                                                               float count, const float* __restrict__ gamma,
                                                               const float* __restrict__ beta, float eps,
@@ -357,7 +358,7 @@
       oy = (int)(t % g.OH);
       n = (int)(t / g.OH);
     }
-    float sc[8], sf[8], best[8], v[8];
+    float sc[8], sf[8], best[8], v[8], xs[XS ? 8 : 1];
     uint8_t bi[8];
 #pragma unroll
     for (int e = 0; e < 8; ++e) { sc[e] = scale[cv * 8 + e]; sf[e] = shift[cv * 8 + e]; best[e] = -INFINITY; bi[e] = 0; }
@@ -366,6 +367,9 @@
 #pragma unroll
       for (int e = 0; e < 8; ++e) {
         const float r = (float)(bf16)fmaxf(v[e] * sc[e] + sf[e], 0.f);
+        if constexpr (XS) {
+          if (local == 0 || r > best[e]) xs[e] = v[e];
+        }
         if (r > best[e]) { best[e] = r; bi[e] = (uint8_t)local; }
       }
     };
@@ -388,6 +392,7 @@
     }
     *reinterpret_cast<uint4*>(y + i * 8) = pack8(best);
     *reinterpret_cast<uint2*>(idx + i * 8) = *reinterpret_cast<uint2*>(bi);
+    if constexpr (XS) *reinterpret_cast<uint4*>(xsel + i * 8) = pack8(xs);
   }
 }
 
@@ -1107,12 +1112,15 @@
 
 void bn_relu_maxpool(const bf16* x, bf16* y, uint8_t* idx, PoolGeom g, const float* sums, int parts, float count,
                      const float* gamma, const float* beta, float eps, float* save_mean, float* save_istd,
-                     float* run_mean, float* run_var, float momentum, hipStream_t s) {
+                     float* run_mean, float* run_var, float momentum, hipStream_t s, bf16* xsel) {
   if (!bn_relu_maxpool_supported(g)) throw std::runtime_error("bn_relu_maxpool: unsupported geometry");
+  if (xsel && !maxpool_bwd_bnb_sums_supported(g))
+    throw std::runtime_error("bn_relu_maxpool: xsel needs 2 x 2 / stride-2 windows that tile the input");
   const long total = (long)g.N * g.OH * g.OW * g.C / 8;
-  auto k = (g.ph == 2 && g.pw == 2) ? bn_relu_maxpool_kernel<2> : bn_relu_maxpool_kernel<0>;
+  auto k = xsel ? bn_relu_maxpool_kernel<2, true>
+                : (g.ph == 2 && g.pw == 2) ? bn_relu_maxpool_kernel<2> : bn_relu_maxpool_kernel<0>;
   hipLaunchKernelGGL(k, dim3(grid_for(total, 256, 2048)), dim3(256), 2 * g.C * sizeof(float), s,
-                     x, y, idx, g, sums, parts, count, gamma, beta, eps, save_mean, save_istd, run_mean, run_var,
+                     x, y, idx, xsel, g, sums, parts, count, gamma, beta, eps, save_mean, save_istd, run_mean, run_var,
                      momentum);
   DCNN_LAUNCH_CHECK();
 }
diff --git a/dcnn_amd/csrc/kernels/pool_act.hip b/dcnn_amd/csrc/kernels/pool_act.hip
--- a/dcnn_amd/csrc/kernels/pool_act.hip
+++ b/dcnn_amd/csrc/kernels/pool_act.hip
@@ -242,6 +242,14 @@
   }
 }
 
+__device__ __forceinline__ float bnb_q_step(float q, float out, float xv, float mu, float is, bool fused) {
+#pragma clang fp contract(off)
+  const float t = out * (xv - mu);
+  if (fused) return __builtin_fmaf(t, is, q);
+  const float u = t * is;
+  return q + u;
+}
+
 __global__ void __launch_bounds__(256) maxpool_bwd_bnb_kernel(const bf16* __restrict__ dy,
                                                               const uint8_t* __restrict__ idx,
                                                               const bf16* __restrict__ ypool,
@@ -707,7 +715,7 @@
   DCNN_LAUNCH_CHECK();
 }
 
-template <int P>
+template <int P, bool STORE = true>
 __global__ void __launch_bounds__(256) maxpool_bwd_bnb_w_kernel(const bf16* __restrict__ dy,
                                                                 const uint8_t* __restrict__ idx,
                                                                 const bf16* __restrict__ ypool,
@@ -732,10 +740,10 @@
   }
   for (unsigned i = blockIdx.x * 256u + threadIdx.x; i < total; i += gridDim.x * 256u) {
     unsigned t = i / CV;
-    const int ox = (int)(t % g.OW);
+    [[maybe_unused]] const int ox = (int)(t % g.OW);
     t /= g.OW;
-    const int oy = (int)(t % g.OH);
-    const int n = (int)(t / g.OH);
+    [[maybe_unused]] const int oy = (int)(t % g.OH);
+    [[maybe_unused]] const int n = (int)(t / g.OH);
     float d[8], yp[8];
     unpack8(*reinterpret_cast<const uint4*>(dy + (size_t)i * 8), d);
     unpack8(*reinterpret_cast<const uint4*>(ypool + (size_t)i * 8), yp);
@@ -748,11 +756,24 @@
       for (int e = 0; e < 8; ++e) {
         out[e] = (b[e] == local && yp[e] > 0.f) ? d[e] : 0.f;
         s[e] += out[e];
-        q[e] += out[e] * (xv[e] - mu[e]) * is[e];
+        if constexpr (P == 2)
+          q[e] = bnb_q_step(q[e], out[e], xv[e], mu[e], is[e], e != 0);
+        else
+          q[e] += out[e] * (xv[e] - mu[e]) * is[e];
       }
       *reinterpret_cast<uint4*>(dx + xi) = pack8(out);
     };
-    if constexpr (P > 0) {
+    if constexpr (!STORE) {
+      static_assert(P == 2, "sums-only instance: 2 x 2 windows");
+      float xs[8];
+      unpack8(*reinterpret_cast<const uint4*>(x + (size_t)i * 8), xs);
+#pragma unroll
+      for (int e = 0; e < 8; ++e) {
+        const float out = (b[e] < P * P && yp[e] > 0.f) ? d[e] : 0.f;
+        s[e] += out;
+        q[e] = bnb_q_step(q[e], out, xs[e], mu[e], is[e], e != 0);
+      }
+    } else if constexpr (P > 0) {
       size_t xi[P * P];
       uint4 w[P * P];
 #pragma unroll
@@ -811,6 +832,19 @@
   DCNN_LAUNCH_CHECK();
 }
 
+bool maxpool_bwd_bnb_sums_supported(PoolGeom g) {
+  return maxpool_bwd_bnb_supported(g) && g.ph == 2 && g.pw == 2 && g.H % 2 == 0 && g.W % 2 == 0 && g.OH == g.H / 2 &&
+         g.OW == g.W / 2 && (long)g.N * g.H * g.W * g.C < (1l << 31);
+}
+
+void maxpool_bwd_bnb_sums(const bf16* dy, const uint8_t* idx, const bf16* ypool, const bf16* xsel, const float* mean,
+                          const float* istd, PoolGeom g, float* slab, float* zero_sums, hipStream_t s) {
+  if (!maxpool_bwd_bnb_sums_supported(g)) throw std::runtime_error("maxpool_bwd_bnb_sums: unsupported geometry");
+  hipLaunchKernelGGL((maxpool_bwd_bnb_w_kernel<2, false>), dim3(bnb_pool_blocks(g)), dim3(256), 0, s, dy, idx, ypool,
+                     xsel, mean, istd, (bf16*)nullptr, g, slab, zero_sums);
+  DCNN_LAUNCH_CHECK();
+}
+
 void maxpool_fwd(int dt, const void* x, void* y, uint8_t* idx, PoolGeom g, hipStream_t s) { DCNN_DT(dt, maxpool_fwd_t, x, y, idx, g, s); }
 void maxpool_bwd(int dt, const void* dy, const uint8_t* idx, void* dx, PoolGeom g, hipStream_t s) { DCNN_DT(dt, maxpool_bwd_t, dy, idx, dx, g, s); }
 void avgpool_fwd(int dt, const void* x, void* y, PoolGeom g, hipStream_t s) { DCNN_DT(dt, avgpool_fwd_t, x, y, g, s); }
diff --git a/dcnn_amd/csrc/kernels/stem.hip b/dcnn_amd/csrc/kernels/stem.hip
--- a/dcnn_amd/csrc/kernels/stem.hip
+++ b/dcnn_amd/csrc/kernels/stem.hip
@@ -50,6 +50,10 @@
 
 __device__ __forceinline__ bf16x8 cat44(bf16x4 lo, bf16x4 hi) {
   return bf16x8{lo[0], lo[1], lo[2], lo[3], hi[0], hi[1], hi[2], hi[3]};
+}
+
+__device__ __forceinline__ float bn_bwd_dy(const float* coef, int CO, int c, float d, float x) {
+  return coef[c] * d + coef[CO + c] * (x - coef[2 * CO + c]) + coef[3 * CO + c];
 }
 }
 
@@ -142,8 +146,9 @@
   }
 }
 
-template <int NCB, bool BNT>
+template <int NCB, bool BNT, bool POOL = false>
 __global__ void __launch_bounds__(256, NCB <= 2 ? (BNT ? 3 : 4) : 2) stem_wgrad_kernel(StemArgs p) {
+  static_assert(BNT || !POOL, "the pooled operands come with the BatchNorm fold");
   constexpr int CO = NCB * 16;
   extern __shared__ __attribute__((aligned(16))) char smem[];
   bf16* halo = reinterpret_cast<bf16*>(smem);
@@ -179,6 +184,7 @@
     }
   }
   constexpr int NVT = SPX * CO / 8 / 256;
+  constexpr int NPV = NVT / 4;
   f32x4 acc[NCB][3];
 #pragma unroll
   for (int cb = 0; cb < NCB; ++cb)
@@ -197,21 +203,60 @@
     __syncthreads();
     const int tpi = p.H / p.TH, n = tile / tpi, y0 = (tile - n * tpi) * p.TH;
     const unsigned src = (unsigned)((((long)n * p.H + y0) * p.W) * CO * 2);
-#pragma unroll
-    for (int j = 0; j < SPX * CO * 2 / 1024 / 4; ++j) {
-      const int blk = wid * (SPX * CO * 2 / 1024 / 4) + j;
-      glds16_opaque(rs_dy, reinterpret_cast<char*>(dys) + blk * 1024, src + blk * 1024 + lane * 16);
+    if constexpr (!POOL) {
+#pragma unroll
+      for (int j = 0; j < SPX * CO * 2 / 1024 / 4; ++j) {
+        const int blk = wid * (SPX * CO * 2 / 1024 / 4) + j;
+        glds16_opaque(rs_dy, reinterpret_cast<char*>(dys) + blk * 1024, src + blk * 1024 + lane * 16);
+      }
     }
     stage_halo(p, tile, halo);
-    uint4 xv[BNT ? NVT : 1];
-    if constexpr (BNT) {
+    if constexpr (POOL) {
+      const int W2 = p.W >> 1;
+      const long pbase = (((long)n * (p.H >> 1) + (y0 >> 1)) * W2) * CO;
       const char* xb = reinterpret_cast<const char*>(p.bn_x) + src;
+#pragma unroll 1
+      for (int j = 0; j < NPV; ++j) {
+        const int v = threadIdx.x + j * 256, pp = v / (CO / 8), pr = pp / W2, pc = pp - pr * W2;
+        int c0 = (v % (CO / 8)) * 8;
+        asm volatile("" : "+v"(c0));
+        const uint4 gv = *reinterpret_cast<const uint4*>(p.pool_dy + pbase + v * 8);
+        const uint4 yv = *reinterpret_cast<const uint4*>(p.pool_y + pbase + v * 8);
+        const uint2 iv = *reinterpret_cast<const uint2*>(p.pool_idx + pbase + v * 8);
+        uint4 xw[4];
+#pragma unroll
+        for (int k = 0; k < 4; ++k) {
+          const int px = (2 * pr + (k >> 1)) * p.W + 2 * pc + (k & 1);
+          xw[k] = *reinterpret_cast<const uint4*>(xb + (px * CO + c0) * 2);
+        }
+        const uint8_t* b = reinterpret_cast<const uint8_t*>(&iv);
+        float g[8], yp[8];
+        unpack8(gv, g);
+        unpack8(yv, yp);
+#pragma unroll
+        for (int k = 0; k < 4; ++k) {
+          const int px = (2 * pr + (k >> 1)) * p.W + 2 * pc + (k & 1);
+          float d[8], xf[8];
+          unpack8(xw[k], xf);
+#pragma unroll
+          for (int e = 0; e < 8; ++e)
+            d[e] = bn_bwd_dy(coef, CO, c0 + e, (b[e] == k && yp[e] > 0.f) ? g[e] : 0.f, xf[e]);
+          *reinterpret_cast<uint4*>(dys + px * CO + c0) = pack8(d);
+        }
+      }
+      __syncthreads();
+    }
+    uint4 xv[BNT && !POOL ? NVT : 1];
+    if constexpr (BNT && !POOL) {
+      const char* xb = reinterpret_cast<const char*>(p.bn_x) + src;
 #pragma unroll
       for (int j = 0; j < NVT; ++j) xv[j] = *reinterpret_cast<const uint4*>(xb + (threadIdx.x + j * 256) * 16);
     }
-    asm volatile("s_waitcnt vmcnt(0)" ::: "memory");
-    __syncthreads();
-    if constexpr (BNT) {
+    if constexpr (!POOL) {
+      asm volatile("s_waitcnt vmcnt(0)" ::: "memory");
+      __syncthreads();
+    }
+    if constexpr (BNT && !POOL) {
       {
         constexpr int j0 = 0, RV = NVT;
 #pragma unroll
@@ -225,7 +270,7 @@
           unpack8(xv[j], xf);
 #pragma unroll
           for (int e = 0; e < 8; ++e)
-            d[e] = coef[c0 + e] * d[e] + coef[CO + c0 + e] * (xf[e] - coef[2 * CO + c0 + e]) + coef[3 * CO + c0 + e];
+            d[e] = bn_bwd_dy(coef, CO, c0 + e, d[e], xf[e]);
           *q = pack8(d);
         }
       }
@@ -315,14 +360,18 @@
   if (blocks < 1 || blocks > stem_tiles_host(a.N, a.H, a.W)) throw std::runtime_error("stem_wgrad: bad block count");
   a.TH = SPX / a.W;
   a.halo_bytes = (((a.TH + 2) * (a.W + 2) * 8) + 15) / 16 * 16;
-  const bool bnt = a.bn_x != nullptr;
+  const bool bnt = a.bn_x != nullptr, pool = a.pool_dy != nullptr;
   if (bnt && (!a.bn_mean || !a.bn_istd || !a.bn_sums || a.bn_parts < 1 || a.bn_count <= 0.f))
     throw std::runtime_error("stem_wgrad: incomplete BatchNorm-backward operands");
+  if (pool && (!bnt || !a.pool_idx || !a.pool_y))
+    throw std::runtime_error("stem_wgrad: the pooled operands need the BatchNorm fold, argmax and pooled output");
+  if (!pool && !a.dy) throw std::runtime_error("stem_wgrad: no output gradient");
   const int main = a.halo_bytes + SPX * a.Co * 2 + (bnt ? 4 * a.Co * 4 : 0), epi = 4 * a.Co * 48 * 4;
   const int lds = main > epi ? main : epi;
 #define DCNN_SW(C)                                                                                        \
   {                                                                                                       \
-    auto k = bnt ? stem_wgrad_kernel<C, true> : stem_wgrad_kernel<C, false>;                              \
+    auto k = pool ? stem_wgrad_kernel<C, true, true>                                                      \
+                  : bnt ? stem_wgrad_kernel<C, true> : stem_wgrad_kernel<C, false>;                       \
     DCNN_HIP_CHECK(hipFuncSetAttribute((const void*)k, hipFuncAttributeMaxDynamicSharedMemorySize, lds)); \
     hipLaunchKernelGGL(k, dim3(blocks), dim3(256), lds, s, a);                                            \
   }
```

Result: no change. 92030 images/sec, median of 6 (+0.8%).
